# nschloe/flow

Hardware: AMD Instinct MI355X
Metric: ipcs_time_steps_per_sec (higher is better)
Workload: dtype f64

## Files before the change

flow_amd/_hip.py:

```python
import ctypes
import os

import torch

from . import device

_HERE = os.path.dirname(os.path.abspath(__file__))
LIB_PATH = os.path.join(_HERE, 'csrc', 'libflow_hip.so')

REDUCE_WORK = 4096
GMRES_MAX_RESTART = 30
GMRES_PARTIALS = (GMRES_MAX_RESTART + 2) * 1024
GMRES_STATE = 1280
SPMV_ROWS_PER_BLOCK = 256
SPMV_NNZ_PER_BLOCK = 1022
PMG_NNZ_PER_BLOCK = 2044

c_double_p = ctypes.c_void_p
c_int_p = ctypes.c_void_p


class Operator(ctypes.Structure):
    _fields_ = [
        ('kind', ctypes.c_int),
# ... 127 lines not shown
        ('packed16', ctypes.c_void_p),
        ('cbase16', ctypes.c_void_p),
        ('work16_rows', ctypes.c_int),
        ]


class MassStripsS(ctypes.Structure):
    _fields_ = [
        ('nlevels', ctypes.c_int),
        ('rowblocks16', ctypes.c_void_p * 16),
        ('nblocks16', ctypes.c_int * 16),
        ('row_lo_last', ctypes.c_int), ('row_hi_last', ctypes.c_int),
        ]


class MeshS(ctypes.Structure):
    _fields_ = [('nc', ctypes.c_int), ('xy', ctypes.c_void_p),
                ('c0', ctypes.c_int), ('c1', ctypes.c_int)]


class SpaceS(ctypes.Structure):
    _fields_ = [
        ('deg', ctypes.c_int),
        ('n', ctypes.c_int),
        ('nnz', ctypes.c_int),
        ('cell_dofs', ctypes.c_void_p),
        ('cptr', ctypes.c_void_p),
        ('csrc', ctypes.c_void_p),
        ('vptr', ctypes.c_void_p),
        ('vsrc', ctypes.c_void_p),
        ('r0', ctypes.c_int), ('r1', ctypes.c_int),
        ('nnz0', ctypes.c_int), ('nnz1', ctypes.c_int),
        ]


class CoefS(ctypes.Structure):
    _fields_ = [
        ('nl', ctypes.c_int),
        ('cell_stride', ctypes.c_int),
        ('values', ctypes.c_void_p),
        ('G', ctypes.c_void_p),
        ]


FORM_MAX_PROGRAM = 64
FORM_REGISTERS = 8
FORM_MAX_CONSTANTS = 32
FORM_MAX_FIELDS = 6
FORM_MAX_EXPRESSIONS = 4
FORM_MAX_POINTS = 256


class FormS(ctypes.Structure):
    _fields_ = [
        ('nprog', ctypes.c_int),
        ('prog', ctypes.c_int * (4 * FORM_MAX_PROGRAM)),
        ('nconst', ctypes.c_int),
        ('consts', ctypes.c_double * FORM_MAX_CONSTANTS),
        ('nfield', ctypes.c_int),
        ('field', ctypes.c_void_p * FORM_MAX_FIELDS),
        ('field_deg', ctypes.c_int * FORM_MAX_FIELDS),
        ('cell_dofs', ctypes.c_void_p * 2),
        ('nexpr', ctypes.c_int),
        ('expr', ctypes.c_void_p * FORM_MAX_EXPRESSIONS),
        ('expr_nl', ctypes.c_int * FORM_MAX_EXPRESSIONS),
        ('expr_table', ctypes.c_int * FORM_MAX_EXPRESSIONS),
        ('nq', ctypes.c_int),
        ('rule', ctypes.c_void_p),
        ('tables', ctypes.c_void_p),
        ('ntables', ctypes.c_int),
        ('nout', ctypes.c_int),
        ]


class PointGridS(ctypes.Structure):
    _fields_ = [
        ('nx', ctypes.c_int), ('ny', ctypes.c_int),
        ('x0', ctypes.c_double), ('y0', ctypes.c_double),
        ('hx_inv', ctypes.c_double), ('hy_inv', ctypes.c_double),
        ('start', ctypes.c_void_p),
        ('cells', ctypes.c_void_p),
        ]


class NsParams(ctypes.Structure):
    _fields_ = [
        ('dt', ctypes.c_double), ('rho', ctypes.c_double),
        ('mu', ctypes.c_double), ('theta_i', ctypes.c_double),
        ('theta_e', ctypes.c_double),
        ]


ALLREDUCE_FN = ctypes.CFUNCTYPE(ctypes.c_int, ctypes.c_void_p, ctypes.c_int)


class PeerS(ctypes.Structure):
    _fields_ = [
        ('flags', ctypes.c_void_p), ('land', ctypes.c_void_p),
        ('land_cap', ctypes.c_int), ('spin_limit', ctypes.c_int),
        ('nb_flags', ctypes.c_void_p * 2), ('nb_land', ctypes.c_void_p * 2),
        ('seq_host', ctypes.POINTER(ctypes.c_ulonglong * 5)),
        ]


PEER_FLAGS = 16


class CommS(ctypes.Structure):
    _fields_ = [
        ('rank', ctypes.c_int), ('world', ctypes.c_int),
        ('buf', ctypes.c_void_p), ('capacity', ctypes.c_int),
        ('allreduce', ALLREDUCE_FN), ('user', ctypes.c_void_p),
        ('peer', ctypes.POINTER(PeerS)),
        ]


class RcclBinding(ctypes.Structure):
    _fields_ = [('comm', ctypes.c_void_p), ('buf', ctypes.c_void_p),
                ('stream', ctypes.c_void_p)]


class RowsS(ctypes.Structure):
    _fields_ = [
        ('n', ctypes.c_int), ('r0', ctypes.c_int), ('r1', ctypes.c_int),
        ('e0', ctypes.c_int), ('e1', ctypes.c_int), ('nhalo', ctypes.c_int),
        ('send_row', ctypes.c_int * 2), ('send_len', ctypes.c_int * 2),
        ('send_slot', ctypes.c_int * 2),
        ('recv_row', ctypes.c_int * 2), ('recv_len', ctypes.c_int * 2),
        ('recv_slot', ctypes.c_int * 2),
        ]


class MgShardS(ctypes.Structure):
    _fields_ = [
        ('mg', ctypes.POINTER(MgS)),
        ('Ah0', Operator), ('Ps0', Operator), ('Rg', Operator),
        ('Cg', Operator),
        ('up_rowblocks0', ctypes.c_void_p), ('up_nblocks0', ctypes.c_int),
        ('z_lo', ctypes.c_int), ('z_hi', ctypes.c_int),
        ]


class MomentumJvp(ctypes.Structure):
    _fields_ = [
        ('mesh', ctypes.POINTER(MeshS)),
        ('W', ctypes.POINTER(SpaceS)),
        ('bfmask', ctypes.c_void_p),
        ('ui', ctypes.c_void_p),
        ('prm', NsParams),
        ('scratch', ctypes.c_void_p),
        ('nbc', ctypes.c_int),
        ('bc_dofs', ctypes.c_void_p),
        ('bc_mask', ctypes.c_void_p),
        ]


_VP = ctypes.c_void_p
_I = ctypes.c_int
_D = ctypes.c_double
_P = ctypes.POINTER
SYMBOLS = {
    'flow_abi_version': [],
    'flow_launch_count': [_P(ctypes.c_ulonglong)],
    'flow_graph_mode': [_I, ctypes.c_longlong],
    'flow_graph_stats': [_P(ctypes.c_ulonglong)],
    'flow_xcd_tile_host': [_I, _I],
    'flow_spmv_tile_nnz': [_I],
    'flow_operator_apply': [_P(Operator), _VP, _VP, _VP],
    'flow_profile_spmv_begin': [_I, _I],
    'flow_profile_spmv_end': [_P(_D), _P(_I)],
    'flow_profile_event_overhead': [_P(_D), _VP],
    'flow_profile_marker': [_I, _VP],
    'flow_profile_stream_copy': [ctypes.c_size_t, _VP, _VP, _VP],
    'flow_profile_stream_read': [ctypes.c_size_t, _VP, _VP, _VP],
    'flow_operator_diag_inv': [_P(Operator), _VP, _VP, _VP],
    'flow_dot_host': [_I, _VP, _VP, _VP, _P(_D), _VP],
    'flow_norm_host': [_I, _VP, _I, _VP, _P(_D), _VP],
    'flow_axpby': [_I, _D, _VP, _D, _VP, _VP],
    'flow_vmul': [_I, _D, _VP, _VP, _VP, _VP],
    'flow_fill': [_I, _D, _VP, _VP],
    'flow_lincomb': [_I, _I, _P(_D), _P(_VP), _VP, _VP],
    'flow_fingerprint': [_I, _P(_VP), _P(_I), _VP, _VP, _VP],
    'flow_read_doubles': [_VP, _I, _P(_D), _VP],
    'flow_extrapolation_weights': [_I, _P(_D), _D, _I, _I, _P(_D)],
    'flow_scale_rows': [_I, _VP, _VP, _VP, _VP],
    'flow_cg_solve': [_P(Operator), _VP, _P(CoarseS), _P(MgS), _VP, _VP, _D, _D,
                      _I, _I, _I, _VP, ctypes.c_size_t, _P(_I), _P(_D), _VP],
    'flow_cg_solve_guarded': [_P(Operator), _VP, _P(CoarseS), _P(MgS), _VP, _VP,
                              _VP, _D, _D, _I, _I, _I, _VP, ctypes.c_size_t,
                              _P(_I), _P(_D), _P(_I), _VP],
    'flow_mg_apply': [_P(MgS), _I, _VP, _VP, _VP],
    'flow_two_level_apply': [_P(CoarseS), _VP, _VP, _VP, _VP, _VP],
    'flow_bicgstab_solve': [_P(Operator), _VP, _P(IluS), _VP, _VP, _D, _D, _I,
                            _I, _I, _VP, ctypes.c_size_t, _P(_I), _P(_D), _VP],
    'flow_gmres_solve': [_P(Operator), _VP, _P(IluS), _P(PmgS), _VP, _VP, _D,
                         _D, _I, _I, _I, _I, _I, _VP, ctypes.c_size_t, _P(_I),
                         _P(_D), _VP],
    'flow_pmg_pack': [_I, _I, _VP, _VP, _VP, _VP, _VP, _VP, _VP, _VP, _VP],
    'flow_pmg_pack1': [_I, _I, _I, _VP, _VP, _VP, _VP, _VP, _VP, _VP, _VP, _VP,
                       _VP, _VP, _VP, _VP],
    'flow_pmg_cols16': [_I, _VP, _VP, _VP, _VP, _VP, _VP, _VP],
    'flow_pmg_lambda_max': [_P(PmgLevelS), _I, _VP, _VP, _VP, _P(_D), _VP],
    'flow_pmg_apply': [_P(PmgS), _VP, _VP, _VP],
    'flow_tl_apply': [_P(TlS), _VP, _VP, _VP],
    'flow_aggregate_host': [_I, _VP, _VP, _VP, ctypes.c_double, _VP, _VP,
                            _P(ctypes.c_int)],
    'flow_peer_alloc': [ctypes.c_int, _P(ctypes.c_void_p), ctypes.c_char_p],
    'flow_peer_open': [ctypes.c_char_p, _P(ctypes.c_void_p)],
    'flow_peer_close': [_VP],
    'flow_peer_free': [_VP],
    'flow_peer_status': [_P(PeerS), _P(ctypes.c_ulonglong), _VP],
    'flow_mass_pack': [_I, _VP, _VP, _VP, _VP, _VP],
    'flow_mass_pack16': [_I, _I, _VP, _VP, _VP, _VP, _VP, _VP, _VP, _VP, _VP],
    'flow_mass_solve': [_P(MassS), _VP, _VP, _D, _D, _I, _I, _VP,
                        ctypes.c_size_t, _P(_I), _P(_D), _VP],
    'flow_mass_solve_increment': [_P(MassS), _VP, _VP, _VP, _VP, _D, _D, _I, _I, _VP,
                                  ctypes.c_size_t, _P(_I), _P(_D), _VP],
    'flow_gather_rows': [_I, _VP, _I, _VP, _I, _VP, _I, _VP],
    'flow_color_greedy_host': [_I, _VP, _VP, _VP, _P(_I)],
    'flow_color_iterate_host': [_I, _VP, _VP, _VP, _P(_I), _I],
    'flow_ilu0_factor': [_P(IluPlanS), _I, _VP, _VP, _VP, _VP],
    'flow_ilu0_pack': [_P(IluS), _VP, _VP],
    'flow_ilu0_solve': [_P(IluS), _VP, _VP, _VP, _VP],
    'flow_rccl_load': [ctypes.c_char_p],
    'flow_rccl_unique_id': [_VP],
    'flow_rccl_comm_create': [_VP, _I, _I, _P(_VP)],
    'flow_rccl_comm_destroy': [_VP],
    'flow_rccl_allreduce': [_VP, _I],
    'flow_shard_halo': [_P(CommS), _P(RowsS), _I, _VP, _I, _VP],
    'flow_shard_reduce_host': [_P(CommS), _P(RowsS), _I, _VP, _VP, _I, _I, _VP,
                               _P(_D), _VP],
    'flow_shard_cg_solve': [_P(CommS), _P(RowsS), _P(Operator), _VP, _VP, _VP,
                            _D, _D, _I, _I, _I, _VP, ctypes.c_size_t, _P(_I),
                            _P(_D), _P(_I), _VP],
    'flow_shard_mgcg_solve': [_P(CommS), _P(RowsS), _P(Operator), _VP,
                              _P(MgShardS), _VP, _VP, _D, _D, _I, _I, _I, _VP,
                              ctypes.c_size_t, _P(_I), _P(_D), _P(_I), _VP],
    'flow_shard_mass_solve': [_P(CommS), _P(RowsS), _P(MassS), _P(MassStripsS),
                              _VP, _VP, _VP, _VP, _D, _D, _I, _I, _VP,
                              ctypes.c_size_t, _P(_I), _P(_D), _VP],
    'flow_shard_gmres_solve': [_P(CommS), _P(RowsS), _P(Operator), _P(IluS),
                               _P(PmgS), _VP, _VP, _D, _D, _I, _I, _I, _I, _I,
                               _VP, ctypes.c_size_t, _P(_I), _P(_D), _VP],
    'flow_assemble_scalar_matrix': [_I, _P(MeshS), _P(SpaceS), _VP, _VP, _VP],
    'flow_assemble_pressure_rhs': [_P(MeshS), _P(SpaceS), _P(SpaceS), _VP, _VP,
                                   _D, _D, _I, _VP, _VP, _VP],
    'flow_assemble_correction_rhs': [_P(MeshS), _P(SpaceS), _P(SpaceS), _VP,
                                     _VP, _VP, _D, _D, _I, _VP, _VP, _VP],
    'flow_assemble_momentum': [_P(MeshS), _P(SpaceS), _P(SpaceS), _VP, _VP, _VP,
                               _VP, _P(CoefS), _P(CoefS), _P(NsParams), _VP,
                               _VP, _VP, ctypes.c_size_t, _VP],
    'flow_momentum_jvp_apply': [_P(MomentumJvp), _VP, _VP, _VP],
    'flow_assemble_source': [_P(MeshS), _P(SpaceS), _I, _P(CoefS), _VP, _VP,
                             _VP],
    'flow_assemble_magnitude': [_P(MeshS), _P(SpaceS), _I, _VP, _VP, _VP, _VP],
    'flow_assemble_div_adjoint': [_P(MeshS), _P(SpaceS), _P(SpaceS), _VP, _VP,
                                  _VP, _VP],
    'flow_bc_identity_rows': [_P(Operator), _VP, _VP, _I, _VP, _VP],
    'flow_bc_residual': [_I, _VP, _VP, _VP, _VP, _VP],
    'flow_bc_set_values': [_I, _VP, _VP, _VP, _VP],
    'flow_bc_symmetric_matrix': [_I, _VP, _VP, _VP, _VP, _VP, _VP],
    'flow_assemble_heat': [_P(MeshS), _P(SpaceS), _P(SpaceS), _VP, _D, _D, _I,
                           _VP, _VP, _VP, _VP, _VP, _VP],
    'flow_assemble_heat_supg_source': [_P(MeshS), _P(SpaceS), _P(SpaceS), _VP,
                                       _D, _D, _P(CoefS), _VP, _VP, _VP, _VP],
    'flow_form_functional': [_P(MeshS), _P(FormS), _VP, _VP, _P(_D), _VP],
    'flow_form_load_vector': [_P(MeshS), _P(SpaceS), _P(FormS), _VP, _VP, _VP],
    'flow_form_facet_functional': [_P(MeshS), _P(FormS), _I, _VP, _VP, _VP, _VP,
                                   _P(_D), _VP],
    'flow_locate_points': [_P(MeshS), _P(PointGridS), _I, _VP, _VP, _VP, _VP],
    'flow_form_points': [_P(MeshS), _P(FormS), _I, _VP, _VP, _VP, _VP],
    }

_LIB = None


class HipError(RuntimeError):
    pass


class NotConverged(RuntimeError):
    '''Krylov / Newton non-convergence.  A RuntimeError, because callers of the
    reference catch exactly that (tests/test_boussinesq.py:254).'''


ABI_VERSION = 30


def load_library():
    global _LIB
    if _LIB is None:
        if not os.path.isfile(LIB_PATH):
            raise HipError(
                'libflow_hip.so not found at %s -- build it with '
                '`python -c "import __graft_entry__ as g; g.build()"` or '
                '`make -C flow_amd/csrc`' % LIB_PATH
                )
        lib = ctypes.CDLL(LIB_PATH)
        lib.flow_last_error.restype = ctypes.c_char_p
        lib.flow_last_error.argtypes = []
        for name, argtypes in SYMBOLS.items():
            fn = getattr(lib, name)
            fn.restype = ctypes.c_int
            fn.argtypes = argtypes
        got = lib.flow_abi_version()
        if got != ABI_VERSION:
            raise HipError(
                '%s is ABI version %d, these bindings are version %d: '
                'rebuild it (`make -C flow_amd/csrc`)'
                % (LIB_PATH, got, ABI_VERSION))
        _LIB = lib
    return _LIB


def launch_count():
    n = ctypes.c_ulonglong(0)
    check(load_library().flow_launch_count(ctypes.byref(n)))
    return int(n.value)


_GRAPHS = {'mode': None}


def graph_mode(mode, auto_rows=-1, sites=0):
    check(load_library().flow_graph_mode(int(mode) | (int(sites) << 4),
                                         int(auto_rows)))
    _GRAPHS['mode'] = int(mode)


def graphs_possible():
    if _GRAPHS['mode'] is not None:
        return _GRAPHS['mode'] != 0
    return os.environ.get('FLOW_AMD_GRAPHS', '0') not in ('', '0')


def graph_stats():
    v = (ctypes.c_ulonglong * 8)()
    check(load_library().flow_graph_stats(v))
    return {'graphs': int(v[0]), 'captures': int(v[1]), 'replays': int(v[2]),
            'nodes': int(v[3]), 'captures_cg': int(v[4]),
            'captures_gmres': int(v[5]), 'captures_mass': int(v[6])}


def spmv_tile_nnz(kind=0):
    return int(load_library().flow_spmv_tile_nnz(int(kind)))


def lib():
    handle = load_library()
    if not device.on_gpu():
        raise HipError(
            'flow_amd needs an AMD GPU (MI355X): the hot path has no CPU '
            'fallback'
            )
    return handle


def check(rc):
    if rc == 0:
        return
    msg = load_library().flow_last_error().decode('utf-8', 'replace')
    if rc == 1:
        raise NotConverged(msg)
    if rc == 2:
        raise ValueError(msg)
    raise HipError(msg)


def _ptr(t, dtype, numel=None, name='operand'):
    if t is None:
        return None
    if not isinstance(t, torch.Tensor):
        raise TypeError('%s: expected a torch tensor' % name)
    if t.dtype != dtype:
        raise TypeError('%s: dtype %s, expected %s' % (name, t.dtype, dtype))
    if not t.is_cuda:
        raise HipError('%s is not in device memory' % name)
    if not t.is_contiguous():
        raise ValueError('%s is not contiguous' % name)
    if numel is not None and t.numel() < numel:
        raise ValueError(
            '%s has %d elements, needs %d' % (name, t.numel(), numel)
            )
    return ctypes.c_void_p(t.data_ptr())


def f64(t, numel=None, name='fp64 operand'):
    return _ptr(t, torch.float64, numel, name)


def f32(t, numel=None, name='fp32 operand'):
    return _ptr(t, torch.float32, numel, name)


def f16(t, numel=None, name='fp16 operand'):
    return _ptr(t, torch.float16, numel, name)


def i32(t, numel=None, name='int32 operand'):
    return _ptr(t, torch.int32, numel, name)


def u8(t, numel=None, name='uint8 operand'):
    return _ptr(t, torch.uint8, numel, name)

# ... 27 lines not shown
```

flow_amd/csrc/assembly_kernels.hip:

```cpp
#include <cstdlib>

#include "fem_device.h"

namespace flow {

template <int NP>
__global__ __launch_bounds__(kBlock) void gather_kernel(
    int nout, const int* __restrict__ ptr, const int* __restrict__ src,
    const double* __restrict__ scratch, size_t plane_stride, size_t out_stride,
    double* __restrict__ out, const double* __restrict__ stop,
    const unsigned char* __restrict__ idrow = nullptr, size_t id_stride = 0,
    const double* __restrict__ v = nullptr, size_t v_stride = 0) {
  if (stopped(stop)) return;
  for (int k = blockIdx.x * blockDim.x + threadIdx.x; k < nout;
       k += gridDim.x * blockDim.x) {
    const int a = ptr[k];
    const int b = ptr[k + 1];
    double s[NP];
#pragma unroll
    for (int p = 0; p < NP; ++p) s[p] = 0.0;
    for (int t = a; t < b; t += 4) {
      int idx[4];
#pragma unroll
      for (int j = 0; j < 4; ++j) idx[j] = t + j < b ? src[t + j] : -1;
      double w[NP][4];
#pragma unroll
      for (int p = 0; p < NP; ++p)
#pragma unroll
        for (int j = 0; j < 4; ++j)
          w[p][j] = idx[j] >= 0 ? scratch[p * plane_stride + idx[j]] : 0.0;
#pragma unroll
      for (int p = 0; p < NP; ++p)
#pragma unroll
        for (int j = 0; j < 4; ++j) s[p] += w[p][j];
    }
    if (idrow) {
#pragma unroll
      for (int p = 0; p < NP; ++p)
        if (idrow[p * id_stride + k]) s[p] = v[p * v_stride + k];
    }
#pragma unroll
    for (int p = 0; p < NP; ++p) out[static_cast<size_t>(p) * out_stride + k] = s[p];
  }
}

int gather(int nout, int nplanes, const int* ptr, const int* src,
           const double* scratch, size_t plane_stride, double* out,
           hipStream_t st, size_t out_stride, int r0, int r1, const double* stop,
           const unsigned char* idrow, const double* v, size_t v_stride) {
  const size_t os = out_stride ? out_stride : static_cast<size_t>(nout);
  const size_t ids = static_cast<size_t>(nout);
  if (r1 > 0) {
    ptr += r0;
    out += r0;
    if (idrow) idrow += r0;
    if (v) v += r0;
    nout = r1 - r0;
  }
  const dim3 grid(grid_for(nout, kBlock, 1 << 20));
  FLOW_REQUIRE(nplanes == 1 || nplanes == 2, "gather: 1 or 2 planes");
  if (nplanes == 1)
    hipLaunchKernelGGL(gather_kernel<1>, grid, dim3(kBlock), 0, st, nout, ptr,
                       src, scratch, plane_stride, os, out, stop, idrow, ids, v,
                       v_stride);
  else
    hipLaunchKernelGGL(gather_kernel<2>, grid, dim3(kBlock), 0, st, nout, ptr,
                       src, scratch, plane_stride, os, out, stop, idrow, ids, v,
                       v_stride);
  FLOW_CHECK_LAUNCH();
  return FLOW_OK;
}

template <int NL>
__device__ __forceinline__ void load_local(const double* __restrict__ u, int n,
                                           const int* __restrict__ cd, int nc,
                                           int c, int ,
                                           double U[2][NL]) {
#pragma unroll
  for (int i = 0; i < NL; ++i) {
    const int d = cd[i * nc + c];
    U[0][i] = u[d];
    U[1][i] = u[static_cast<size_t>(n) + d];
  }
}

template <int DEG>
__global__ __launch_bounds__(kBlock) void scalar_matrix_kernel(
    int kind, int nc, const double* __restrict__ xy,
    double* __restrict__ scratch) {
  constexpr int NL = Elem<DEG>::NL;
  constexpr int NQ = Elem<2>::NQ;
  const int c = blockIdx.x * blockDim.x + threadIdx.x;
  if (c >= nc) return;
  const Geom g = load_geom(xy, nc, c);
  double Ke[NL][NL];
#pragma unroll
  for (int i = 0; i < NL; ++i)
#pragma unroll
    for (int j = 0; j < NL; ++j) Ke[i][j] = 0.0;
  if (kind == 2) {
#pragma unroll
    for (int i = 0; i < 3; ++i) Ke[i][i] = g.adet / 6.0;
  } else {
#pragma unroll
    for (int q = 0; q < NQ; ++q) {
      const double L[3] = {kQ7L[q][0], kQ7L[q][1], kQ7L[q][2]};
      const double w = 0.5 * kQ7W[q] * g.adet;
      double phi[NL], dphi[NL][3], gphi[NL][2];
      basis<DEG>(L, phi, dphi);
      phys_grad<NL>(g, dphi, gphi);
#pragma unroll
      for (int i = 0; i < NL; ++i)
#pragma unroll
        for (int j = 0; j < NL; ++j)
          Ke[i][j] += (kind == 0)
                          ? w * (gphi[i][0] * gphi[j][0] + gphi[i][1] * gphi[j][1])
                          : w * phi[i] * phi[j];
    }
  }
#pragma unroll
  for (int i = 0; i < NL; ++i)
#pragma unroll
    for (int j = 0; j < NL; ++j)
      scratch[static_cast<size_t>(i * NL + j) * nc + c] = Ke[i][j];
}

template <int DEG>
__global__ __launch_bounds__(kBlock) void pressure_rhs_kernel(
    int nc, int cb, int ce, const double* __restrict__ xy, const int* __restrict__ cdu, int nu,
    const int* __restrict__ cdp, const double* __restrict__ u,
    const double* __restrict__ p0, double alpha_rho_dt, double mu,
    int rotational, double* __restrict__ scratch) {
  constexpr int NL = Elem<DEG>::NL;
  const int c = cb + xcd_tile(blockIdx.x, gridDim.x) * blockDim.x + threadIdx.x;
  if (c >= ce) return;
  const Geom g = load_geom(xy, nc, c);
  double U[2][NL];
  load_local<NL>(u, nu, cdu, nc, c, 2, U);
  double d[3];
  div_at_vertices<DEG>(g, U, d);
  const double area = 0.5 * g.adet;
  const double dsum = d[0] + d[1] + d[2];
  double gp[2] = {0.0, 0.0};
#pragma unroll
  for (int k = 0; k < 3; ++k) {
    double coef = p0[cdp[k * nc + c]];
    if (rotational) coef -= mu * d[k];
    gp[0] += coef * g.gl[k][0];
    gp[1] += coef * g.gl[k][1];
  }
#pragma unroll
  for (int i = 0; i < 3; ++i) {
    const double b = -alpha_rho_dt * (area / 12.0) * (dsum + d[i]) +
                     area * (gp[0] * g.gl[i][0] + gp[1] * g.gl[i][1]);
    scratch[static_cast<size_t>(i) * nc + c] = b;
  }
}

template <int DEG>
__global__ __launch_bounds__(kBlock) void correction_rhs_kernel(
    int nc, int cb, int ce, const double* __restrict__ xy, const int* __restrict__ cdu, int nu,
    const int* __restrict__ cdp, const double* __restrict__ u,
    const double* __restrict__ p1, const double* __restrict__ p0, double dt_rho,
    double mu, int rotational, double* __restrict__ scratch) {
  constexpr int NL = Elem<DEG>::NL;
  constexpr int NQ = Elem<2>::NQ;
  const int c = cb + xcd_tile(blockIdx.x, gridDim.x) * blockDim.x + threadIdx.x;
  if (c >= ce) return;
  const Geom g = load_geom(xy, nc, c);
  double U[2][NL];
  load_local<NL>(u, nu, cdu, nc, c, 2, U);
  double d[3] = {0.0, 0.0, 0.0};
  if (rotational & 1) div_at_vertices<DEG>(g, U, d);
  const double mass = (rotational & 2) ? 0.0 : 1.0;
  double gphi_f[2] = {0.0, 0.0};
#pragma unroll
  for (int k = 0; k < 3; ++k) {
    const int dof = cdp[k * nc + c];
    const double coef = p1[dof] - p0[dof] + mu * d[k];
    gphi_f[0] += coef * g.gl[k][0];
    gphi_f[1] += coef * g.gl[k][1];
  }
  double acc[2][NL];
#pragma unroll
  for (int a = 0; a < 2; ++a)
#pragma unroll
    for (int i = 0; i < NL; ++i) acc[a][i] = 0.0;
#pragma unroll
  for (int q = 0; q < NQ; ++q) {
    const double L[3] = {kQ7L[q][0], kQ7L[q][1], kQ7L[q][2]};
    const double w = 0.5 * kQ7W[q] * g.adet;
    double phi[NL], dphi[NL][3];
    basis<DEG>(L, phi, dphi);
#pragma unroll
    for (int a = 0; a < 2; ++a) {
      double uq = 0.0;
#pragma unroll
      for (int j = 0; j < NL; ++j) uq += U[a][j] * phi[j];
      const double val = w * (mass * uq - dt_rho * gphi_f[a]);
#pragma unroll
      for (int i = 0; i < NL; ++i) acc[a][i] += val * phi[i];
    }
  }
#pragma unroll
  for (int a = 0; a < 2; ++a)
#pragma unroll
    for (int i = 0; i < NL; ++i)
      scratch[static_cast<size_t>(a * NL + i) * nc + c] = acc[a][i];
}

template <int NL>
__device__ __forceinline__ void add_source(const flow_coef& f, int nc, int c,
                                           int dim, double scale,
                                           double acc[][NL]) {
  const size_t nce = f.cell_stride ? static_cast<size_t>(nc) : 1;
  const size_t cc = f.cell_stride ? static_cast<size_t>(c) : 0;
  for (int a = 0; a < dim; ++a) {
    for (int l = 0; l < f.nl; ++l) {
      const double F = scale * f.values[(static_cast<size_t>(a) * f.nl + l) * nce + cc];
#pragma unroll
      for (int i = 0; i < NL; ++i) acc[a][i] += F * f.G[l * NL + i];
    }
  }
}

template <int DEG>
__global__ __launch_bounds__(kBlock) void source_kernel(
    int nc, const double* __restrict__ xy, int dim, flow_coef f,
    double* __restrict__ scratch) {
  constexpr int NL = Elem<DEG>::NL;
  const int c = blockIdx.x * blockDim.x + threadIdx.x;
  if (c >= nc) return;
  const Geom g = load_geom(xy, nc, c);
  double acc[2][NL];
#pragma unroll
  for (int a = 0; a < 2; ++a)
#pragma unroll
    for (int i = 0; i < NL; ++i) acc[a][i] = 0.0;
  add_source<NL>(f, nc, c, dim, g.adet, acc);
  for (int a = 0; a < dim; ++a)
#pragma unroll
    for (int i = 0; i < NL; ++i)
      scratch[static_cast<size_t>(a * NL + i) * nc + c] = acc[a][i];
}

template <int NL>
__device__ __forceinline__ void add_rhs_weak_point(
    double w, double rho, double mu, const double U[2][NL], const double P[3],
    const double L[3], const double phi[NL], const double gphi[NL][2],
    double acc[2][NL]) {
  double uq[2] = {0.0, 0.0};
  double gu[2][2] = {{0.0, 0.0}, {0.0, 0.0}};
#pragma unroll
  for (int j = 0; j < NL; ++j) {
#pragma unroll
    for (int a = 0; a < 2; ++a) {
      uq[a] += U[a][j] * phi[j];
      gu[a][0] += U[a][j] * gphi[j][0];
      gu[a][1] += U[a][j] * gphi[j][1];
    }
  }
  const double pq = P[0] * L[0] + P[1] * L[1] + P[2] * L[2];
  const double conv[2] = {gu[0][0] * uq[0] + gu[0][1] * uq[1],
                          gu[1][0] * uq[0] + gu[1][1] * uq[1]};
#pragma unroll
  for (int i = 0; i < NL; ++i) {
    const double ugp = uq[0] * gphi[i][0] + uq[1] * gphi[i][1];
#pragma unroll
    for (int a = 0; a < 2; ++a) {
      double r = -0.5 * rho * (conv[a] * phi[i] - ugp * uq[a]);
      r -= mu * ((gu[a][0] + gu[0][a]) * gphi[i][0] +
                 (gu[a][1] + gu[1][a]) * gphi[i][1]);
      r += pq * gphi[i][a];
      acc[a][i] += w * r;
    }
  }
}

template <int DEG>
__device__ __forceinline__ void add_rhs_weak_facets(
    int mask, double scale, double mu, const Geom& g,
    const double U[2][Elem<DEG>::NL], const double P[3],
    double acc[2][Elem<DEG>::NL]) {
  constexpr int NL = Elem<DEG>::NL;
  for (int lf = 0; lf < 3; ++lf) {
    if (!((mask >> lf) & 1)) continue;
    const int v0 = facet_v0(lf), v1 = facet_v1(lf);
    const double nL[2] = {-g.gl[lf][0] * g.adet, -g.gl[lf][1] * g.adet};
    for (int gq = 0; gq < 2; ++gq) {
      const double s = gq == 0 ? FLOW_G2A : FLOW_G2B;
      double L[3] = {0.0, 0.0, 0.0};
      L[v0] = 1.0 - s;
      L[v1] = s;
      double phi[NL], dphi[NL][3], gphi[NL][2];
      basis<DEG>(L, phi, dphi);
      phys_grad<NL>(g, dphi, gphi);
      double gu[2][2] = {{0.0, 0.0}, {0.0, 0.0}};
#pragma unroll
      for (int j = 0; j < NL; ++j)
#pragma unroll
        for (int a = 0; a < 2; ++a) {
          gu[a][0] += U[a][j] * gphi[j][0];
          gu[a][1] += U[a][j] * gphi[j][1];
        }
      const double pq = P[0] * L[0] + P[1] * L[1] + P[2] * L[2];
      const double w = 0.5 * scale;
#pragma unroll
      for (int a = 0; a < 2; ++a) {
        const double t = -pq * nL[a] + mu * (gu[0][a] * nL[0] + gu[1][a] * nL[1]);
#pragma unroll
        for (int i = 0; i < NL; ++i) acc[a][i] += w * t * phi[i];
      }
    }
  }
}

template <int DEG>
__global__ __launch_bounds__(kBlock) void momentum_residual_kernel(
    int nc, int cb, int ce, const double* __restrict__ xy, const int* __restrict__ cdu, int nu,
    const int* __restrict__ cdp, const int* __restrict__ bfmask,
    const double* __restrict__ ui, const double* __restrict__ u0,
    const double* __restrict__ p0, flow_coef f0, flow_coef f1,
    flow_ns_params prm, double* __restrict__ scratch) {
  constexpr int NL = Elem<DEG>::NL;
  constexpr int NQ = Elem<DEG>::NQ;
  const int c = cb + xcd_tile(blockIdx.x, gridDim.x) * blockDim.x + threadIdx.x;
  if (c >= ce) return;
  const Geom g = load_geom(xy, nc, c);
  double Ui[2][NL], U0[2][NL], P[3];
  load_local<NL>(ui, nu, cdu, nc, c, 2, Ui);
  load_local<NL>(u0, nu, cdu, nc, c, 2, U0);
#pragma unroll
  for (int k = 0; k < 3; ++k) P[k] = p0[cdp[k * nc + c]];
  const int mask = bfmask[c];
  const double ci = -prm.dt / prm.rho * prm.theta_i;
  const double cexp = -prm.dt / prm.rho * prm.theta_e;
  double acc[2][NL];
#pragma unroll
  for (int a = 0; a < 2; ++a)
#pragma unroll
    for (int i = 0; i < NL; ++i) acc[a][i] = 0.0;

#pragma unroll
  for (int q = 0; q < NQ; ++q) {
    const double L[3] = {qpoint<DEG>(q, 0), qpoint<DEG>(q, 1), qpoint<DEG>(q, 2)};
    const double w = 0.5 * qweight<DEG>(q) * g.adet;
    double phi[NL], dphi[NL][3], gphi[NL][2];
    basis<DEG>(L, phi, dphi);
    phys_grad<NL>(g, dphi, gphi);
#pragma unroll
    for (int a = 0; a < 2; ++a) {
      double du = 0.0;
#pragma unroll
      for (int j = 0; j < NL; ++j) du += (Ui[a][j] - U0[a][j]) * phi[j];
#pragma unroll
      for (int i = 0; i < NL; ++i) acc[a][i] += w * du * phi[i];
    }
    if (ci != 0.0)
      add_rhs_weak_point<NL>(w * ci, prm.rho, prm.mu, Ui, P, L, phi, gphi, acc);
    if (cexp != 0.0)
      add_rhs_weak_point<NL>(w * cexp, prm.rho, prm.mu, U0, P, L, phi, gphi, acc);
  }
  if (mask) {
    if (ci != 0.0) add_rhs_weak_facets<DEG>(mask, ci, prm.mu, g, Ui, P, acc);
    if (cexp != 0.0) add_rhs_weak_facets<DEG>(mask, cexp, prm.mu, g, U0, P, acc);
  }
  if (ci != 0.0) add_source<NL>(f1, nc, c, 2, ci * g.adet, acc);
  if (cexp != 0.0) add_source<NL>(f0, nc, c, 2, cexp * g.adet, acc);
#pragma unroll
  for (int a = 0; a < 2; ++a)
#pragma unroll
    for (int i = 0; i < NL; ++i)
      scratch[static_cast<size_t>(a * NL + i) * nc + c] = acc[a][i];
}

template <int DEG>
__global__ __launch_bounds__(kBlock) void momentum_jvp_kernel(
    int nc, int cb, int ce, const double* __restrict__ xy,
    const int* __restrict__ cdu, int nu, int nv,
    const int* __restrict__ bfmask, const double* __restrict__ ui,
    const double* __restrict__ v, flow_ns_params prm,
    const double* __restrict__ prm_dev,
    double* __restrict__ scratch, const double* __restrict__ stop) {
  constexpr int NL = Elem<DEG>::NL;
  constexpr int NQ = Elem<DEG>::NQ;
  if (stopped(stop)) return;
  const int c = cb + xcd_tile(blockIdx.x, gridDim.x) * blockDim.x + threadIdx.x;
  if (c >= ce) return;
  const Geom g = load_geom(xy, nc, c);
  double U[2][NL], V[2][NL];
  load_local<NL>(ui, nu, cdu, nc, c, 2, U);
  load_local<NL>(v, nv, cdu, nc, c, 2, V);
  const int mask = bfmask[c];
  const double ci = prm_dev ? load_scalar(prm_dev)
                            : -prm.dt / prm.rho * prm.theta_i;
  const double hr = prm_dev ? load_scalar(prm_dev + 1) : 0.5 * prm.rho;
  const double mu = prm_dev ? load_scalar(prm_dev + 2) : prm.mu;
  double acc[2][NL];
#pragma unroll
  for (int a = 0; a < 2; ++a)
#pragma unroll
    for (int i = 0; i < NL; ++i) acc[a][i] = 0.0;

#pragma unroll
  for (int q = 0; q < NQ; ++q) {
    const double L[3] = {qpoint<DEG>(q, 0), qpoint<DEG>(q, 1), qpoint<DEG>(q, 2)};
    const double w = 0.5 * qweight<DEG>(q) * g.adet;
    double uq[2], vq[2], gu[2][2], gv[2][2];
#pragma unroll
    for (int a = 0; a < 2; ++a) {
      uq[a] = eval_at<DEG>(U[a], L);
      vq[a] = eval_at<DEG>(V[a], L);
      double gur[3], gvr[3];
      ref_gradient<DEG>(U[a], L, gur);
      ref_gradient<DEG>(V[a], L, gvr);
#pragma unroll
      for (int d = 0; d < 2; ++d) {
        gu[a][d] = gur[0] * g.gl[0][d] + gur[1] * g.gl[1][d] + gur[2] * g.gl[2][d];
        gv[a][d] = gvr[0] * g.gl[0][d] + gvr[1] * g.gl[1][d] + gvr[2] * g.gl[2][d];
      }
    }
#pragma unroll
    for (int a = 0; a < 2; ++a) {
      const double dconv = gv[a][0] * uq[0] + gv[a][1] * uq[1] +
                           gu[a][0] * vq[0] + gu[a][1] * vq[1];
      const double s0 = w * (vq[a] - ci * hr * dconv);
      double S1[2];
#pragma unroll
      for (int d = 0; d < 2; ++d)
        S1[d] = w * ci * (hr * (vq[d] * uq[a] + uq[d] * vq[a]) -
                          mu * (gv[a][d] + gv[d][a]));
      double T[3];
#pragma unroll
      for (int k = 0; k < 3; ++k) T[k] = g.gl[k][0] * S1[0] + g.gl[k][1] * S1[1];
      test_accumulate<DEG>(L, s0, T, acc[a]);
    }
  }
  if (mask && ci != 0.0) {
    const double P0[3] = {0.0, 0.0, 0.0};
    add_rhs_weak_facets<DEG>(mask, ci, mu, g, V, P0, acc);
  }
#pragma unroll
  for (int a = 0; a < 2; ++a)
#pragma unroll
    for (int i = 0; i < NL; ++i)
      scratch[static_cast<size_t>(a * NL + i) * nc + c] = acc[a][i];
}

template <int DEG>
__global__ __launch_bounds__(kBlock) void momentum_jvp_pair_kernel(
    int nc, int cb, int ce, const double* __restrict__ xy,
    const int* __restrict__ cdu, int nu, int nv,
    const int* __restrict__ bfmask, const double* __restrict__ ui,
    const double* __restrict__ v, flow_ns_params prm,
    const double* __restrict__ prm_dev,
    double* __restrict__ scratch, const double* __restrict__ stop) {
  constexpr int NL = Elem<DEG>::NL;
  constexpr int NQ = Elem<DEG>::NQ;
  if (stopped(stop)) return;
  const int t = xcd_tile(blockIdx.x, gridDim.x) * blockDim.x + threadIdx.x;
  const int c = cb + (t >> 1);
  const int a = t & 1;
  if (c >= ce) return;
  const Geom g = load_geom(xy, nc, c);
  double U[NL], V[NL];
#pragma unroll
  for (int i = 0; i < NL; ++i) {
    const int d = cdu[i * nc + c];
    U[i] = ui[static_cast<size_t>(a) * nu + d];
    V[i] = v[static_cast<size_t>(a) * nv + d];
  }
  const int mask = bfmask[c];
  const double ci = prm_dev ? load_scalar(prm_dev)
                            : -prm.dt / prm.rho * prm.theta_i;
  const double hr = prm_dev ? load_scalar(prm_dev + 1) : 0.5 * prm.rho;
  const double mu = prm_dev ? load_scalar(prm_dev + 2) : prm.mu;
  double acc[NL];
#pragma unroll
  for (int i = 0; i < NL; ++i) acc[i] = 0.0;

#pragma unroll
  for (int q = 0; q < NQ; ++q) {
    const double L[3] = {qpoint<DEG>(q, 0), qpoint<DEG>(q, 1), qpoint<DEG>(q, 2)};
    const double w = 0.5 * qweight<DEG>(q) * g.adet;
    const double uq = eval_at<DEG>(U, L);
    const double vq = eval_at<DEG>(V, L);
    double gur[3], gvr[3], gu[2], gv[2];
    ref_gradient<DEG>(U, L, gur);
    ref_gradient<DEG>(V, L, gvr);
#pragma unroll
    for (int d = 0; d < 2; ++d) {
      gu[d] = gur[0] * g.gl[0][d] + gur[1] * g.gl[1][d] + gur[2] * g.gl[2][d];
      gv[d] = gvr[0] * g.gl[0][d] + gvr[1] * g.gl[1][d] + gvr[2] * g.gl[2][d];
    }
    const double uo = __shfl_xor(uq, 1, 64);
    const double vo = __shfl_xor(vq, 1, 64);
    const double cross = __shfl_xor(a == 0 ? gv[1] : gv[0], 1, 64);
    const double u0 = a == 0 ? uq : uo, u1 = a == 0 ? uo : uq;
    const double v0 = a == 0 ? vq : vo, v1 = a == 0 ? vo : vq;
    const double dconv = gv[0] * u0 + gv[1] * u1 + gu[0] * v0 + gu[1] * v1;
    const double s0 = w * (vq - ci * hr * dconv);
    const double t0 = a == 0 ? gv[0] : cross;
    const double t1 = a == 0 ? cross : gv[1];
    double S1[2];
    S1[0] = w * ci * (hr * (v0 * uq + u0 * vq) - mu * (gv[0] + t0));
    S1[1] = w * ci * (hr * (v1 * uq + u1 * vq) - mu * (gv[1] + t1));
    double T[3];
#pragma unroll
    for (int k = 0; k < 3; ++k) T[k] = g.gl[k][0] * S1[0] + g.gl[k][1] * S1[1];
    test_accumulate<DEG>(L, s0, T, acc);
  }
  if (mask && ci != 0.0) {
    for (int lf = 0; lf < 3; ++lf) {
      if (!((mask >> lf) & 1)) continue;
      const int f0 = facet_v0(lf), f1 = facet_v1(lf);
      const double nL[2] = {-g.gl[lf][0] * g.adet, -g.gl[lf][1] * g.adet};
      for (int gq = 0; gq < 2; ++gq) {
        const double sg = gq == 0 ? FLOW_G2A : FLOW_G2B;
        double L[3] = {0.0, 0.0, 0.0};
        L[f0] = 1.0 - sg;
        L[f1] = sg;
        double gvr[3], gv[2];
        ref_gradient<DEG>(V, L, gvr);
#pragma unroll
        for (int d = 0; d < 2; ++d)
          gv[d] = gvr[0] * g.gl[0][d] + gvr[1] * g.gl[1][d] + gvr[2] * g.gl[2][d];
        const double cross = __shfl_xor(a == 0 ? gv[1] : gv[0], 1, 64);
        const double tn = a == 0 ? gv[0] * nL[0] + cross * nL[1]
                                 : cross * nL[0] + gv[1] * nL[1];
        const double wt = 0.5 * ci * mu * tn;
        double phi[NL], dphi[NL][3];
        basis<DEG>(L, phi, dphi);
#pragma unroll
        for (int i = 0; i < NL; ++i) acc[i] += wt * phi[i];
      }
    }
  }
#pragma unroll
  for (int i = 0; i < NL; ++i)
    scratch[static_cast<size_t>(a * NL + i) * nc + c] = acc[i];
}

__global__ void bc_copy_kernel(int nbc, const int* __restrict__ dofs, int n,
                               int r0, int r1, const double* __restrict__ v,
                               int vs, double* __restrict__ out, int os,
                               const double* __restrict__ stop) {
  if (stopped(stop)) return;
  const int k = blockIdx.x * blockDim.x + threadIdx.x;
  if (k >= nbc) return;
  const int d = dofs[k];
  const int a = d / n;
  const int row = d - a * n;
  if (row >= r0 && row < r1)
    out[static_cast<size_t>(a) * os + row] = v[static_cast<size_t>(a) * vs + row];
}

template <int DEG>
struct BasisTab {
  double phi[Elem<DEG>::NQ][Elem<DEG>::NL];
  double dphi[Elem<DEG>::NQ][Elem<DEG>::NL][3];
};

template <int DEG>
__global__ __launch_bounds__(kBlock) void momentum_jacobian_kernel(
    int nc, int cb, int ce, const double* __restrict__ xy, const int* __restrict__ cdu, int nu,
    const int* __restrict__ bfmask, const double* __restrict__ ui,
    flow_ns_params prm, double* __restrict__ scratch) {
  constexpr int NL = Elem<DEG>::NL;
  constexpr int NQ = Elem<DEG>::NQ;
  constexpr int NP = NL * NL;
  __shared__ double s_uq[NQ][2][64];
  __shared__ double s_gu[NQ][4][64];
  __shared__ BasisTab<DEG> tab;

  const int lane = threadIdx.x & 63;
  const int grp = threadIdx.x >> 6;
  const int c = cb + blockIdx.x * 64 + lane;
  const bool active = c < ce;
  const int cc = active ? c : ce - 1;

  for (int t = threadIdx.x; t < NQ * NL; t += kBlock) {
    const int q = t / NL, i = t % NL;
    const double L[3] = {qpoint<DEG>(q, 0), qpoint<DEG>(q, 1), qpoint<DEG>(q, 2)};
    double phi[NL], dphi[NL][3];
    basis<DEG>(L, phi, dphi);
    tab.phi[q][i] = phi[i];
    tab.dphi[q][i][0] = dphi[i][0];
    tab.dphi[q][i][1] = dphi[i][1];
    tab.dphi[q][i][2] = dphi[i][2];
  }

  const Geom g = load_geom(xy, nc, cc);
  const int mask = bfmask[cc];
  {
    double U[2][NL];
    load_local<NL>(ui, nu, cdu, nc, cc, 2, U);
    for (int q = grp; q < NQ; q += 4) {
      const double L[3] = {qpoint<DEG>(q, 0), qpoint<DEG>(q, 1),
                           qpoint<DEG>(q, 2)};
// ... 503 lines not shown
    const flow_mesh* mesh, const flow_space* W, const flow_space* P,
    const double* u, const double* p1, const double* p0, double dt_rho,
    double mu, int rotational, double* scratch, double* b, void* stream) {
  int rc = check_mesh_space(mesh, W);
  if (rc) return rc;
  if ((rc = check_mesh_space(mesh, P))) return rc;
  FLOW_REQUIRE(P->deg == 1 && W->vptr && W->vsrc, "spaces");
  FLOW_REQUIRE(u && p1 && p0 && scratch && b, "pointers");
  hipStream_t st = as_stream(stream);
  const CellRange cr(mesh);
  FLOW_DISPATCH_DEG(W->deg, correction_rhs_kernel, cell_grid(cr.count()), st,
                    mesh->nc, cr.cb, cr.ce, mesh->xy, W->cell_dofs, W->n,
                    P->cell_dofs, u, p1, p0, dt_rho, mu, rotational, scratch);
  const int nl = W->deg == 1 ? 3 : 6;
  return gather(W->n, 2, W->vptr, W->vsrc, scratch,
                static_cast<size_t>(nl) * mesh->nc, b, st, 0, W->r0, W->r1);
}

static int check_coef(const flow_coef* f) {
  FLOW_REQUIRE(f && f->nl >= 1 && f->nl <= 21 && f->values && f->G, "coefficient");
  FLOW_REQUIRE(f->cell_stride == 0 || f->cell_stride == 1, "coefficient stride");
  return FLOW_OK;
}

extern "C" int flow_assemble_source(const flow_mesh* mesh, const flow_space* V,
                                    int dim, const flow_coef* f, double* scratch,
                                    double* b, void* stream) {
  int rc = check_mesh_space(mesh, V);
  if (rc) return rc;
  if ((rc = check_coef(f))) return rc;
  FLOW_REQUIRE(dim == 1 || dim == 2, "dim");
  FLOW_REQUIRE(scratch && b && V->vptr && V->vsrc, "pointers");
  hipStream_t st = as_stream(stream);
  FLOW_DISPATCH_DEG(V->deg, source_kernel, cell_grid(mesh->nc), st, mesh->nc,
                    mesh->xy, dim, *f, scratch);
  const int nl = V->deg == 1 ? 3 : 6;
  return gather(V->n, dim, V->vptr, V->vsrc, scratch,
                static_cast<size_t>(nl) * mesh->nc, b, st);
}

extern "C" int flow_assemble_momentum(
    const flow_mesh* mesh, const flow_space* W, const flow_space* P,
    const int* bfmask, const double* ui, const double* u0, const double* p0,
    const flow_coef* f0, const flow_coef* f1, const flow_ns_params* prm,
    double* scratch, double* F, double* Jvals, size_t j_plane_stride,
    void* stream) {
  int rc = check_mesh_space(mesh, W);
  if (rc) return rc;
  if ((rc = check_mesh_space(mesh, P))) return rc;
  if ((rc = check_coef(f0))) return rc;
  if ((rc = check_coef(f1))) return rc;
  FLOW_REQUIRE(P->deg == 1, "pressure space must be P1");
  FLOW_REQUIRE(bfmask && ui && u0 && p0 && prm && scratch, "pointers");
  FLOW_REQUIRE(prm->dt > 0.0 && prm->rho > 0.0 && prm->mu > 0.0, "parameters");
  hipStream_t st = as_stream(stream);
  const int nl = W->deg == 1 ? 3 : 6;
  const CellRange cr(mesh);
  if (F) {
    FLOW_REQUIRE(W->vptr && W->vsrc, "vector map");
    FLOW_DISPATCH_DEG(W->deg, momentum_residual_kernel, cell_grid(cr.count()),
                      st, mesh->nc, cr.cb, cr.ce, mesh->xy, W->cell_dofs, W->n,
                      P->cell_dofs, bfmask, ui, u0, p0, *f0, *f1, *prm, scratch);
    if ((rc = gather(W->n, 2, W->vptr, W->vsrc, scratch,
                     static_cast<size_t>(nl) * mesh->nc, F, st, 0, W->r0,
                     W->r1)))
      return rc;
  }
  if (Jvals) {
    FLOW_REQUIRE(W->cptr && W->csrc && W->nnz > 0, "matrix map");
    FLOW_REQUIRE(j_plane_stride >= (size_t)W->nnz, "Jacobian plane stride");
    FLOW_DISPATCH_DEG(W->deg, momentum_jacobian_kernel,
                      dim3((cr.count() + 63) / 64), st, mesh->nc, cr.cb, cr.ce,
                      mesh->xy, W->cell_dofs, W->n, bfmask, ui, *prm, scratch);
    int k0 = 0, k1 = W->nnz;
    if (W->r1 > 0) {
      FLOW_REQUIRE(W->nnz0 >= 0 && W->nnz0 < W->nnz1 && W->nnz1 <= W->nnz,
                   "space nonzero range");
      k0 = W->nnz0;
      k1 = W->nnz1;
    }
    hipLaunchKernelGGL(gather_blocks_kernel,
                       dim3(grid_for(k1 - k0, kBlock, 1 << 20)), dim3(kBlock), 0,
                       st, k0, k1, mesh->nc, nl * nl, W->cptr, W->csrc, scratch,
                       j_plane_stride, Jvals);
    FLOW_CHECK_LAUNCH();
  }
  return FLOW_OK;
}

int flow::momentum_jvp_check(const flow_momentum_jvp* J) {
  FLOW_REQUIRE(J != nullptr, "matrix-free Jacobian is NULL");
  int rc = check_mesh_space(J->mesh, J->W);
  if (rc) return rc;
  FLOW_REQUIRE(J->W->vptr && J->W->vsrc, "vector map");
  FLOW_REQUIRE(J->bfmask && J->ui && J->scratch, "matrix-free Jacobian pointers");
  FLOW_REQUIRE(J->prm.dt > 0.0 && J->prm.rho > 0.0 && J->prm.mu > 0.0,
               "parameters");
  FLOW_REQUIRE(J->nbc >= 0 && (J->nbc == 0 || J->bc_dofs), "Dirichlet dofs");
  return FLOW_OK;
}

__global__ void jvp_params_kernel(flow_ns_params prm, double* __restrict__ dst) {
  if (threadIdx.x == 0) {
    store_scalar(dst, -prm.dt / prm.rho * prm.theta_i);
    store_scalar(dst + 1, 0.5 * prm.rho);
    store_scalar(dst + 2, prm.mu);
  }
}

int flow::momentum_jvp_params(const flow_momentum_jvp* J, double* dst,
                              hipStream_t st) {
  hipLaunchKernelGGL(jvp_params_kernel, dim3(1), dim3(64), 0, st, J->prm, dst);
  FLOW_CHECK_LAUNCH();
  return FLOW_OK;
}

int flow::momentum_jvp_apply(const flow_momentum_jvp* J, const double* v,
                             double* out, hipStream_t st, int v_stride,
                             int out_stride, const double* stop,
                             const double* prm_dev) {
  const flow_mesh* mesh = J->mesh;
  const flow_space* W = J->W;
  const int nl = W->deg == 1 ? 3 : 6;
  const int vs = v_stride ? v_stride : W->n;
  const int os = out_stride ? out_stride : W->n;
  const CellRange cr(mesh);
  int rc;
  static const bool pair = [] {
    const char* e = getenv("FLOW_AMD_JVP_PAIR");
    return e && e[0] == '1';
  }();
  if (W->deg == 2 && pair) {
    hipLaunchKernelGGL(momentum_jvp_pair_kernel<2>, cell_grid(2 * cr.count()),
                       dim3(kBlock), 0, st, mesh->nc, cr.cb, cr.ce, mesh->xy,
                       W->cell_dofs, W->n, vs, J->bfmask, J->ui, v, J->prm,
                       prm_dev, J->scratch, stop);
    FLOW_CHECK_LAUNCH();
  } else {
    FLOW_DISPATCH_DEG(W->deg, momentum_jvp_kernel, cell_grid(cr.count()), st,
                      mesh->nc, cr.cb, cr.ce, mesh->xy, W->cell_dofs, W->n, vs,
                      J->bfmask, J->ui, v, J->prm, prm_dev, J->scratch, stop);
  }
  if ((rc = gather(W->n, 2, W->vptr, W->vsrc, J->scratch,
                   static_cast<size_t>(nl) * mesh->nc, out, st, os, W->r0,
                   W->r1, stop, J->nbc > 0 ? J->bc_mask : nullptr, v, vs)))
    return rc;
  if (J->nbc > 0 && !J->bc_mask) {
    const int r0 = W->r1 > 0 ? W->r0 : 0, r1 = W->r1 > 0 ? W->r1 : W->n;
    hipLaunchKernelGGL(bc_copy_kernel, dim3(grid_for(J->nbc)), dim3(kBlock), 0,
                       st, J->nbc, J->bc_dofs, W->n, r0, r1, v, vs, out, os, stop);
    FLOW_CHECK_LAUNCH();
  }
  return FLOW_OK;
}

extern "C" int flow_momentum_jvp_apply(const flow_momentum_jvp* J,
                                       const double* v, double* out,
                                       void* stream) {
  int rc = momentum_jvp_check(J);
  if (rc) return rc;
  FLOW_REQUIRE(v && out && v != out, "jvp vectors");
  return momentum_jvp_apply(J, v, out, as_stream(stream), 0, 0, nullptr);
}

extern "C" int flow_assemble_magnitude(const flow_mesh* mesh, const flow_space* W,
                                       int mode, const double* u,
                                       double* scratch, double* b,
                                       void* stream) {
  int rc = check_mesh_space(mesh, W);
  if (rc) return rc;
  FLOW_REQUIRE(mode == 0 || mode == 1, "mode");
  FLOW_REQUIRE(u && scratch && b && W->vptr && W->vsrc, "pointers");
  hipStream_t st = as_stream(stream);
  const CellRange cr(mesh);
  FLOW_DISPATCH_DEG(W->deg, magnitude_kernel, cell_grid(cr.count()), st, mesh->nc,
                    cr.cb, cr.ce, mesh->xy, W->cell_dofs, W->n, u, mode, scratch);
  return gather(W->n, 1, W->vptr, W->vsrc, scratch, 0, b, st, 0, W->r0, W->r1);
}

extern "C" int flow_assemble_div_adjoint(const flow_mesh* mesh,
                                         const flow_space* W, const flow_space* P,
                                         const double* p, double* scratch,
                                         double* out, void* stream) {
  int rc = check_mesh_space(mesh, W);
  if (rc) return rc;
  if ((rc = check_mesh_space(mesh, P))) return rc;
  FLOW_REQUIRE(P->deg == 1, "pressure space must be P1");
  FLOW_REQUIRE(p && scratch && out && W->vptr && W->vsrc, "pointers");
  hipStream_t st = as_stream(stream);
  FLOW_DISPATCH_DEG(W->deg, div_adjoint_kernel, cell_grid(mesh->nc), st, mesh->nc,
                    mesh->xy, P->cell_dofs, p, scratch);
  const int nl = W->deg == 1 ? 3 : 6;
  return gather(W->n, 2, W->vptr, W->vsrc, scratch,
                static_cast<size_t>(nl) * mesh->nc, out, st);
}

extern "C" int flow_bc_identity_rows(const flow_operator* A, double* vals_planes,
                                     const int* diag_idx, int nbc,
                                     const int* dofs, void* stream) {
  FLOW_REQUIRE(A && A->n > 0 && A->nnz > 0 && A->rowptr, "operator");
  FLOW_REQUIRE(A->kind >= 0 && A->kind <= 2, "operator kind");
  FLOW_REQUIRE(vals_planes && diag_idx && nbc >= 0, "pointers");
  if (nbc == 0) return FLOW_OK;
  FLOW_REQUIRE(dofs != nullptr, "dofs");
  FLOW_REQUIRE(vals_planes == A->vals[0], "vals_planes must be A->vals[0]");
  const long long stride =
      A->kind == 0 ? A->nnz : static_cast<long long>(A->vals[1] - A->vals[0]);
  FLOW_REQUIRE(stride >= A->nnz, "plane stride");
  if (A->kind == 2)
    FLOW_REQUIRE(A->vals[2] - A->vals[0] == 2 * stride &&
                     A->vals[3] - A->vals[0] == 3 * stride,
                 "equally spaced planes");
  hipLaunchKernelGGL(bc_identity_rows_kernel, dim3(grid_for(nbc)), dim3(kBlock),
                     0, as_stream(stream), A->kind, A->n,
                     static_cast<size_t>(stride), A->rowptr, diag_idx, nbc, dofs,
                     vals_planes);
  FLOW_CHECK_LAUNCH();
  return FLOW_OK;
}

extern "C" int flow_bc_residual(int nbc, const int* dofs, const double* g,
                                const double* u, double* F, void* stream) {
  FLOW_REQUIRE(nbc >= 0, "nbc");
  if (nbc == 0) return FLOW_OK;
  FLOW_REQUIRE(dofs && g && u && F, "pointers");
  hipLaunchKernelGGL(bc_residual_kernel, dim3(grid_for(nbc)), dim3(kBlock), 0,
                     as_stream(stream), nbc, dofs, g, u, F);
  FLOW_CHECK_LAUNCH();
  return FLOW_OK;
}

extern "C" int flow_bc_set_values(int nbc, const int* dofs, const double* g,
                                  double* x, void* stream) {
  FLOW_REQUIRE(nbc >= 0, "nbc");
  if (nbc == 0) return FLOW_OK;
  FLOW_REQUIRE(dofs && g && x, "pointers");
  hipLaunchKernelGGL(bc_residual_kernel, dim3(grid_for(nbc)), dim3(kBlock), 0,
                     as_stream(stream), nbc, dofs, g,
                     static_cast<const double*>(nullptr), x);
  FLOW_CHECK_LAUNCH();
  return FLOW_OK;
}

extern "C" int flow_bc_symmetric_matrix(int n, const int* rowptr,
                                        const int* cols, const double* vals_in,
                                        const unsigned char* isbc,
                                        double* vals_out, void* stream) {
  FLOW_REQUIRE(n > 0 && rowptr && cols && vals_in && isbc && vals_out, "pointers");
  hipLaunchKernelGGL(bc_symmetric_kernel, dim3(grid_for(n)), dim3(kBlock), 0,
                     as_stream(stream), n, rowptr, cols, vals_in, isbc, vals_out);
  FLOW_CHECK_LAUNCH();
  return FLOW_OK;
}

extern "C" int flow_assemble_heat(const flow_mesh* mesh, const flow_space* Q,
                                  const flow_space* W, const double* conv,
                                  double kappa, double rho_cp, int supg,
                                  double* scratch, double* Avals,
                                  double* Msupg_vals, double* tau_out,
                                  int* status_dev, void* stream) {
  int rc = check_mesh_space(mesh, Q);
  if (rc) return rc;
  if ((rc = check_mesh_space(mesh, W))) return rc;
  FLOW_REQUIRE(conv && scratch && Avals && status_dev, "pointers");
  FLOW_REQUIRE(Q->cptr && Q->csrc && Q->nnz > 0, "matrix map");
  FLOW_REQUIRE(!supg || Msupg_vals, "Msupg_vals required with supg");
  FLOW_REQUIRE(kappa > 0.0 && rho_cp > 0.0, "coefficients");
  hipStream_t st = as_stream(stream);
  const CellRange cr(mesh);
  const dim3 grid = cell_grid(cr.count());
#define FLOW_HEAT(DQ, DW)                                                      \
  do {                                                                         \
    if (supg)                                                                  \
      hipLaunchKernelGGL((heat_kernel<DQ, DW, true>), grid, dim3(kBlock), 0, st, \
                         mesh->nc, cr.cb, cr.ce, mesh->xy, W->cell_dofs, W->n, \
                         conv, kappa, rho_cp, scratch, tau_out, status_dev);   \
    else                                                                       \
      hipLaunchKernelGGL((heat_kernel<DQ, DW, false>), grid, dim3(kBlock), 0,  \
                         st, mesh->nc, cr.cb, cr.ce, mesh->xy, W->cell_dofs,   \
                         W->n, conv, kappa, rho_cp, scratch, tau_out,          \
                         status_dev);                                          \
  } while (0)
  if (Q->deg == 1 && W->deg == 1) FLOW_HEAT(1, 1);
  else if (Q->deg == 1 && W->deg == 2) FLOW_HEAT(1, 2);
  else if (Q->deg == 2 && W->deg == 1) FLOW_HEAT(2, 1);
  else FLOW_HEAT(2, 2);
#undef FLOW_HEAT
  FLOW_CHECK_LAUNCH();
  const int nl = Q->deg == 1 ? 3 : 6;
  const size_t plane = static_cast<size_t>(nl) * nl * mesh->nc;
  int k0 = 0, k1 = 0;
  if (Q->r1 > 0) {
    FLOW_REQUIRE(Q->nnz0 >= 0 && Q->nnz0 < Q->nnz1 && Q->nnz1 <= Q->nnz,
                 "space nonzero range");
    k0 = Q->nnz0;
    k1 = Q->nnz1;
  }
  if ((rc = gather(Q->nnz, 1, Q->cptr, Q->csrc, scratch, 0, Avals, st, 0, k0, k1)))
    return rc;
  if (supg)
    return gather(Q->nnz, 1, Q->cptr, Q->csrc, scratch + plane, 0, Msupg_vals, st,
                  0, k0, k1);
  return FLOW_OK;
}

extern "C" int flow_assemble_heat_supg_source(
// ... 30 lines not shown
```

flow_amd/csrc/common.h:

```cpp
#pragma once
#include <hip/hip_runtime.h>

#include <algorithm>
#include <cstdarg>
#include <cstdio>
#include <functional>
#include <vector>

#include "../../include/flow_hip.h"

namespace flow {
extern unsigned long long g_launches;
}
#undef hipLaunchKernelGGL
#define hipLaunchKernelGGL(kernelName, numBlocks, numThreads, memPerBlock,        \
                           streamId, ...)                                       \
  do {                                                                          \
    ++flow::g_launches;                                                         \
    (kernelName)<<<(numBlocks), (numThreads), (memPerBlock), (streamId)>>>(     \
        __VA_ARGS__);                                                           \
  } while (0)

namespace flow {

void set_error(const char* fmt, ...);

inline hipStream_t as_stream(void* s) { return static_cast<hipStream_t>(s); }

int ilu_apply(const flow_ilu* ilu, const double* in, double* out, double* work,
              hipStream_t st, const double* stop = nullptr);
int ilu_check(const flow_ilu* ilu, int op_size);

int pmg_apply(const flow_pmg* M, const double* r, double* z, hipStream_t st,
              const double* stop = nullptr);
int pmg_check(const flow_pmg* M, int op_size);
int tl_apply(const flow_tl* T, const double* r, double* z, hipStream_t st,
             const double* stop = nullptr);
int tl_check(const flow_tl* T, int op_size);
int operator_apply(const flow_operator* A, const double* x, double* y,
                   hipStream_t st, const double* stop = nullptr);
int operator_size(const flow_operator* A);
int sum_partials_host(double* work, int nparts, double* host, hipStream_t st);
int check_operator(const flow_operator* A);
int fill(int n, double value, double* y, hipStream_t st);
struct NoEarly {
  __device__ __forceinline__ void operator()(int, bool) const {}
};

enum Slot {
  kGamma = 0, kAlpha, kBeta, kRes2, kB2, kRho, kOmega, kRhoNew, kTmp,
  kBreak, kTarget2, kDone, kConvIt, kIter, kNumSlots = 16
};
int read_state(const double* S, double* host, hipStream_t st);
int check_comm(const flow_comm* c, long long need);
int check_rows(const flow_rows* R);
int exchange(const flow_comm* c, int count);
int exchange_halo(const flow_comm* C, const flow_rows* R, int ncomp, int sum_count,
                  int hoff, hipStream_t st);

int gather(int nout, int nplanes, const int* ptr, const int* src,
           const double* scratch, size_t plane_stride, double* out,
           hipStream_t st, size_t out_stride = 0, int r0 = 0, int r1 = 0,
           const double* stop = nullptr, const unsigned char* idrow = nullptr,
           const double* v = nullptr, size_t v_stride = 0);
int momentum_jvp_check(const flow_momentum_jvp* J);
int momentum_jvp_apply(const flow_momentum_jvp* J, const double* v, double* out,
                       hipStream_t st, int v_stride = 0, int out_stride = 0,
                       const double* stop = nullptr,
                       const double* prm_dev = nullptr);
int momentum_jvp_params(const flow_momentum_jvp* J, double* dst, hipStream_t st);

constexpr long long kReplayAutoRows = 1500000;
struct KeyHash {
  unsigned long long h = 1469598103934665603ull;
  void bytes(const void* p, size_t n) {
    const unsigned char* c = static_cast<const unsigned char*>(p);
    for (size_t i = 0; i < n; ++i) h = (h ^ c[i]) * 1099511628211ull;
  }
  template <class T> KeyHash& pod(const T& v) {
    bytes(&v, sizeof(T));
    return *this;
  }
  template <class T> KeyHash& obj(const T* p) {
    const unsigned char tag = p ? 1 : 0;
    bytes(&tag, 1);
    if (p) bytes(p, sizeof(T));
    return *this;
  }
};
enum ReplaySite { kReplayCg = 1, kReplayGmres = 2, kReplayMass = 4 };
bool replay_wanted(long long rows, int site);
int replay_prepare(unsigned long long key, int site, hipStream_t st,
                   const std::function<int()>& body, hipGraphExec_t* exec,
                   int* nodes);
int replay_launch(hipGraphExec_t exec, int nodes, hipStream_t st);
void key_operator(KeyHash& k, const flow_operator* A, bool skip_prm = false);

#define FLOW_CHECK_HIP(expr)                                                 \
  do {                                                                       \
    hipError_t err_ = (expr);                                                \
    if (err_ != hipSuccess) {                                                \
      flow::set_error("%s failed: %s (%s:%d)", #expr, hipGetErrorString(err_), \
                      __FILE__, __LINE__);                                   \
      return FLOW_HIP_ERROR;                                                 \
    }                                                                        \
  } while (0)

#define FLOW_REQUIRE(cond, msg)                                  \
  do {                                                           \
    if (!(cond)) {                                               \
      flow::set_error("invalid argument: %s (%s)", msg, #cond);  \
      return FLOW_INVALID;                                       \
    }                                                            \
  } while (0)

#define FLOW_CHECK_LAUNCH() FLOW_CHECK_HIP(hipGetLastError())

constexpr int kBlock = 256;
constexpr int kRedBlocks = 1024;
constexpr int kMaxGrid = 2048;

inline int grid_for(long long n, int per_block = kBlock, int cap = kMaxGrid) {
  long long g = (n + per_block - 1) / per_block;
  if (g < 1) g = 1;
  if (g > cap) g = cap;
  return static_cast<int>(g);
}

__device__ __forceinline__ double load_scalar(const double* p) {
  return __hip_atomic_load(const_cast<double*>(p), __ATOMIC_RELAXED,
                           __HIP_MEMORY_SCOPE_SYSTEM);
}
__device__ __forceinline__ void store_scalar(double* p, double v) {
  __hip_atomic_store(p, v, __ATOMIC_RELAXED, __HIP_MEMORY_SCOPE_SYSTEM);
}

__device__ __forceinline__ bool stopped(const double* stop) {
  return stop != nullptr && load_scalar(stop) != 0.0;
}

constexpr int kXcdRun = 64;
__host__ __device__ __forceinline__ int xcd_tile(int b, int nwg) {
  constexpr int kGroup = 8 * kXcdRun;
  const int full = (nwg / kGroup) * kGroup;
  if (b < full) {
    const int g = b / kGroup, i = b - g * kGroup;
    return g * kGroup + (i & 7) * kXcdRun + (i >> 3);
  }
  const int nt = nwg - full, i = b - full;
  const int q = nt >> 3, r = nt & 7, xcd = i & 7;
  return full + (xcd < r ? xcd * (q + 1) : r * (q + 1) + (xcd - r) * q) +
         (i >> 3);
}

__device__ inline double block_sum(double v) {
  __shared__ double wave_part[4];
#pragma unroll
  for (int off = 32; off > 0; off >>= 1) v += __shfl_down(v, off, 64);
  const int lane = threadIdx.x & 63;
  const int wave = threadIdx.x >> 6;
  __syncthreads();
  if (lane == 0) wave_part[wave] = v;
  __syncthreads();
  if (threadIdx.x == 0) v = wave_part[0] + wave_part[1] + wave_part[2] + wave_part[3];
  return v;
}

__device__ inline double block_sum_once(double v) {
  __shared__ double wave_part_once[4];
#pragma unroll
  for (int off = 32; off > 0; off >>= 1) v += __shfl_down(v, off, 64);
  if ((threadIdx.x & 63) == 0) wave_part_once[threadIdx.x >> 6] = v;
  __syncthreads();
  if (threadIdx.x == 0)
    v = wave_part_once[0] + wave_part_once[1] + wave_part_once[2] +
        wave_part_once[3];
  return v;
}

__device__ inline double block_max(double v) {
  __shared__ double wave_part_m[4];
#pragma unroll
  for (int off = 32; off > 0; off >>= 1) v = fmax(v, __shfl_down(v, off, 64));
  const int lane = threadIdx.x & 63;
  const int wave = threadIdx.x >> 6;
  __syncthreads();
  if (lane == 0) wave_part_m[wave] = v;
  __syncthreads();
  if (threadIdx.x == 0)
    v = fmax(fmax(wave_part_m[0], wave_part_m[1]), fmax(wave_part_m[2], wave_part_m[3]));
  return v;
}

}
```

flow_amd/csrc/la_kernels.hip:

```cpp
#include <cstring>

#include "common.h"
#include "csr_stream.h"

namespace flow {

thread_local char g_error[512] = "";

void set_error(const char* fmt, ...) {
  va_list ap;
  va_start(ap, fmt);
  vsnprintf(g_error, sizeof(g_error), fmt, ap);
  va_end(ap);
}

static_assert(3 * kRedBlocks + kNumSlots <= FLOW_REDUCE_WORK, "work size");


template <bool DOT>
__global__ __launch_bounds__(kBlock) void spmv_stream_kernel(
    int n, const int* __restrict__ rowptr, const int* __restrict__ cols,
    const double* __restrict__ vals0, const double* __restrict__ vals1,
    const int* __restrict__ rowblocks, const double* __restrict__ x,
    double* __restrict__ y, double* __restrict__ dpart,
// ... 44 lines not shown
        g = ci * yi;
        rr = yi * yi;
      }
    } else {
      y[r] = ci - s;
    }
  }
  if (DOTS) {
    g = block_sum(g);
    rr = block_sum(rr);
    if (threadIdx.x == 0) {
      gpart[blockIdx.x] = g;
      rpart[blockIdx.x] = rr;
    }
  }
}

template <bool DOTS>
__global__ __launch_bounds__(kBlock) void mg_up2_kernel(
    const int* __restrict__ rowblocks, const int* __restrict__ p_rowptr,
    const int* __restrict__ p_cols, const double* __restrict__ p_vals,
    const int* __restrict__ a_rowptr, const int* __restrict__ a_cols,
    const double* __restrict__ a_vals, const double* __restrict__ xc,
    const double* __restrict__ c, const double* __restrict__ dinv, double omega,
    double* __restrict__ y, double* __restrict__ gpart,
    double* __restrict__ rpart, const double* __restrict__ stop,
    int own_lo = 0, int own_hi = 0x7fffffff) {
  __shared__ double prod_p[kTile];
  __shared__ double prod_a[kTile];
  if (stopped(stop)) return;
  const int tile = xcd_tile(blockIdx.x, gridDim.x);
  const int r0 = rowblocks[tile];
  const int r1 = rowblocks[tile + 1];
  const int r = r0 + threadIdx.x;
  double ci = 0.0, di = 0.0;
  if (r < r1) {
    ci = c[r];
    di = dinv[r];
  }
  const double sp = stream_rows_sum(r0, r1, p_rowptr, p_cols, p_vals, xc, prod_p);
  const double sa = stream_rows_sum(r0, r1, a_rowptr, a_cols, a_vals, c, prod_a);
  double g = 0.0, rr = 0.0;
  if (r < r1) {
    const double yi = sp + omega * di * (2.0 * ci - sa);
    y[r] = yi;
    if (DOTS && r >= own_lo && r < own_hi) {
      g = ci * yi;
      rr = yi * yi;
    }
  }
  if (DOTS) {
    g = block_sum(g);
    rr = block_sum(rr);
    if (threadIdx.x == 0) {
      gpart[blockIdx.x] = g;
      rpart[blockIdx.x] = rr;
    }
  }
}

template <bool DOT>
__global__ __launch_bounds__(kBlock) void spmv_stream_block2_kernel(
    int n, const int* __restrict__ rowptr, const int* __restrict__ cols,
    const double* __restrict__ vxx, const double* __restrict__ vxy,
    const double* __restrict__ vyx, const double* __restrict__ vyy,
    const int* __restrict__ rowblocks, const double* __restrict__ x,
    double* __restrict__ y, double* __restrict__ dpart,
    const double* __restrict__ stop) {
  __shared__ double prod0[kTile2];
  __shared__ double prod1[kTile2];
  if (stopped(stop)) return;
  const int tile = xcd_tile(blockIdx.x, gridDim.x);
  const int r0 = rowblocks[tile];
  const int r1 = rowblocks[tile + 1];
  const int k0 = rowptr[r0];
  const int k1 = rowptr[r1];
  const int ka = k0 & ~1;
  const int r = r0 + threadIdx.x;
  int a = 0, b = 0;
  if (r < r1) {
    a = rowptr[r] - ka;
    b = rowptr[r + 1] - ka;
  }
  const int npair = (k1 - ka + 1) >> 1;
  const int2* __restrict__ c2p = reinterpret_cast<const int2*>(cols + ka);
  const double2* __restrict__ pxx = reinterpret_cast<const double2*>(vxx + ka);
  const double2* __restrict__ pxy = reinterpret_cast<const double2*>(vxy + ka);
  const double2* __restrict__ pyx = reinterpret_cast<const double2*>(vyx + ka);
  const double2* __restrict__ pyy = reinterpret_cast<const double2*>(vyy + ka);
#pragma unroll
  for (int j = 0; j < kPairs2; ++j) {
    const int p = threadIdx.x + j * kBlock;
    if (p < npair) {
      const int2 c = c2p[p];
      const double2 axx = pxx[p], axy = pxy[p], ayx = pyx[p], ayy = pyy[p];
      const int cx = 2 * p >= k0 - ka ? c.x : cols[k0];
      const int cy = 2 * p + 1 < k1 - ka ? c.y : cols[k0];
      const double u0 = x[cx], u1 = x[n + cx];
      const double w0 = x[cy], w1 = x[n + cy];
      prod0[2 * p] = axx.x * u0 + axy.x * u1;
      prod1[2 * p] = ayx.x * u0 + ayy.x * u1;
      prod0[2 * p + 1] = axx.y * w0 + axy.y * w1;
      prod1[2 * p + 1] = ayx.y * w0 + ayy.y * w1;
    }
  }
  __syncthreads();
  double t = 0.0;
  if (r < r1) {
    double s0 = 0.0, s1 = 0.0;
    for (int k = a; k < b; ++k) {
      s0 += prod0[k];
      s1 += prod1[k];
    }
    y[r] = s0;
    y[n + r] = s1;
    if (DOT) t = s0 * x[r] + s1 * x[n + r];
  }
  if (DOT) {
    t = block_sum_once(t);
    if (threadIdx.x == 0) dpart[blockIdx.x] = t;
  }
}

template <bool DOT>
__global__ __launch_bounds__(kBlock) void spmv_stream_pair_kernel(
    int n, const int* __restrict__ rowptr, const int* __restrict__ cols,
    const double* __restrict__ vals, const int* __restrict__ rowblocks,
    const unsigned char* __restrict__ mask, const double* __restrict__ x,
    double* __restrict__ y, int xs, double* __restrict__ dpart,
    const double* __restrict__ stop) {
  __shared__ double2 prod[kTile2];
  if (stopped(stop)) return;
  int r, r1;
  const double2 s =
      stream_tile_pair_row_sum(rowptr, cols, vals, rowblocks, x, xs, prod, r, r1);
  double s0 = s.x, s1 = s.y;
  double t = 0.0;
  if (r < r1) {
    const double x0 = x[r], x1 = x[xs + r];
    if (!mask[r]) s0 = x0;
    if (!mask[n + r]) s1 = x1;
    y[r] = s0;
    y[xs + r] = s1;
    if (DOT) t = s0 * x0 + s1 * x1;
  }
  if (DOT) {
    t = block_sum_once(t);
    if (threadIdx.x == 0) dpart[blockIdx.x] = t;
  }
}

int check_operator(const flow_operator* A) {
  FLOW_REQUIRE(A != nullptr, "operator is NULL");
  FLOW_REQUIRE(A->kind >= 0 && A->kind <= 4, "operator kind");
  if (A->kind == 3) {
    const flow_momentum_jvp* J =
        static_cast<const flow_momentum_jvp*>(A->matfree);
    int rc = momentum_jvp_check(J);
    if (rc) return rc;
    FLOW_REQUIRE(A->n == J->W->n, "matrix-free operator size");
    return FLOW_OK;
  }
  FLOW_REQUIRE(A->n > 0 && A->nnz > 0 && A->nblocks > 0, "operator sizes");
  FLOW_REQUIRE(A->rowptr && A->cols && A->rowblocks, "operator pattern");
  const int planes = (A->kind == 0 || A->kind == 4) ? 1 : (A->kind == 1 ? 2 : 4);
  FLOW_REQUIRE(A->kind != 4 || A->rowmask != nullptr, "operator row mask");
  for (int p = 0; p < planes; ++p) {
    FLOW_REQUIRE(A->vals[p] != nullptr, "operator value plane");
    FLOW_REQUIRE((reinterpret_cast<size_t>(A->vals[p]) & 15) == 0,
                 "value planes must be 16-byte aligned");
  }
  FLOW_REQUIRE((reinterpret_cast<size_t>(A->cols) & 7) == 0,
               "cols must be 8-byte aligned");
  return FLOW_OK;
}

static inline int op_size(const flow_operator* A) {
  return A->kind == 0 ? A->n : 2 * A->n;
}

static inline int dot_parts(const flow_operator* A) {
  return A->kind == 1 ? 2 * A->nblocks : A->nblocks;
}

struct SpmvProfile {
  int rows = 0, cap = 0, used = 0;
  hipEvent_t* ev = nullptr;
};
static SpmvProfile g_spmv_profile;

void key_operator(KeyHash& k, const flow_operator* A, bool skip_prm) {
  k.obj(A);
  if (A && A->kind == 3 && A->matfree) {
    flow_momentum_jvp J = *static_cast<const flow_momentum_jvp*>(A->matfree);
    if (skip_prm) J.prm = flow_ns_params{0.0, 0.0, 0.0, 0.0, 0.0};
    k.obj(&J).obj(J.mesh).obj(J.W);
  }
}

static int apply(const flow_operator* A, const double* x, double* y,
                 hipStream_t st, double* dpart = nullptr,
                 const double* stop = nullptr, int vec_stride = 0,
                 int out_stride = 0, const double* jvp_prm = nullptr) {
  if (A->kind == 3) {
    FLOW_REQUIRE(dpart == nullptr, "matrix-free operators carry no fused dot");
    return momentum_jvp_apply(static_cast<const flow_momentum_jvp*>(A->matfree),
                              x, y, st, vec_stride, out_stride, stop, jvp_prm);
  }
  const int xs = vec_stride ? vec_stride : A->n;
  const dim3 grid(A->nblocks, A->kind == 1 ? 2 : 1);
  const double* v1 = A->kind == 1 ? A->vals[1] : A->vals[0];
  if (A->kind == 4) {
    if (dpart)
      hipLaunchKernelGGL(spmv_stream_pair_kernel<true>, grid, dim3(kBlock), 0, st,
                         A->n, A->rowptr, A->cols, A->vals[0], A->rowblocks,
                         A->rowmask, x, y, xs, dpart, stop);
    else
      hipLaunchKernelGGL(spmv_stream_pair_kernel<false>, grid, dim3(kBlock), 0,
                         st, A->n, A->rowptr, A->cols, A->vals[0], A->rowblocks,
                         A->rowmask, x, y, xs, dpart, stop);
  } else if (A->kind == 2) {
    if (dpart)
      hipLaunchKernelGGL(spmv_stream_block2_kernel<true>, grid, dim3(kBlock), 0,
                         st, A->n, A->rowptr, A->cols, A->vals[0], A->vals[1],
                         A->vals[2], A->vals[3], A->rowblocks, x, y, dpart,
                         stop);
    else
      hipLaunchKernelGGL(spmv_stream_block2_kernel<false>, grid, dim3(kBlock), 0,
                         st, A->n, A->rowptr, A->cols, A->vals[0], A->vals[1],
                         A->vals[2], A->vals[3], A->rowblocks, x, y, dpart,
                         stop);
  } else if (dpart) {
    SpmvProfile& pf = g_spmv_profile;
    const bool timed = pf.used < pf.cap && A->kind == 0 && A->n == pf.rows;
    if (timed) FLOW_CHECK_HIP(hipEventRecord(pf.ev[2 * pf.used], st));
    hipLaunchKernelGGL(spmv_stream_kernel<true>, grid, dim3(kBlock), 0, st, A->n,
                       A->rowptr, A->cols, A->vals[0], v1, A->rowblocks, x, y,
                       dpart, stop);
    if (timed) FLOW_CHECK_HIP(hipEventRecord(pf.ev[2 * pf.used++ + 1], st));
  } else {
    hipLaunchKernelGGL(spmv_stream_kernel<false>, grid, dim3(kBlock), 0, st,
                       A->n, A->rowptr, A->cols, A->vals[0], v1, A->rowblocks, x,
                       y, dpart, stop);
  }
  FLOW_CHECK_LAUNCH();
  return FLOW_OK;
}

int operator_apply(const flow_operator* A, const double* x, double* y,
                   hipStream_t st, const double* stop) {
  return apply(A, x, y, st, nullptr, stop);
}
int operator_size(const flow_operator* A) { return op_size(A); }

__global__ void diag_inv_kernel(int n, int planes_kind,
                                const int* __restrict__ diag_idx,
                                const double* __restrict__ v0,
                                const double* __restrict__ v1,
                                const unsigned char* __restrict__ mask,
                                double* __restrict__ dinv) {
  for (int i = blockIdx.x * blockDim.x + threadIdx.x; i < n;
       i += gridDim.x * blockDim.x) {
    const int k = diag_idx[i];
    dinv[i] = (mask && !mask[i]) ? 1.0 : 1.0 / v0[k];
    if (planes_kind > 0)
      dinv[n + i] = (mask && !mask[n + i]) ? 1.0 : 1.0 / v1[k];
  }
}

__global__ __launch_bounds__(kBlock) void dot3_kernel(
    int n, int nd, const double* __restrict__ a0, const double* __restrict__ b0,
    const double* __restrict__ a1, const double* __restrict__ b1,
    const double* __restrict__ a2, const double* __restrict__ b2,
    double* __restrict__ partial) {
  double s0 = 0.0, s1 = 0.0, s2 = 0.0;
  for (int i = blockIdx.x * blockDim.x + threadIdx.x; i < n;
       i += gridDim.x * blockDim.x) {
    s0 += a0[i] * b0[i];
    if (nd > 1) s1 += a1[i] * b1[i];
    if (nd > 2) s2 += a2[i] * b2[i];
  }
  s0 = block_sum(s0);
  if (nd > 1) s1 = block_sum(s1);
  if (nd > 2) s2 = block_sum(s2);
  if (threadIdx.x == 0) {
    partial[blockIdx.x] = s0;
    if (nd > 1) partial[kRedBlocks + blockIdx.x] = s1;
    if (nd > 2) partial[2 * kRedBlocks + blockIdx.x] = s2;
  }
}

__global__ __launch_bounds__(kBlock) void absmax_kernel(
    int n, const double* __restrict__ x, double* __restrict__ partial) {
  double m = 0.0;
  for (int i = blockIdx.x * blockDim.x + threadIdx.x; i < n;
       i += gridDim.x * blockDim.x)
    m = fmax(m, fabs(x[i]));
  m = block_max(m);
  if (threadIdx.x == 0) partial[blockIdx.x] = m;
}

__global__ __launch_bounds__(kBlock) void finish_kernel(
    int nparts, int nd, int is_max, const double* __restrict__ partial,
    double* __restrict__ out) {
  for (int j = 0; j < nd; ++j) {
    double v = 0.0;
    for (int i = threadIdx.x; i < nparts; i += kBlock) {
      const double p = load_scalar(partial + j * kRedBlocks + i);
      v = is_max ? fmax(v, p) : v + p;
    }
    v = is_max ? block_max(v) : block_sum(v);
    if (threadIdx.x == 0) store_scalar(out + j, v);
  }
}

__global__ void axpby_kernel(int n, double a, const double* __restrict__ x,
                             double b, double* __restrict__ y) {
  for (int i = blockIdx.x * blockDim.x + threadIdx.x; i < n;
       i += gridDim.x * blockDim.x)
    y[i] = (b == 0.0) ? a * x[i] : a * x[i] + b * y[i];
}

__global__ void fill_kernel(int n, double value, double* __restrict__ y) {
  for (int i = blockIdx.x * blockDim.x + threadIdx.x; i < n;
       i += gridDim.x * blockDim.x)
    y[i] = value;
}

int fill(int n, double value, double* y, hipStream_t st) {
  hipLaunchKernelGGL(fill_kernel, dim3(grid_for(n)), dim3(kBlock), 0, st, n,
                     value, y);
  FLOW_CHECK_LAUNCH();
  return FLOW_OK;
}

__global__ void vmul_kernel(int n, double a, const double* x, const double* y,
                            double* out, const double* stop = nullptr) {
  if (stopped(stop)) return;
  for (int i = blockIdx.x * blockDim.x + threadIdx.x; i < n;
       i += gridDim.x * blockDim.x)
    out[i] = a * x[i] * y[i];
}

__global__ void residual_kernel(int n, const double* __restrict__ b,
                                const double* __restrict__ q,
                                const double* __restrict__ dinv,
                                double* __restrict__ r, double* __restrict__ z) {
  for (int i = blockIdx.x * blockDim.x + threadIdx.x; i < n;
       i += gridDim.x * blockDim.x) {
    const double ri = b[i] - q[i];
    r[i] = ri;
    if (z) z[i] = dinv ? dinv[i] * ri : ri;
  }
}

constexpr int kScalarBlock = 1024;
__global__ __launch_bounds__(kScalarBlock) void cg_scalar_kernel(
    int nparts, int ndelta, int first, const double* __restrict__ gpart,
    const double* __restrict__ rpart, const double* __restrict__ dpart,
    double rtol2, double atol2, double* __restrict__ S) {
// ... 746 lines not shown

extern "C" int flow_xcd_tile_host(int block, int nblocks) {
  return xcd_tile(block, nblocks);
}

extern "C" int flow_profile_spmv_begin(int rows, int max_launches) {
  SpmvProfile& pf = g_spmv_profile;
  FLOW_REQUIRE(rows > 0 && max_launches > 0 && max_launches <= 100000,
               "profile arguments");
  FLOW_REQUIRE(pf.ev == nullptr, "a profile is already running");
  pf.ev = new hipEvent_t[2 * static_cast<size_t>(max_launches)];
  for (int i = 0; i < 2 * max_launches; ++i)
    FLOW_CHECK_HIP(hipEventCreate(&pf.ev[i]));
  pf.rows = rows;
  pf.used = 0;
  pf.cap = max_launches;
  return FLOW_OK;
}

__global__ void profile_null_kernel() {}

__global__ void profile_busy_kernel() {
  const unsigned long long t0 = wall_clock64();
  for (int i = 0; i < 100000; ++i) {
    if (wall_clock64() - t0 > 2000ull) break;
    __builtin_amdgcn_s_sleep(8);
  }
}

extern "C" int flow_profile_event_overhead(double* overhead_us, void* stream) {
  FLOW_REQUIRE(overhead_us != nullptr, "overhead result");
  hipStream_t st = as_stream(stream);
  constexpr int kN = 33;
  hipEvent_t ev[2 * kN];
  for (int i = 0; i < 2 * kN; ++i) FLOW_CHECK_HIP(hipEventCreate(&ev[i]));
  for (int i = 0; i < kN; ++i) {
    hipLaunchKernelGGL(profile_busy_kernel, dim3(256), dim3(64), 0, st);
    FLOW_CHECK_HIP(hipEventRecord(ev[2 * i], st));
    hipLaunchKernelGGL(profile_null_kernel, dim3(1), dim3(64), 0, st);
    FLOW_CHECK_HIP(hipEventRecord(ev[2 * i + 1], st));
  }
  FLOW_CHECK_HIP(hipStreamSynchronize(st));
  double t[kN];
  for (int i = 0; i < kN; ++i) {
    float ms = 0.0f;
    FLOW_CHECK_HIP(hipEventElapsedTime(&ms, ev[2 * i], ev[2 * i + 1]));
    t[i] = 1.0e3 * ms;
  }
  for (int i = 0; i < 2 * kN; ++i) (void)hipEventDestroy(ev[i]);
  for (int i = 1; i < kN; ++i)
    for (int j = i; j > 0 && t[j] < t[j - 1]; --j) {
      const double tmp = t[j];
      t[j] = t[j - 1];
      t[j - 1] = tmp;
    }
  *overhead_us = t[kN / 2];
  return FLOW_OK;
}

extern "C" int flow_profile_spmv_end(double* total_us, int* launches) {
  SpmvProfile& pf = g_spmv_profile;
  FLOW_REQUIRE(total_us && launches, "profile results");
  FLOW_REQUIRE(pf.ev != nullptr, "no profile is running");
  double total = 0.0;
  int rc = FLOW_OK;
  for (int i = 0; i < pf.used && rc == FLOW_OK; ++i) {
    float ms = 0.0f;
    if (hipEventSynchronize(pf.ev[2 * i + 1]) != hipSuccess ||
        hipEventElapsedTime(&ms, pf.ev[2 * i], pf.ev[2 * i + 1]) != hipSuccess) {
      set_error("reading the SpMV profile events failed");
      rc = FLOW_HIP_ERROR;
    }
    total += 1.0e3 * ms;
  }
  for (int i = 0; i < 2 * pf.cap; ++i) (void)hipEventDestroy(pf.ev[i]);
  delete[] pf.ev;
  *total_us = total;
  *launches = pf.used;
  pf = SpmvProfile();
  return rc;
}

extern "C" int flow_peer_alloc(int land_cap, void** base_out, char* handle_out) {
  FLOW_REQUIRE(land_cap > 0 && base_out && handle_out, "flow_peer_alloc arguments");
  static_assert(sizeof(hipIpcMemHandle_t) == 64, "IPC handle size");
  const size_t bytes = sizeof(unsigned long long) * FLOW_PEER_FLAGS +
                       2 * sizeof(double) * static_cast<size_t>(land_cap);
  void* base = nullptr;
  if (hipExtMallocWithFlags(&base, bytes, hipDeviceMallocFinegrained) != hipSuccess) {
    (void)hipGetLastError();
    FLOW_CHECK_HIP(hipMalloc(&base, bytes));
  }
  FLOW_CHECK_HIP(hipMemset(base, 0, bytes));
  FLOW_CHECK_HIP(hipDeviceSynchronize());
  hipIpcMemHandle_t h;
  hipError_t err = hipIpcGetMemHandle(&h, base);
  if (err != hipSuccess) {
    (void)hipGetLastError();
    (void)hipFree(base);
    FLOW_CHECK_HIP(hipMalloc(&base, bytes));
    FLOW_CHECK_HIP(hipMemset(base, 0, bytes));
    FLOW_CHECK_HIP(hipDeviceSynchronize());
    FLOW_CHECK_HIP(hipIpcGetMemHandle(&h, base));
  }
  memcpy(handle_out, &h, sizeof(h));
  *base_out = base;
  return FLOW_OK;
}

extern "C" int flow_peer_open(const char* handle, void** base_out) {
  FLOW_REQUIRE(handle && base_out, "flow_peer_open arguments");
  hipIpcMemHandle_t h;
  memcpy(&h, handle, sizeof(h));
  FLOW_CHECK_HIP(hipIpcOpenMemHandle(base_out, h, hipIpcMemLazyEnablePeerAccess));
  return FLOW_OK;
}

extern "C" int flow_peer_close(void* mapped_base) {
  FLOW_REQUIRE(mapped_base != nullptr, "flow_peer_close argument");
  FLOW_CHECK_HIP(hipIpcCloseMemHandle(mapped_base));
  return FLOW_OK;
}

extern "C" int flow_peer_free(void* base) {
  FLOW_REQUIRE(base != nullptr, "flow_peer_free argument");
  FLOW_CHECK_HIP(hipFree(base));
  return FLOW_OK;
}

extern "C" int flow_peer_status(const flow_peer* peer,
                                unsigned long long* error_host, void* stream) {
  FLOW_REQUIRE(peer && peer->flags && error_host, "flow_peer_status arguments");
  hipStream_t st = as_stream(stream);
  FLOW_CHECK_HIP(hipMemcpyAsync(error_host, peer->flags + 4, sizeof(*error_host),
                                hipMemcpyDeviceToHost, st));
  FLOW_CHECK_HIP(hipStreamSynchronize(st));
  return FLOW_OK;
}

extern "C" int flow_operator_apply(const flow_operator* A, const double* x,
                                   double* y, void* stream) {
  int rc = check_operator(A);
  if (rc) return rc;
  FLOW_REQUIRE(x && y && x != y, "x, y");
  return apply(A, x, y, as_stream(stream));
}

extern "C" int flow_operator_diag_inv(const flow_operator* A,
                                      const int* diag_idx, double* dinv,
                                      void* stream) {
  int rc = check_operator(A);
  if (rc) return rc;
  FLOW_REQUIRE(diag_idx && dinv, "diag_idx, dinv");
  FLOW_REQUIRE(A->kind != 3, "a matrix-free operator has no stored diagonal");
  const double* v1 = (A->kind == 0 || A->kind == 4)
                         ? A->vals[0]
                         : (A->kind == 1 ? A->vals[1] : A->vals[3]);
  hipLaunchKernelGGL(diag_inv_kernel, dim3(grid_for(A->n)), dim3(kBlock), 0,
                     as_stream(stream), A->n, A->kind, diag_idx, A->vals[0], v1,
                     A->kind == 4 ? A->rowmask
                                  : static_cast<const unsigned char*>(nullptr),
                     dinv);
  FLOW_CHECK_LAUNCH();
  return FLOW_OK;
}

__global__ void scale_rows_kernel(int n, const int* __restrict__ rowptr,
                                  const double* __restrict__ d,
                                  double* __restrict__ vals) {
  for (int r = blockIdx.x * blockDim.x + threadIdx.x; r < n;
       r += gridDim.x * blockDim.x) {
    const double di = d[r];
    for (int k = rowptr[r]; k < rowptr[r + 1]; ++k) vals[k] *= di;
  }
}

extern "C" int flow_scale_rows(int n, const int* rowptr, const double* d,
                               double* vals, void* stream) {
  FLOW_REQUIRE(n > 0 && rowptr && d && vals, "scale rows arguments");
  hipLaunchKernelGGL(scale_rows_kernel, dim3(grid_for(n)), dim3(kBlock), 0,
                     as_stream(stream), n, rowptr, d, vals);
  FLOW_CHECK_LAUNCH();
  return FLOW_OK;
}

extern "C" int flow_dot_host(int n, const double* x, const double* y,
                             double* work, double* result_host, void* stream) {
  FLOW_REQUIRE(n > 0 && x && y && work && result_host, "dot arguments");
  hipStream_t st = as_stream(stream);
  int np = 0;
  int rc = dots(n, 1, x, y, x, y, x, y, work, &np, st);
  if (rc) return rc;
  double* S = work + 3 * kRedBlocks;
  hipLaunchKernelGGL(finish_kernel, dim3(1), dim3(kBlock), 0, st, np, 1, 0, work,
                     S);
  FLOW_CHECK_LAUNCH();
  return read_slot(S, 0, result_host, st);
}

extern "C" int flow_norm_host(int n, const double* x, int kind, double* work,
                              double* result_host, void* stream) {
  FLOW_REQUIRE(n > 0 && x && work && result_host, "norm arguments");
  FLOW_REQUIRE(kind == 0 || kind == 1, "norm kind");
  hipStream_t st = as_stream(stream);
  double* S = work + 3 * kRedBlocks;
  if (kind == 0) {
    int rc = flow_dot_host(n, x, x, work, result_host, stream);
    if (rc) return rc;
    *result_host = sqrt(*result_host);
    return FLOW_OK;
  }
  const int g = grid_for(n, kBlock * 4, kRedBlocks);
  hipLaunchKernelGGL(absmax_kernel, dim3(g), dim3(kBlock), 0, st, n, x, work);
  hipLaunchKernelGGL(finish_kernel, dim3(1), dim3(kBlock), 0, st, g, 1, 1, work,
                     S);
  FLOW_CHECK_LAUNCH();
  return read_slot(S, 0, result_host, st);
}

extern "C" int flow_axpby(int n, double a, const double* x, double b, double* y,
                          void* stream) {
  FLOW_REQUIRE(n > 0 && x && y, "axpby arguments");
  hipLaunchKernelGGL(axpby_kernel, dim3(grid_for(n)), dim3(kBlock), 0,
                     as_stream(stream), n, a, x, b, y);
  FLOW_CHECK_LAUNCH();
  return FLOW_OK;
}

__global__ void gather_rows_kernel(int ncomp, int m, const int* __restrict__ idx,
                                   const double* __restrict__ src, int src_stride,
                                   double* __restrict__ dst, int dst_stride) {
  for (int t = blockIdx.x * blockDim.x + threadIdx.x; t < ncomp * m;
       t += gridDim.x * blockDim.x) {
    const int a = t / m, k = t - a * m;
    dst[static_cast<size_t>(a) * dst_stride + k] =
        src[static_cast<size_t>(a) * src_stride + idx[k]];
  }
}

extern "C" int flow_gather_rows(int ncomp, const int* idx, int m,
                                const double* src, int src_stride, double* dst,
                                int dst_stride, void* stream) {
  FLOW_REQUIRE(ncomp >= 1 && m > 0 && idx && src && dst && src_stride > 0 &&
                   dst_stride >= m,
               "gather_rows arguments");
  hipLaunchKernelGGL(gather_rows_kernel, dim3(grid_for(static_cast<long long>(ncomp) * m)),
                     dim3(kBlock), 0, as_stream(stream), ncomp, m, idx, src,
                     src_stride, dst, dst_stride);
  FLOW_CHECK_LAUNCH();
  return FLOW_OK;
}

__global__ __launch_bounds__(kBlock) void stream_copy_kernel(
    size_t n2, const double2* __restrict__ src, double2* __restrict__ dst) {
  constexpr int U = 4;
  const size_t stride = static_cast<size_t>(gridDim.x) * blockDim.x;
  size_t i = static_cast<size_t>(blockIdx.x) * blockDim.x + threadIdx.x;
  for (; i + (U - 1) * stride < n2; i += U * stride) {
    double2 v[U];
#pragma unroll
    for (int u = 0; u < U; ++u) {
      v[u].x = __builtin_nontemporal_load(&src[i + u * stride].x);
      v[u].y = __builtin_nontemporal_load(&src[i + u * stride].y);
    }
#pragma unroll
    for (int u = 0; u < U; ++u) {
      __builtin_nontemporal_store(v[u].x, &dst[i + u * stride].x);
      __builtin_nontemporal_store(v[u].y, &dst[i + u * stride].y);
    }
  }
  for (; i < n2; i += stride) dst[i] = src[i];
}

__global__ __launch_bounds__(kBlock) void stream_read_kernel(
    size_t n2, const double2* __restrict__ src, double* __restrict__ sink) {
  constexpr int U = 8;
  const size_t stride = static_cast<size_t>(gridDim.x) * blockDim.x;
  size_t i = static_cast<size_t>(blockIdx.x) * blockDim.x + threadIdx.x;
  double acc = 0.0;
  for (; i + (U - 1) * stride < n2; i += U * stride) {
    double2 v[U];
#pragma unroll
    for (int u = 0; u < U; ++u) v[u] = src[i + u * stride];
#pragma unroll
    for (int u = 0; u < U; ++u) acc += v[u].x + v[u].y;
  }
  for (; i < n2; i += stride) acc += src[i].x + src[i].y;
  if (acc == 12345.678) sink[0] = acc;
}

extern "C" int flow_profile_stream_copy(size_t n, const double* src, double* dst,
                                        void* stream) {
  FLOW_REQUIRE(n >= 2 && n % 2 == 0 && src != nullptr, "stream copy arguments");
  FLOW_REQUIRE(reinterpret_cast<uintptr_t>(src) % 16 == 0 &&
                   reinterpret_cast<uintptr_t>(dst) % 16 == 0 && dst != nullptr,
               "stream copy: 16-byte aligned buffers");
  hipLaunchKernelGGL(stream_copy_kernel, dim3(8192), dim3(kBlock), 0,
                     as_stream(stream), n / 2,
                     reinterpret_cast<const double2*>(src),
                     reinterpret_cast<double2*>(dst));
  FLOW_CHECK_LAUNCH();
  return FLOW_OK;
}

extern "C" int flow_profile_stream_read(size_t n, const double* src, double* sink,
                                        void* stream) {
  FLOW_REQUIRE(n >= 2 && n % 2 == 0 && src != nullptr && sink != nullptr,
// ... 503 lines not shown
    case 1: CALL(1); break;      \
    case 2: CALL(2); break;      \
    case 3: CALL(3); break;      \
    case 4: CALL(4); break;      \
    case 5: CALL(5); break;      \
    case 6: CALL(6); break;      \
    case 7: CALL(7); break;      \
    default: CALL(8); break;     \
  }

static int gmres_combine(int N, int nv, const double* c, double cw,
                         const double* w, const double* V, double* out,
                         double* nn_partial, bool accumulate, hipStream_t st) {
  const int g = grid_for(N, kBlock, kRedBlocks);
  if (nv == 0) {
    FLOW_REQUIRE(w != nullptr, "gmres combine");
    Coef8 none = {};
    hipLaunchKernelGGL(gmres_combine_kernel<1>, dim3(g), dim3(kBlock), 0, st, N,
                       none, cw, 1, w, V, static_cast<size_t>(N), out,
                       nn_partial);
  }
  for (int k0 = 0; k0 < nv; k0 += 8) {
    const int chunk = nv - k0 < 8 ? nv - k0 : 8;
    Coef8 coef = {};
    for (int k = 0; k < chunk; ++k) coef.c[k] = c[k0 + k];
    double* nnp = (k0 + 8 >= nv) ? nn_partial : nullptr;
#define FLOW_CALL(NV)                                                          \
  hipLaunchKernelGGL(gmres_combine_kernel<NV>, dim3(g), dim3(kBlock), 0, st, N, \
                     coef, cw, (k0 == 0 && !accumulate) ? 1 : 0, w,            \
                     V + static_cast<size_t>(k0) * N, static_cast<size_t>(N),  \
                     out, nnp)
    FLOW_NV_SWITCH(chunk, FLOW_CALL)
#undef FLOW_CALL
  }
  FLOW_CHECK_LAUNCH();
  return FLOW_OK;
}

static int gmres_combine_dev(int N, int nv, const double* coef, const double* cw,
                             const double* w, const double* V, double* out,
                             double* nn_partial, bool accumulate,
                             const double* stop, hipStream_t st) {
  const int g = grid_for(N, kBlock, kRedBlocks);
  for (int k0 = 0; k0 < nv; k0 += 8) {
    const int chunk = nv - k0 < 8 ? nv - k0 : 8;
    double* nnp = (k0 + 8 >= nv) ? nn_partial : nullptr;
#define FLOW_CALL(NV)                                                           \
  hipLaunchKernelGGL(gmres_combine_dev_kernel<NV>, dim3(g), dim3(kBlock), 0, st, \
                     N, coef + k0, cw, (k0 == 0 && !accumulate) ? 1 : 0, w,     \
                     V + static_cast<size_t>(k0) * N, static_cast<size_t>(N),   \
                     out, nnp, stop)
    FLOW_NV_SWITCH(chunk, FLOW_CALL)
#undef FLOW_CALL
  }
  FLOW_CHECK_LAUNCH();
  return FLOW_OK;
}

static double gmres_least_squares(const double (*H)[kGmresMax + 1], int j,
                                  double beta, double* y) {
  double R[kGmresMax][kGmresMax + 1];
  double g[kGmresMax + 1];
  double cs[kGmresMax], sn[kGmresMax];
  g[0] = beta;
  for (int c = 0; c < j; ++c) {
    for (int r = 0; r <= c + 1; ++r) R[c][r] = H[c][r];
    for (int i = 0; i < c; ++i) {
      const double t = cs[i] * R[c][i] + sn[i] * R[c][i + 1];
      R[c][i + 1] = -sn[i] * R[c][i] + cs[i] * R[c][i + 1];
      R[c][i] = t;
    }
    const double d = hypot(R[c][c], R[c][c + 1]);
    cs[c] = d > 0.0 ? R[c][c] / d : 1.0;
    sn[c] = d > 0.0 ? R[c][c + 1] / d : 0.0;
    R[c][c] = d;
    g[c + 1] = -sn[c] * g[c];
    g[c] = cs[c] * g[c];
  }
  for (int i = j - 1; i >= 0; --i) {
    double t = g[i];
    for (int c = i + 1; c < j; ++c) t -= R[c][i] * y[c];
    y[i] = R[i][i] != 0.0 ? t / R[i][i] : 0.0;
  }
  return fabs(g[j]);
}

static int gmres(const flow_operator* A, const double* dinv, const flow_ilu* ilu,
                 const flow_pmg* pmg, const double* b, double* x, double rtol,
                 double atol, int maxit, int m, int x_is_zero, int expected,
                 int verify, double* work, int* iters_host, double* resid_host,
                 hipStream_t st) {
  const int N = op_size(A);
  double* partial = work;
  double* S = work + 3 * kRedBlocks;
  double* V = work + FLOW_REDUCE_WORK;
  double* Z = V + static_cast<size_t>(m + 1) * N;
  double* iwork = Z + static_cast<size_t>(m) * N;
  double* P = iwork + N;
  double* Pww = P + kGmresMax * kRedBlocks;
  double* Pnn = Pww + kRedBlocks;
  double* G = P + FLOW_GMRES_PARTIALS;
  const double* stop = S + kDone;
  const int gv = grid_for(N);
  const int gd = grid_for(N, kBlock, kRedBlocks);
  int np = 0, rc;

  const double* jprm = nullptr;
  const bool precond = pmg || ilu || dinv;
  const double* Zbase = precond ? Z : V;
  auto precondition = [&](int j) -> int {
    const double* in = V + static_cast<size_t>(j) * N;
    double* out = Z + static_cast<size_t>(j) * N;
    if (pmg) return pmg_apply(pmg, in, out, st, stop);
    if (ilu) return ilu_apply(ilu, in, out, iwork, st, stop);
    if (dinv)
      hipLaunchKernelGGL(vmul_kernel, dim3(gv), dim3(kBlock), 0, st, N, 1.0, dinv,
                         in, out, stop);
    return FLOW_OK;
  };
  auto arnoldi = [&](int j, double beta, double target, bool last) -> int {
    int r;
    double* w = V + static_cast<size_t>(j + 1) * N;
    if ((r = precondition(j))) return r;
    if ((r = apply(A, Zbase + static_cast<size_t>(j) * N, w, st, nullptr, stop, 0,
                   0, jprm)))
      return r;
    for (int k0 = 0; k0 <= j; k0 += 8) {
      const int chunk = j + 1 - k0 < 8 ? j + 1 - k0 : 8;
#define FLOW_CALL(NV)                                                         \
  hipLaunchKernelGGL(gmres_dots_kernel<NV>, dim3(gd), dim3(kBlock), 0, st, N,  \
                     w, V + static_cast<size_t>(k0) * N,                      \
                     static_cast<size_t>(N), k0 == 0 ? 1 : 0,                 \
                     P + k0 * kRedBlocks, Pww, stop)
      FLOW_NV_SWITCH(chunk, FLOW_CALL)
#undef FLOW_CALL
    }
    hipLaunchKernelGGL(gmres_step_kernel, dim3(1), dim3(kBlock), 0, st, gd, j,
                       last ? 1 : 0, beta, target, P, G, S);
    FLOW_CHECK_LAUNCH();
    if (!last &&
        (r = gmres_combine_dev(N, j + 1, G + kGCoef, G + kGCw, w, V, w, Pnn, false,
                               stop, st)))
      return r;
    return FLOW_OK;
  };

  const bool replay = replay_wanted(N, kReplayGmres);
  KeyHash base;
  if (replay) {
    base.pod(0x676dull);
    key_operator(base, A, true);
    base.pod(dinv).obj(ilu).obj(ilu ? ilu->plan : nullptr).obj(pmg);
    base.pod(work).pod(N).pod(m);
    if (A->kind == 3) {
      jprm = G + kGJvp;
      if ((rc = momentum_jvp_params(
               static_cast<const flow_momentum_jvp*>(A->matfree), G + kGJvp, st)))
        return rc;
    }
  }
  auto arnoldi_replayed = [&](int j, bool last) -> int {
    if (!replay) return arnoldi(j, -1.0, 0.0, last);
    KeyHash key = base;
    key.pod(j).pod(last);
    hipGraphExec_t graph = nullptr;
    int nodes = 0, r;
    if ((r = replay_prepare(key.h, kReplayGmres, st,
                            [&]() { return arnoldi(j, -1.0, 0.0, last); }, &graph,
                            &nodes)))
      return r;
    return graph ? replay_launch(graph, nodes, st) : arnoldi(j, -1.0, 0.0, last);
  };

  if ((rc = fill(kNumSlots, 0.0, S, st))) return rc;
  double resid = 0.0;
  int it = 0;
  bool first = true;
  bool claimed = false;
  double state[kNumSlots];
  while (true) {
    const bool b_is_r0 = x_is_zero && it == 0;
    if (b_is_r0) {
      hipLaunchKernelGGL(axpby_kernel, dim3(gv), dim3(kBlock), 0, st, N, 1.0, b,
                         0.0, V);
    } else {
      if ((rc = apply(A, x, iwork, st))) return rc;
      hipLaunchKernelGGL(residual_kernel, dim3(gv), dim3(kBlock), 0, st, N, b,
                         iwork,
                         static_cast<const double*>(nullptr), V,
                         static_cast<double*>(nullptr));
    }
    const int have_b2 = first && !b_is_r0;
    if ((rc = dots(N, have_b2 ? 2 : 1, V, V, b, b, V, V, partial, &np, st)))
      return rc;
    hipLaunchKernelGGL(gmres_begin_kernel, dim3(1), dim3(kBlock), 0, st, np,
                       have_b2, first ? 1 : 0, claimed ? 1 : 0, rtol, atol,
                       partial, S);
    if (have_b2)
      hipLaunchKernelGGL(gmres_drop_start_kernel, dim3(gv), dim3(kBlock), 0, st,
                         N, S, b, V, x);
    FLOW_CHECK_LAUNCH();
    first = false;
    claimed = false;
    if (it >= maxit) {
      if ((rc = read_state(S, state, st))) return rc;
      resid = state[kBeta];
      if (state[kDone] == 4.0) break;
      *iters_host = it;
      *resid_host = resid;
      if (state[kDone] == 2.0) {
        set_error("GMRES broke down (NaN residual) at iteration %d", it);
      } else {
        set_error("GMRES did not converge in %d iterations: |r| = %.3e > %.3e",
                  it, resid, state[kTarget2]);
      }
      return FLOW_NOT_CONVERGED;
    }

    const int it0 = it;
    int enq = 0, cols = 0;
    bool converged = false, start_passes = false;
    while (true) {
      const int room = (m < maxit - it0 ? m : maxit - it0) - enq;
      if (room <= 0) break;
      int plan = expected - (it0 + enq);
      if (plan < 1) plan = 1;
      if (plan > room) plan = room;
      for (int k = 0; k < plan; ++k, ++enq) {
        const bool last = enq + 1 >= m || it0 + enq + 1 >= maxit;
        if ((rc = arnoldi_replayed(enq, last))) return rc;
      }
      if ((rc = read_state(S, state, st))) return rc;
      cols = static_cast<int>(state[kConvIt]);
      if (state[kDone] == 2.0) {
        *iters_host = it0 + cols;
        *resid_host = state[kRes2];
        set_error("GMRES broke down (NaN) at iteration %d", it0 + cols);
        return FLOW_NOT_CONVERGED;
      }
      resid = state[kRes2];
      if (state[kDone] == 4.0) {
        start_passes = true;
        break;
      }
      if (state[kDone] != 0.0) {
        converged = state[kDone] == 1.0;
        break;
      }
    }
    if (start_passes) break;
    it = it0 + (cols > 0 ? cols : 1);
    if ((rc = fill(1, 0.0, S + kDone, st))) return rc;
    if (cols > 0 &&
        (rc = gmres_combine_dev(N, cols, G + kGYc, nullptr, nullptr, Zbase, x,
                                nullptr, true, nullptr, st)))
      return rc;
    x_is_zero = 0;
    if (converged && !verify) break;
    claimed = converged;
  }
  *iters_host = it;
  *resid_host = resid;
  return FLOW_OK;
}

static int check_solver_args(const flow_operator* A, const double* b,
                             const double* x, double rtol, double atol,
                             int maxit, int check_every, int first_check,
                             const double* work, size_t work_len, size_t nvec,
                             const int* iters_host, const double* resid_host) {
  int rc = check_operator(A);
  if (rc) return rc;
  FLOW_REQUIRE(b && x && work && iters_host && resid_host, "solver pointers");
  FLOW_REQUIRE(rtol >= 0.0 && atol >= 0.0 && maxit >= 0 && check_every > 0 &&
                   first_check >= 0,
               "solver tolerances");
  FLOW_REQUIRE(work_len >= FLOW_REDUCE_WORK + nvec * (size_t)op_size(A),
               "solver workspace too small");
  return FLOW_OK;
}

extern "C" int flow_cg_solve(const flow_operator* A, const double* dinv,
                             const flow_coarse* coarse, const flow_mg* mg,
                             const double* b,
                             double* x, double rtol, double atol, int maxit,
                             int check_every, int first_check, double* work,
                             size_t work_len, int* iters_host,
                             double* resid_host, void* stream) {
  int rc = check_solver_args(A, b, x, rtol, atol, maxit, check_every,
                             first_check, work, work_len, 5, iters_host,
                             resid_host);
  if (rc) return rc;
  FLOW_REQUIRE(A->kind != 3, "CG: assembled (symmetric) operators only");
  if (coarse) {
    FLOW_REQUIRE(dinv != nullptr, "two-level preconditioner needs dinv");
    FLOW_REQUIRE(A->kind == 0, "two-level preconditioner: scalar operators");
    if ((rc = check_coarse(coarse, A->n))) return rc;
  }
  if (mg) {
    FLOW_REQUIRE(coarse == nullptr, "multigrid and two-level are exclusive");
    FLOW_REQUIRE(dinv != nullptr && A->kind == 0,
                 "multigrid preconditioner: scalar operators with dinv");
    if ((rc = check_mg(mg, A->n))) return rc;
    FLOW_REQUIRE(mg->nlevels >= 2, "multigrid: at least two levels");
  }
  FLOW_REQUIRE(work_len >= cg_work_len(A, coarse, mg),
               "solver workspace too small (FLOW_REDUCE_WORK + 5 N + SpMV "
               "workgroups + 2 [+ 2 lda] [+ 2 mg->Ps[0].nblocks])");
  FLOW_REQUIRE(reinterpret_cast<uintptr_t>(work) % 16 == 0,
               "solver workspace must be 16-byte aligned");
  return cg(A, dinv, coarse, mg, b, x, rtol, atol, maxit, check_every,
            first_check, work, iters_host, resid_host, as_stream(stream));
}

extern "C" int flow_cg_solve_guarded(
    const flow_operator* A, const double* dinv, const flow_coarse* coarse,
    const flow_mg* mg, const double* b, double* x, const double* x_fallback,
    double rtol, double atol, int maxit, int check_every, int first_check,
    double* work, size_t work_len, int* iters_host, double* resid_host,
    int* starts_dropped_host, void* stream) {
  FLOW_REQUIRE(starts_dropped_host != nullptr, "starts_dropped_host is NULL");
  *starts_dropped_host = 0;
  int rc = check_solver_args(A, b, x, rtol, atol, maxit, check_every,
                             first_check, work, work_len, 5, iters_host,
                             resid_host);
  if (rc) return rc;
  FLOW_REQUIRE(A->kind != 3, "CG: assembled (symmetric) operators only");
  if (coarse) {
    FLOW_REQUIRE(dinv != nullptr, "two-level preconditioner needs dinv");
    FLOW_REQUIRE(A->kind == 0, "two-level preconditioner: scalar operators");
    if ((rc = check_coarse(coarse, A->n))) return rc;
  }
  if (mg) {
    FLOW_REQUIRE(coarse == nullptr, "multigrid and two-level are exclusive");
    FLOW_REQUIRE(dinv != nullptr && A->kind == 0,
                 "multigrid preconditioner: scalar operators with dinv");
    if ((rc = check_mg(mg, A->n))) return rc;
    FLOW_REQUIRE(mg->nlevels >= 2, "multigrid: at least two levels");
  }
  FLOW_REQUIRE(work_len >= cg_work_len(A, coarse, mg),
               "solver workspace too small");
  FLOW_REQUIRE(reinterpret_cast<uintptr_t>(work) % 16 == 0,
               "solver workspace must be 16-byte aligned");
  FLOW_REQUIRE(x_fallback != x, "the fallback start must not alias x");
  hipStream_t st = as_stream(stream);
  const int N = op_size(A);
  bool rejected = false;
  rc = cg(A, dinv, coarse, mg, b, x, rtol, atol, maxit, check_every,
          first_check, work, iters_host, resid_host, st, &rejected);
  if (rc || !rejected) return rc;
  *starts_dropped_host = 1;
  if (x_fallback) {
    hipLaunchKernelGGL(axpby_kernel, dim3(grid_for(N)), dim3(kBlock), 0, st, N,
                       1.0, x_fallback, 0.0, x);
    FLOW_CHECK_LAUNCH();
    rc = cg(A, dinv, coarse, mg, b, x, rtol, atol, maxit, check_every, 0, work,
            iters_host, resid_host, st, &rejected);
    if (rc || !rejected) return rc;
    *starts_dropped_host = 2;
  }
  if ((rc = fill(N, 0.0, x, st))) return rc;
  return cg(A, dinv, coarse, mg, b, x, rtol, atol, maxit, check_every, 0, work,
            iters_host, resid_host, st);
}

extern "C" int flow_mg_apply(const flow_mg* mg, int n, const double* r,
                             double* z, void* stream) {
  FLOW_REQUIRE(mg && r && z && r != z && n > 0, "mg apply");
  int rc = check_mg(mg, n);
  if (rc) return rc;
  return vcycle(mg, r, z, as_stream(stream));
}

extern "C" int flow_two_level_apply(const flow_coarse* coarse,
                                    const double* dinv, const double* r,
                                    double* z, double* work, void* stream) {
  FLOW_REQUIRE(coarse && dinv && r && z && work && r != z, "two-level apply");
  int rc = check_coarse(coarse, coarse->n);
  if (rc) return rc;
  FLOW_REQUIRE(reinterpret_cast<uintptr_t>(work) % 16 == 0,
               "two-level workspace must be 16-byte aligned");
  return two_level(coarse, dinv, r, z, work, work + coarse->lda,
                   as_stream(stream));
}

extern "C" int flow_bicgstab_solve(const flow_operator* A, const double* dinv,
                                   const flow_ilu* ilu, const double* b,
                                   double* x, double rtol, double atol,
                                   int maxit, int check_every,
                                   int first_check, double* work,
                                   size_t work_len, int* iters_host,
                                   double* resid_host, void* stream) {
  int rc = check_solver_args(A, b, x, rtol, atol, maxit, check_every,
                             first_check, work, work_len, 7, iters_host,
                             resid_host);
  if (rc) return rc;
  if (ilu) {
    if ((rc = ilu_check(ilu, op_size(A)))) return rc;
    FLOW_REQUIRE(work_len >= FLOW_REDUCE_WORK + 8 * (size_t)op_size(A),
                 "solver workspace too small for the ILU sweep buffer");
  }
  return bicgstab(A, dinv, ilu, b, x, rtol, atol, maxit, check_every,
                  first_check, work, iters_host, resid_host, as_stream(stream));
}

extern "C" int flow_gmres_solve(const flow_operator* A, const double* dinv,
                                const flow_ilu* ilu, const flow_pmg* pmg,
                                const double* b, double* x,
                                double rtol, double atol, int maxit, int restart,
                                int x_is_zero, int expected_its, int verify,
                                double* work, size_t work_len, int* iters_host,
                                double* resid_host, void* stream) {
  int rc = check_solver_args(A, b, x, rtol, atol, maxit, 1, 0, work, work_len, 0,
                             iters_host, resid_host);
  if (rc) return rc;
  FLOW_REQUIRE(restart >= 1 && restart <= FLOW_GMRES_MAX_RESTART,
               "GMRES restart length");
  FLOW_REQUIRE(expected_its >= 0, "expected iterations");
  FLOW_REQUIRE(work_len >= FLOW_REDUCE_WORK +
                               (2 * static_cast<size_t>(restart) + 2) *
                                   op_size(A) +
                               FLOW_GMRES_PARTIALS + FLOW_GMRES_STATE,
               "solver workspace too small (FLOW_REDUCE_WORK + (2 restart + 2) N "
               "+ FLOW_GMRES_PARTIALS + FLOW_GMRES_STATE)");
  FLOW_REQUIRE(!(ilu && pmg), "one preconditioner: ilu or pmg");
  if (ilu && (rc = ilu_check(ilu, op_size(A)))) return rc;
  if (pmg && (rc = pmg_check(pmg, op_size(A)))) return rc;
  return gmres(A, dinv, ilu, pmg, b, x, rtol, atol, maxit, restart, x_is_zero,
               expected_its, verify, work, iters_host, resid_host,
               as_stream(stream));
}


namespace flow {

int check_comm(const flow_comm* c, long long need) {
  FLOW_REQUIRE(c != nullptr && c->allreduce != nullptr && c->buf != nullptr,
               "communicator");
  FLOW_REQUIRE(c->world >= 1 && c->world <= kNumSlots && c->rank >= 0 &&
                   c->rank < c->world,
               "communicator rank / world (at most 16 ranks)");
  FLOW_REQUIRE(c->capacity >= need, "exchange buffer too small");
  FLOW_REQUIRE(reinterpret_cast<uintptr_t>(c->buf) % 16 == 0,
               "exchange buffer must be 16-byte aligned");
  return FLOW_OK;
}

int check_rows(const flow_rows* R) {
  FLOW_REQUIRE(R != nullptr, "row ranges are NULL");
  FLOW_REQUIRE(0 <= R->e0 && R->e0 <= R->r0 && R->r0 < R->r1 && R->r1 <= R->e1 &&
                   R->e1 <= R->n,
               "row ranges");
  FLOW_REQUIRE(R->nhalo >= 0, "halo size");
  for (int i = 0; i < 2; ++i) {
    FLOW_REQUIRE(R->send_len[i] >= 0 && R->recv_len[i] >= 0, "halo lengths");
    FLOW_REQUIRE(R->send_len[i] == 0 ||
                     (R->send_row[i] >= R->r0 &&
                      R->send_row[i] + R->send_len[i] <= R->r1 &&
                      R->send_slot[i] >= 0 &&
                      R->send_slot[i] + R->send_len[i] <= R->nhalo),
                 "halo send range");
    FLOW_REQUIRE(R->recv_len[i] == 0 ||
                     (R->recv_row[i] >= R->e0 &&
                      R->recv_row[i] + R->recv_len[i] <= R->e1 &&
                      (R->recv_row[i] + R->recv_len[i] <= R->r0 ||
                       R->recv_row[i] >= R->r1) &&
                      R->recv_slot[i] >= 0 &&
                      R->recv_slot[i] + R->recv_len[i] <= R->nhalo),
                 "halo receive range");
  }
  return FLOW_OK;
}

int exchange(const flow_comm* c, int count) {
  const int rc = c->allreduce(c->user, count);
  if (rc != 0) {
    set_error("the all-reduce callback failed (code %d, %d doubles)", rc, count);
    return FLOW_HIP_ERROR;
  }
  return FLOW_OK;
// ... 1090 lines not shown
```

flow_amd/fem/ops.py:

```python
import ctypes

import numpy
import torch

from . import reference
from .function import (
    Function, Expression, Constant, as_cell_coefficient, cell_lattice_points,
    )
from .space import mesh_geometry_dev
from .. import _hip
from .. import device


def mesh_struct(mesh):
    if 'mesh_struct' not in mesh._cache:
        xy = mesh_geometry_dev(mesh)
        s = _hip.MeshS(mesh.num_cells(), _hip.f64(xy, 6 * mesh.num_cells(), 'xy'))
        mesh._cache['mesh_struct'] = (s, xy)
    return mesh._cache['mesh_struct'][0]


def space_struct(layout):
    if 'struct' not in layout._dev:
        nc = layout.mesh.num_cells()
        cd = layout.dev('cell_dofs')
        s = _hip.SpaceS(
            layout.degree, layout.N, layout.nnz,
            _hip.i32(cd, layout.nloc * nc, 'cell_dofs'),
            _hip.i32(layout.dev('cptr'), layout.nnz + 1, 'cptr'),
            _hip.i32(layout.dev('csrc'), layout.nloc**2 * nc, 'csrc'),
            _hip.i32(layout.dev('vptr'), layout.N + 1, 'vptr'),
            _hip.i32(layout.dev('vsrc'), layout.nloc * nc, 'vsrc'),
            )
        layout._dev['struct'] = s
    return layout._dev['struct']


_G_CACHE = {}


def coef_struct(coef, mesh, test_degree):
    key = (coef.k, test_degree, str(device.get()))
    if key not in _G_CACHE:
        _G_CACHE[key] = device.to_device(
            reference.source_matrix(coef.k, test_degree)
            )
    G = _G_CACHE[key]
    nce = mesh.num_cells() if coef.cell_stride else 1
    s = _hip.CoefS(
        coef.nl, coef.cell_stride,
        _hip.f64(coef.values, coef.dim * coef.nl * nce, 'coefficient values'),
        _hip.f64(G, coef.nl * reference.nloc(test_degree), 'G'),
        )
    return s, (coef.values, G)


def scratch(mesh, ndoubles):
    buf = mesh._cache.get('scratch')
    if buf is None or buf.numel() < ndoubles:
        mesh._cache['scratch'] = None
        buf = device.empty(ndoubles)
        mesh._cache['scratch'] = buf
    if device._POISON:
        _hip.fill(buf, float('nan'))
    return buf


_WORK = {}


def work(ndoubles):
    key = str(device.get())
    buf = _WORK.get(key)
    if buf is None or buf.numel() < ndoubles:
        _WORK[key] = None
        buf = device.empty(ndoubles)
        _WORK[key] = buf
    return buf


def plane_stride(layout):
    return layout.nnz + (layout.nnz & 1)


def value_plane(layout):
    return device.zeros(plane_stride(layout))


class Matrix(object):
    NPLANES = {0: 1, 1: 2, 2: 4, 4: 1}

    def __init__(self, layout, kind, vals=None, rowmask=None):
        self.layout = layout
        self.kind = kind
        assert (rowmask is not None) == (kind == 4)
        if rowmask is not None:
            assert rowmask.dtype == torch.uint8 and \
                rowmask.numel() == 2 * layout.N
        self.rowmask = rowmask
        self.nplanes = self.NPLANES[kind]
        nnz = layout.nnz
        self.stride = plane_stride(layout)
        if vals is None:
            vals = device.zeros(self.nplanes * self.stride)
        elif vals.numel() == self.nplanes * nnz and self.stride != nnz:
            packed = device.zeros(self.nplanes * self.stride)
            for p in range(self.nplanes):
                packed[p * self.stride:p * self.stride + nnz] = \
                    vals[p * nnz:(p + 1) * nnz]
            vals = packed
        assert vals.numel() == self.nplanes * self.stride
        assert vals.data_ptr() % 16 == 0
        self.vals = vals
        self._op = None
        return

    @property
    def size(self):
        return self.layout.N * (1 if self.kind == 0 else 2)

    def plane(self, p):
        return self.vals[p * self.stride:p * self.stride + self.layout.nnz]

    def operator(self):
        if self._op is None:
            lay = self.layout
            op = _hip.Operator()
            op.kind = self.kind
            op.n = lay.N
            op.nnz = lay.nnz
            rb = lay.dev('rowblocks2' if self.kind in (2, 4) else 'rowblocks')
            op.nblocks = rb.numel() - 1
            op.rowptr = _hip.i32(lay.dev('rowptr'), lay.N + 1, 'rowptr')
            op.cols = _hip.i32(lay.dev('cols'), lay.nnz, 'cols')
            op.rowblocks = _hip.i32(rb, None, 'rowblocks')
            base = _hip.f64(self.vals, self.nplanes * self.stride, 'vals').value
            for p in range(self.nplanes):
                op.vals[p] = base + 8 * p * self.stride
            if self.rowmask is not None:
                op.rowmask = _hip.u8(self.rowmask, 2 * lay.N, 'rowmask').value
            self._op = op
        return self._op

    def apply(self, x, y):
        lib = _hip.lib()
        assert x.data_ptr() != y.data_ptr()
        _hip.check(lib.flow_operator_apply(
            ctypes.byref(self.operator()), _hip.f64(x, self.size, 'x'),
            _hip.f64(y, self.size, 'y'), _hip.stream()
            ))
        return y

    def diag_inv(self):
        lib = _hip.lib()
        out = device.empty(self.size)
        _hip.check(lib.flow_operator_diag_inv(
            ctypes.byref(self.operator()),
            _hip.i32(self.layout.dev('diag_idx'), self.layout.N, 'diag_idx'),
            _hip.f64(out), _hip.stream()
            ))
        return out

    def to_scipy(self):
        import scipy.sparse as sp
        lay = self.layout
        rp = lay.pattern('rowptr')
        cols = lay.pattern('cols')
        v = device.to_host(self.vals).numpy()
        nnz = lay.nnz
        st = self.stride
        P = [sp.csr_matrix((v[p * st:p * st + nnz], cols, rp),
                           shape=(lay.N, lay.N)) for p in range(self.nplanes)]
        if self.kind == 0:
            return P[0]
        if self.kind == 4:
            m = device.to_host(self.rowmask).numpy().astype(float)
            blocks = [
                sp.diags(m[c * lay.N:(c + 1) * lay.N]).dot(P[0])
                + sp.diags(1.0 - m[c * lay.N:(c + 1) * lay.N])
                for c in range(2)
                ]
            return sp.block_diag(blocks, format='csr')
        if self.kind == 1:
            return sp.block_diag(P, format='csr')
        return sp.bmat([[P[0], P[1]], [P[2], P[3]]], format='csr')


class MomentumJacobian(object):
    kind = 3

    def __init__(self, W, bfmask, ui, prm, bc_dofs, mesh_s=None, space_s=None):
        mesh = W.mesh()
        self.layout = W.layout
        self.size = W.size()
        n2 = self.size
        nc = mesh.num_cells()
        if mesh_s is None:
            mesh_s = mesh_struct(mesh)
        if space_s is None:
            space_s = space_struct(W.layout)
        self._keep = (bfmask, ui, bc_dofs,
                      device.empty(2 * W.layout.nloc * nc), mesh_s, space_s)
        self.struct = _hip.MomentumJvp(
            ctypes.pointer(mesh_s),
            ctypes.pointer(space_s),
            _hip.i32(bfmask, nc, 'bfmask'), _hip.f64(ui, n2, 'ui'), prm,
            _hip.f64(self._keep[3]), int(bc_dofs.numel()),
            _hip.i32(bc_dofs) if bc_dofs.numel() else None,
            self._bc_mask(bc_dofs),
            )
        op = _hip.Operator()
        op.kind = 3
        op.n = W.layout.N
        op.matfree = ctypes.cast(ctypes.pointer(self.struct), ctypes.c_void_p)
        self._op = op

    def operator(self):
        return self._op

    def _bc_mask(self, bc_dofs):
        if not bc_dofs.numel():
            return None
        held = getattr(self, '_mask', None)
        stamp = (bc_dofs.data_ptr(), bc_dofs.numel(), bc_dofs._version)
        if held is None or held[0] is not bc_dofs or held[2] != stamp:
            mask = torch.zeros(self.size, dtype=torch.uint8,
                               device=bc_dofs.device)
            mask[bc_dofs.long()] = 1
            device.synchronize()
            self._mask = held = (bc_dofs, mask, stamp)
        return _hip.u8(held[1], self.size, 'bc_mask')

    def rebind(self, bfmask, ui, prm, bc_dofs):
        nc = self.layout.mesh.num_cells()
        self._keep = (bfmask, ui, bc_dofs) + self._keep[3:]
        s = self.struct
        s.bfmask = _hip.i32(bfmask, nc, 'bfmask')
        s.ui = _hip.f64(ui, self.size, 'ui')
        s.prm = prm
        s.nbc = int(bc_dofs.numel())
        s.bc_dofs = _hip.i32(bc_dofs) if bc_dofs.numel() else None
        s.bc_mask = self._bc_mask(bc_dofs)
        return self

    @classmethod
    def cached(cls, W, bfmask, ui, prm, bc_dofs, mesh_s=None, space_s=None):
        key = ('jvp_operator', id(mesh_s), id(space_s))
        held = W.layout._dev.get(key)
        if held is None:
            held = cls(W, bfmask, ui, prm, bc_dofs, mesh_s, space_s)
            W.layout._dev[key] = held
            return held
        return held.rebind(bfmask, ui, prm, bc_dofs)

    def apply(self, x, y):
        lib = _hip.lib()
        assert x.data_ptr() != y.data_ptr()
        _hip.check(lib.flow_momentum_jvp_apply(
            ctypes.byref(self.struct), _hip.f64(x, self.size, 'x'),
            _hip.f64(y, self.size, 'y'), _hip.stream()
            ))
        return y


STIFFNESS, MASS, LUMPED_MASS = 0, 1, 2


def assemble_scalar_matrix(layout, kind):
    key = ('matrix', kind)
    if key not in layout._dev:
        lib = _hip.lib()
        mesh = layout.mesh
        A = Matrix(layout, 0)
        buf = scratch(mesh, layout.nloc**2 * mesh.num_cells())
        _hip.check(lib.flow_assemble_scalar_matrix(
            kind, ctypes.byref(mesh_struct(mesh)),
            ctypes.byref(space_struct(layout)), _hip.f64(buf),
            _hip.f64(A.vals), _hip.stream()
            ))
        layout._dev[key] = A
    return layout._dev[key]


def assemble_mass(V):
    return assemble_scalar_matrix(V.layout, MASS)


def assemble_stiffness(V):
    return assemble_scalar_matrix(V.layout, STIFFNESS)


def symmetric_bc_matrix(A, isbc):
    lib = _hip.lib()
    lay = A.layout
    out = Matrix(lay, 0)
    _hip.check(lib.flow_bc_symmetric_matrix(
        lay.N, _hip.i32(lay.dev('rowptr')), _hip.i32(lay.dev('cols')),
        _hip.f64(A.vals, lay.nnz), _hip.u8(isbc, lay.N, 'isbc'),
        _hip.f64(out.vals, lay.nnz), _hip.stream()
        ))
    return out


class CoarseSpace(object):

    def __init__(self, A, isbc=None, singular=False, target_nc=4096):
        import scipy.sparse as sp
        lay = A.layout
        n = lay.N
        assert A.kind == 0
        isbc = numpy.zeros(n, dtype=bool) if isbc is None else \
            numpy.asarray(isbc, dtype=bool)
        x = lay.dof_coords
        h = numpy.sqrt(2.0 * lay.mesh.cell_areas().mean())
        nfree = int(n - isbc.sum())
        s = max(2.0, numpy.sqrt(max(nfree, 1) / float(target_nc)))
        while True:
            ix = numpy.floor((x[:, 0] - x[:, 0].min()) / (s * h) + 1e-9)
            iy = numpy.floor((x[:, 1] - x[:, 1].min()) / (s * h) + 1e-9)
            key = (ix * 2000003 + iy).astype(numpy.int64)
            key[isbc] = -1
            ukey, agg = numpy.unique(key, return_inverse=True)
            if len(ukey) and ukey[0] == -1:
                agg = agg - 1
                nc = len(ukey) - 1
            else:
                nc = len(ukey)
            if nc <= 1.25 * target_nc or s > 1.0e6:
                break
            s *= 1.1
        assert nc >= 1
        self.s = s
        self.nc = nc
        self.n = n
        free = numpy.nonzero(agg >= 0)[0]
        Pm = sp.csr_matrix(
            (numpy.ones(len(free)), (free, agg[free])), shape=(n, nc)
            )
        Ah = A.to_scipy()
        Ac = (Pm.T.dot(Ah).dot(Pm)).toarray()
        if singular:
            e = numpy.ones(nc)
            beta = numpy.trace(Ac) / nc
            Ainv = numpy.linalg.inv(Ac + beta * numpy.outer(e, e) / nc) \
                - numpy.outer(e, e) / (beta * nc)
        else:
            Ainv = numpy.linalg.inv(Ac)
        Ainv = 0.5 * (Ainv + Ainv.T)
        order = numpy.argsort(agg[free], kind='stable')
        agg_dofs = free[order].astype(numpy.int32)
        agg_ptr = numpy.zeros(nc + 1, dtype=numpy.int64)
        numpy.cumsum(numpy.bincount(agg[free], minlength=nc), out=agg_ptr[1:])
        self.agg_of_host = agg.astype(numpy.int32)
        lda = (nc + 3) // 4 * 4
        A32 = numpy.zeros((nc, lda), dtype=numpy.float32)
        A32[:, :nc] = Ainv
        self._keep = (
            device.to_device(agg_ptr.astype(numpy.int32)),
            device.to_device(agg_dofs),
            device.to_device(self.agg_of_host),
            device.to_device(A32),
            )
        k = self._keep
        self.struct = _hip.CoarseS(
            n, nc, _hip.i32(k[0], nc + 1), _hip.i32(k[1], len(agg_dofs)),
            _hip.i32(k[2], n), lda, _hip.f32(k[3], nc * lda)
            )


def vector_norm(x, kind='l2'):
    lib = _hip.lib()
    code = {'l2': 0, 'linf': 1}[kind]
    res = ctypes.c_double(0.0)
    _hip.check(lib.flow_norm_host(
        x.numel(), _hip.f64(x), code, _hip.f64(work(_hip.REDUCE_WORK)),
        ctypes.byref(res), _hip.stream()
        ))
    return res.value


def dot(x, y):
    lib = _hip.lib()
    assert x.numel() == y.numel()
    res = ctypes.c_double(0.0)
    _hip.check(lib.flow_dot_host(
        x.numel(), _hip.f64(x), _hip.f64(y), _hip.f64(work(_hip.REDUCE_WORK)),
        ctypes.byref(res), _hip.stream()
        ))
    return res.value


def axpby(a, x, b, y):
    lib = _hip.lib()
    assert x.numel() == y.numel()
    _hip.check(lib.flow_axpby(
        x.numel(), float(a), _hip.f64(x), float(b), _hip.f64(y), _hip.stream()
        ))
    return y


copy = _hip.copy
fill = _hip.fill


def vmul(x, y, out=None, a=1.0):
    lib = _hip.lib()
    assert x.numel() == y.numel()
    if out is None:
        out = device.empty(x.numel())
    _hip.check(lib.flow_vmul(
# ... 457 lines not shown
```

flow_amd/fem/space.py:

```python
import numpy

from . import reference

SPMV_ROWS_PER_BLOCK = 256
SPMV_NNZ_PER_BLOCK = 1022


class ScalarLayout(object):

    def __init__(self, mesh, degree):
        assert degree in (1, 2)
        self.mesh = mesh
        self.degree = degree
        self.nloc = reference.nloc(degree)
        nv = mesh.num_vertices()
        if degree == 1:
            self.N = nv
            self.cell_dofs = mesh.cell_vertices.copy()
            self.vertex_dofs = numpy.arange(nv, dtype=numpy.int32)
            self.edge_dofs = None
            self.dof_coords = mesh.points.copy()
        else:
            edges = mesh.edges.astype(numpy.int64)
            ne = len(edges)
            vkey = numpy.arange(nv, dtype=numpy.int64) * (nv + 1)
            ekey = edges[:, 0] * (nv + 1) + 1 + edges[:, 1]
            order = numpy.argsort(numpy.concatenate([vkey, ekey]))
            rank = numpy.empty(nv + ne, dtype=numpy.int32)
            rank[order] = numpy.arange(nv + ne, dtype=numpy.int32)
            self.N = nv + ne
            self.vertex_dofs = rank[:nv]
            self.edge_dofs = rank[nv:]
            self.cell_dofs = numpy.concatenate([
                self.vertex_dofs[mesh.cell_vertices],
                self.edge_dofs[mesh.cell_edges],
                ], axis=1).astype(numpy.int32)
            coords = numpy.empty((self.N, 2))
            coords[self.vertex_dofs] = mesh.points
            coords[self.edge_dofs] = 0.5 * (
                mesh.points[edges[:, 0]] + mesh.points[edges[:, 1]]
                )
            self.dof_coords = coords
        self.cell_dofs = numpy.ascontiguousarray(self.cell_dofs)
        self._pattern = None
        self._vmap = None
        self._dev = {}
        return

    def _build_pattern(self):
        nloc = self.nloc
        nc = len(self.cell_dofs)
        cd = self.cell_dofs.astype(numpy.int64)
        key = (cd[:, :, None] * self.N + cd[:, None, :]).ravel()
        order = numpy.argsort(key, kind='stable')
        skey = key[order]
        del key
        new = numpy.empty(len(skey), dtype=bool)
        new[0] = True
        numpy.not_equal(skey[1:], skey[:-1], out=new[1:])
        first = numpy.nonzero(new)[0]
        ukey = skey[first]
        del skey, new
        rows = ukey // self.N
        cols = (ukey % self.N).astype(numpy.int32)
        nnz = len(ukey)
        rowptr = numpy.zeros(self.N + 1, dtype=numpy.int64)
        numpy.cumsum(numpy.bincount(rows, minlength=self.N), out=rowptr[1:])
        cptr = numpy.concatenate([first, [len(order)]]).astype(numpy.int32)
        csrc = ((order % (nloc * nloc)) * nc + order // (nloc * nloc)).astype(
            numpy.int32
            )
        assert nloc * nloc * nc < 2**31
        is_diag = cols == rows
        diag_idx = numpy.nonzero(is_diag)[0].astype(numpy.int32)
        assert len(diag_idx) == self.N
        self._pattern = {
            'rowptr': rowptr.astype(numpy.int32),
            'cols': cols,
            'nnz': nnz,
            'cptr': cptr,
            'csrc': csrc,
            'diag_idx': diag_idx,
            'rowblocks': csr_stream_rowblocks(rowptr),
            'rowblocks2': csr_stream_rowblocks(
                rowptr, nnz_per_block=SPMV_NNZ_PER_BLOCK),
            }
        return

    def pattern(self, name):
        if self._pattern is None:
            self._build_pattern()
        return self._pattern[name]

    @property
    def nnz(self):
        return self.pattern('nnz')

    def _build_vmap(self):
        nc = len(self.cell_dofs)
        flat = self.cell_dofs.ravel()
        order = numpy.argsort(flat, kind='stable')
        vptr = numpy.zeros(self.N + 1, dtype=numpy.int64)
        numpy.cumsum(numpy.bincount(flat, minlength=self.N), out=vptr[1:])
        vsrc = ((order % self.nloc) * nc + order // self.nloc).astype(
            numpy.int32
            )
        self._vmap = {'vptr': vptr.astype(numpy.int32), 'vsrc': vsrc}
        return

    def vmap(self, name):
        if self._vmap is None:
            self._build_vmap()
        return self._vmap[name]

    def dev(self, name):
        from .. import device
        if name not in self._dev:
            if name == 'cell_dofs':
                arr = numpy.ascontiguousarray(self.cell_dofs.T)
            elif name in ('vptr', 'vsrc'):
                arr = self.vmap(name)
            else:
                arr = self.pattern(name)
            if name == 'cols':
                arr = numpy.concatenate([arr, numpy.zeros(4, dtype=arr.dtype)])
            self._dev[name] = device.to_device(arr)
        return self._dev[name]


def csr_stream_rowblocks(rowptr, rows_per_block=SPMV_ROWS_PER_BLOCK,
                         nnz_per_block=None):
    if nnz_per_block is None:
        from .. import _hip
        try:
            nnz_per_block = _hip.spmv_tile_nnz(0)
        except (OSError, _hip.HipError):
            nnz_per_block = _hip.SPMV_NNZ_PER_BLOCK
    rowptrs = rowptr if isinstance(rowptr, (list, tuple)) else [rowptr]
    rowptrs = [numpy.asarray(rp, dtype=numpy.int64) for rp in rowptrs]
    n = len(rowptrs[0]) - 1
    for rp in rowptrs:
        assert len(rp) == n + 1
        if n > 0:
            assert (rp[1:] - rp[:-1]).max() <= nnz_per_block, \
                'row longer than the CSR-stream LDS tile'
    blocks = [0]
    r = 0
    while r < n:
        r_next = min(r + rows_per_block, n)
        for rp in rowptrs:
            r_nnz = int(numpy.searchsorted(
                rp, rp[r] + nnz_per_block, side='right')) - 1
            r_next = min(r_next, r_nnz)
        assert r_next > r
        blocks.append(r_next)
        r = r_next
    return numpy.array(blocks, dtype=numpy.int32)


def mesh_geometry_dev(mesh):
    from .. import device
    if 'geom_dev' not in mesh._cache:
        p = mesh.points[mesh.cell_vertices]
        xy = numpy.ascontiguousarray(p.transpose(2, 1, 0))
        mesh._cache['geom_dev'] = device.to_device(xy)
    return mesh._cache['geom_dev']


def scalar_layout(mesh, degree):
    key = ('layout', degree)
    if key not in mesh._cache:
        mesh._cache[key] = ScalarLayout(mesh, degree)
    return mesh._cache[key]


class FunctionSpace(object):

    def __new__(cls, mesh, family='CG', *args, **kwargs):
        if isinstance(family, MixedElement):
            return MixedFunctionSpace(mesh, family)
        return super(FunctionSpace, cls).__new__(cls)

    def __init__(self, mesh, family='CG', degree=1, dim=1, _component=None,
                 _parent=None):
        if isinstance(family, FiniteElement):
            degree = family.degree()
            dim = family.dim
            family = family.family
        assert family in ('CG', 'Lagrange', 'P'), family
        assert dim in (1, 2)
        self._mesh = mesh
        self.degree = degree
        self.dim = dim
        self.layout = scalar_layout(mesh, degree)
        self.component = _component
        self.parent = _parent
        return

    def mesh(self):
        return self._mesh

    @property
    def N(self):
        return self.layout.N

    def size(self):
        return self.dim * self.layout.N

    def dim_(self):
        return self.size()

    def num_sub_spaces(self):
        return self.dim if self.dim > 1 else 0

    def sub(self, i):
        assert self.dim == 2 and i in (0, 1)
        return FunctionSpace(
            self._mesh, 'CG', self.degree, dim=1, _component=i, _parent=self
            )

    def collapse(self):
        return FunctionSpace(self._mesh, 'CG', self.degree, dim=1)

    def ufl_element(self):
        return FiniteElement('Lagrange', 'triangle', self.degree, self.dim)

    def tabulate_dof_coordinates(self):
        c = self.layout.dof_coords
        return numpy.concatenate([c] * self.dim) if self.dim > 1 else c

    def same_as(self, other):
        return (
            self._mesh is other._mesh and self.degree == other.degree
            and self.dim == other.dim
            )


class FiniteElement(object):
    def __init__(self, family, cell, degree, dim=1):
        self.family = family
        self.cell = cell
        self._degree = degree
        self.dim = dim

    def degree(self):
        return self._degree

    def __mul__(self, other):
        return MixedElement([self, other])


class MixedElement(object):
    def __init__(self, elements):
        self.elements = list(elements)


class MixedFunctionSpace(object):

    def __init__(self, mesh, element):
        self._mesh = mesh
        self.spaces = [FunctionSpace(mesh, e) for e in element.elements]

    def mesh(self):
        return self._mesh

    def sub(self, i):
        return self.spaces[i]

    def num_sub_spaces(self):
        return len(self.spaces)


def VectorElement(family, cell, degree):
    return FiniteElement(family, cell, degree, dim=2)


def VectorFunctionSpace(mesh, family, degree):
    return FunctionSpace(mesh, family, degree, dim=2)
```

flow_amd/navier_stokes/pressure_correction.py:

```python
from __future__ import print_function

import ctypes
import time

import numpy

from ..fem import ops
from ..fem.bcs import collect
from ..fem.function import Function, as_cell_coefficient, scalar_value
from ..message import Message, info
from .. import _hip
from .. import device
from .. import parallel
from . import start_vectors
from .start_vectors import (
    extrapolation_weights, forget_history,
    extrapolated_increment as _extrapolated_increment,
    remember_increment as _remember_increment,
    newton_key as _newton_key,
    )
from .newton_preconditioner import (
    age as _age, contraction as _contraction, choose_cycle as _choose_cycle,
    contraction_on_strips as _contraction_on_strips,
    coarse_jacobian as _coarse_jacobian, mass_share as _mass_share,
# ... 87 lines not shown
                                                         'chebyshev')
                == 'chebyshev'))


def _history(lay):
    hist = lay._dev.get('step_history')
    if hist is None or not _uses_history() or not hist.get('continuing'):
        return None
    return hist

last_step_info = {}

_THETA = {
    'forward euler': (0.0, 1.0),
    'backward euler': (1.0, 0.0),
    'crank-nicolson': (0.5, 0.5),
    }


def _persistent(lay, name, n):
    key = ('persistent', name)
    buf = lay._dev.get(key)
    if buf is None or buf.numel() != n:
        buf = lay._dev[key] = device.empty(n)
    return buf


def _zeros(n):
    return _hip.fill(device.empty(n), 0.0)


def _bc_arrays(bcs, size):
    dofs, vals = collect(bcs, size)
    hit = _BC_UPLOADS.get(id(vals))
    if hit is not None and hit[0] is vals and hit[1] is dofs:
        return hit[2]
    out = (
        dofs, device.to_device(dofs.astype(numpy.int32)),
        device.to_device(vals.astype(numpy.float64)),
        )
    if len(_BC_UPLOADS) >= 16:
        _BC_UPLOADS.clear()
    _BC_UPLOADS[id(vals)] = (vals, dofs, out)
    return out


_BC_UPLOADS = {}


def _mesh_s(mesh):
    return parallel.mesh_view(mesh) if parallel.active() \
        else ops.mesh_struct(mesh)


def _space_s(layout):
    return parallel.view(layout).space if parallel.active() \
        else ops.space_struct(layout)


def _bc_mask(dofs, n, comp=None):
    mask = numpy.zeros(n, dtype=numpy.uint8)
    if comp is None:
        mask[dofs] = 1
    else:
        sel = dofs[(dofs >= comp * n) & (dofs < (comp + 1) * n)] - comp * n
        mask[sel] = 1
    return mask


def _as_ilu(kind, pre):
    if kind == 'ilu0':
        return pre
    if kind == 'tlilu':
        return pre.front if getattr(pre, 'use_cycle', True) else pre.fine
    return None


class _Bare(object):

    def __init__(self, factors):
        self.factors = factors

    def apply(self, r, z):
        return self.factors.solve(r, z)


def _remainder_tolerance(lay, npar, lin_atol, nrm, tol):
    frac = npar.get('linear_remainder_fraction', 0.0)
    quad_c = lay._dev.get('newton_quad_C')
    if not frac or quad_c is None or not numpy.isfinite(quad_c):
        return lin_atol
    predicted = quad_c * nrm * nrm
    return max(lin_atol, min(frac * predicted,
                             npar.get('linear_atol_cap', 1.0e-4) * tol))


def _compute_tentative_velocity(
        u, p0, f, u_bcs, time_step_method, rho, mu, dt, v=None,
        tol=1.0e-10
        ):
    lib = _hip.lib()
    assert time_step_method in _THETA, time_step_method
    theta_i, theta_e = _THETA[time_step_method]
    alpha = 1.0
    if parallel.active():
        return _tentative_velocity_on_strips(
            u, p0, f, u_bcs, theta_i, theta_e, rho, mu, dt, tol), alpha
    W = u[0].function_space()
    P = p0.function_space()
    mesh = W.mesh()
    lay = W.layout
    nc = mesh.num_cells()
    n2 = W.size()

    ui = Function(W, ops.copy(
        _persistent(lay, 'newton_iterate', n2) if _hip.graphs_possible()
        else device.empty(n2), u[0].data))
    hist = _history(lay)
    candidates = ['u0']
    if hist is not None and 'ui' in hist and \
            solver_parameters['newton'].get('initial_guess') == 'best':
        settled = 'ui_prev' in hist and 0.7 <= dt / hist['dt'] <= 1.5
        if hist.get('countdown', 0) > 0 and (
                hist['winner'] != 'ux' or settled):
            hist['countdown'] -= 1
            candidates = [hist['winner']]
        else:
            candidates = ['u0', 'ui']
            if settled:
                candidates.append('ux')

    f0 = as_cell_coefficient(f[0], mesh, 2)
    f1 = as_cell_coefficient(f[1], mesh, 2)
    f0s, keep0 = ops.coef_struct(f0, mesh, lay.degree)
    f1s, keep1 = ops.coef_struct(f1, mesh, lay.degree)
    prm = _hip.NsParams(dt, rho, mu, theta_i, theta_e)
    bc_dofs_host, bc_dofs, bc_vals = _bc_arrays(u_bcs, n2)
    nbc = bc_dofs.numel()
    bfmask = mesh._cache.get('bfmask_dev')
    if bfmask is None:
        bfmask = device.to_device(mesh.cell_bfacet_mask())
        mesh._cache['bfmask_dev'] = bfmask

    J = lay._dev.get('jacobian')
    if J is None:
        J = ops.Matrix(lay, 2)
        lay._dev['jacobian'] = J
    F = device.empty(n2)
    dx = device.empty(n2)
    buf = ops.scratch(mesh, max(2 * lay.nloc, 4 * lay.nloc**2) * nc)
    ms = ops.mesh_struct(mesh)
    ws = ops.space_struct(lay)
    ps = ops.space_struct(P.layout)
    st = _hip.stream()
    npar = solver_parameters['newton']

    def assemble(want_f, want_j):
        _hip.check(lib.flow_assemble_momentum(
            ctypes.byref(ms), ctypes.byref(ws), ctypes.byref(ps),
            _hip.i32(bfmask, nc, 'bfmask'), _hip.f64(ui.data, n2),
            _hip.f64(u[0].data, n2), _hip.f64(p0.data, P.size()),
            ctypes.byref(f0s), ctypes.byref(f1s), ctypes.byref(prm),
            _hip.f64(buf), _hip.f64(F, n2) if want_f else None,
            _hip.f64(J.vals, 4 * J.stride) if want_j else None, J.stride, st
            ))

    def residual():
        assemble(True, False)
        _hip.check(lib.flow_bc_residual(
            nbc, _hip.i32(bc_dofs), _hip.f64(bc_vals), _hip.f64(ui.data),
            _hip.f64(F), st
            ))
        return ops.vector_norm(F)

    def load_candidate(name):
        ops.copy(ui.data, u[0].data if name == 'u0' else hist['ui'])
        if name == 'ux':
            r = dt / hist['dt']
            ops.axpby(r, hist['ui'], 1.0, ui.data)
            ops.axpby(-r, hist['ui_prev'], 1.0, ui.data)

    first_nrm = None
    if candidates != ['u0']:
        best = None
        for name in candidates:
            load_candidate(name)
            nrm_c = residual()
            score = 3.0 * nrm_c if name == 'ux' else nrm_c
            if best is None or score < best[3]:
                best = (name, nrm_c, _hip.clone(F) if len(candidates) > 1
                        else None, score)
        if len(candidates) > 1:
            hist['winner'] = best[0]
            hist['countdown'] = npar['guess_retry']
            if best[0] != candidates[-1]:
                load_candidate(best[0])
                ops.copy(F, best[2])
        first_nrm = best[1]
        last_step_info['initial_guess'] = best[0]

    history = []
    linear_its = []
    applications = []
    linear_residuals = []
    last_linear_residual = 0.0
    it = 0
    Jop = None
    finish = None
    by_total = npar.get('linear_history', 'increments') == 'total' and \
        npar.get('linear_solver', 'gmres') == 'gmres'
    total_pred = found = None
    loose_step = False
    while True:
        if first_nrm is not None:
            nrm, first_nrm = first_nrm, None
        else:
            nrm = residual()
        if nrm < tol and finish is not None and \
                npar.get('finish_loose_solves', True):
            info('Newton iteration %d passes against the prediction: its '
                 'linear solve is continued to the tight tolerance' % it)
            nrm, last_linear_residual = finish()
            linear_residuals[-1] = last_linear_residual
            last_step_info['newton_finished_loose_solves'] = \
                last_step_info.get('newton_finished_loose_solves', 0) + 1
        finish = None
        if history and history[-1] > 0.0:
            quad = numpy.sqrt(max(nrm**2 - last_linear_residual**2, 0.0))
            lay._dev['newton_quad_C'] = quad / history[-1]**2
        history.append(nrm)
        info('Newton iteration %d: r (abs) = %.3e (tol = %.3e)' % (it, nrm, tol))
        if nrm < tol:
            break
        if it >= npar['maximum_iterations'] or not numpy.isfinite(nrm):
            raise RuntimeError(
                'Newton solver did not converge after %d iterations '
                '(residual history %r)' % (it, history)
                )
        def assemble_jacobian():
            assemble(False, True)
            _hip.check(lib.flow_bc_identity_rows(
                ctypes.byref(J.operator()), _hip.f64(J.vals),
                _hip.i32(lay.dev('diag_idx')), nbc, _hip.i32(bc_dofs), st
                ))

        ops.fill(dx, 0.0)
        dx_is_zero = True
        hkey = _newton_key(it)
        extrapolate = npar.get('linear_start') == 'extrapolated'
        if extrapolate and by_total and it == 0:
            dx_is_zero = not _extrapolated_increment(
                lay, dt, dx, int(npar.get('linear_start_points', 5)),
                key='newton_total', degree=npar.get('linear_start_degree'))
            if not dx_is_zero:
                total_pred = ops.copy(_persistent(lay, 'newton_total_pred', n2),
                                      dx)
        elif extrapolate and by_total and loose_step and total_pred is not None:
            ops.copy(dx, total_pred)
            ops.axpby(-1.0, found, 1.0, dx)
            dx_is_zero = False
        elif hkey is not None and extrapolate:
            dx_is_zero = not _extrapolated_increment(
                lay, dt, dx, int(npar.get('linear_start_points', 5)),
                key=hkey, degree=npar.get('linear_start_degree'))
        pre = None
        kind = npar.get('preconditioner', 'jacobi')
        use_gmres = npar.get('linear_solver', 'gmres') == 'gmres'
        key = (rho, mu, theta_i, nbc, hash(bc_dofs_host.tobytes()))
        if kind == 'pmg':
            rej = lay._dev.get('pmg_rejected')
            if lay.degree != 2 or not use_gmres:
                kind = 'ilu0'
            elif rej is not None and rej[0] == key and dt > 0.5 * rej[1]:
                kind = npar.get('fallback', 'ilu0')
        if kind == 'tlilu' and (lay.degree != 2 or not use_gmres):
            kind = 'ilu0'
        with_ilu = kind in ('ilu0', 'pmg', 'tlilu')
        matfree = with_ilu and npar.get('matrix_free', True)
        if not matfree:
            assemble_jacobian()
        if matfree and Jop is None:
            Jop = ops.MomentumJacobian.cached(W, bfmask, ui.data, prm, bc_dofs)
        operator = Jop if matfree else J
        refactored = False

        def build(kind):
            from ..fem import ilu
            slot = {'ilu0': 'jacobian_ilu', 'pmg': 'jacobian_pmg',
                    'tlilu': 'jacobian_tl'}[kind]
            pre = lay._dev.get(slot)
            if not (pre is None or pre.key != key or pre.stale or (
                    it == 0 and not (1.0 / npar['ilu_lag'] <= dt / pre.dt
                                     <= npar['ilu_lag']))):
                return kind, pre, False
            if matfree:
                assemble_jacobian()
            lay._dev['newton_rebuilds'] = lay._dev.get('newton_rebuilds', 0) + 1
            last_step_info['newton_preconditioner_rebuilds'] = \
                lay._dev['newton_rebuilds']
            if kind == 'pmg':
                if pre is None:
                    from ..fem.pmg import Pmg
                    pre = Pmg(W, **npar.get('pmg', {}))
                    lay._dev[slot] = pre
                J1 = _coarse_jacobian(
                    pre, W, P, ui, p0, f0, f1, prm, bfmask, bc_dofs_host)
                pre.refactor(J, J1, mass_share=_mass_share(pre, J1)
                             if pre.coarse_auto else None)
                last_step_info['pmg_coarse_steps'] = pre.struct.coarse_steps
                pre.dt, pre.key, pre.stale = dt, key, False
                pre.contraction = _contraction(pre, operator, lay, bc_dofs_host)
                last_step_info['pmg_contraction'] = pre.contraction
                if not pre.contraction < npar.get('pmg_accept', 0.8):
                    lay._dev['pmg_rejected'] = (key, dt)
                    pre.stale = True
                    fallback = npar.get('fallback', 'ilu0')
                    info('p-multigrid rejected (contraction %.2f): %s'
                         % (pre.contraction, fallback))
# ... 764 lines not shown
```

include/flow_hip.h:

```cpp
#ifndef FLOW_HIP_H
#define FLOW_HIP_H

#include <stddef.h>

#ifdef __cplusplus
extern "C" {
#endif

#define FLOW_OK 0
#define FLOW_NOT_CONVERGED 1
#define FLOW_INVALID 2
#define FLOW_HIP_ERROR 3

#define FLOW_SPMV_ROWS_PER_BLOCK 256
#define FLOW_SPMV_NNZ_PER_BLOCK 1022
int flow_spmv_tile_nnz(int kind);

const char* flow_last_error(void);
int flow_abi_version(void);
int flow_launch_count(unsigned long long* count_host);
int flow_graph_mode(int mode, long long auto_rows);
int flow_graph_stats(unsigned long long* stats_host);
int flow_xcd_tile_host(int block, int nblocks);

// ... 270 lines not shown
  void* user;
  const flow_peer* peer;
} flow_comm;
int flow_peer_alloc(int land_cap, void** base_out, char* handle_out);
int flow_peer_open(const char* handle, void** base_out);
int flow_peer_close(void* mapped_base);
int flow_peer_free(void* base);
int flow_peer_status(const flow_peer* peer, unsigned long long* error_host,
                     void* stream);

#define FLOW_RCCL_ID_BYTES 128
typedef struct {
  void* comm;
  double* buf;
  void* stream;
} flow_rccl_binding;
int flow_rccl_load(const char* librccl_path);
int flow_rccl_unique_id(char* id_host);
int flow_rccl_comm_create(const char* id_host, int rank, int world,
                          void** comm_out);
int flow_rccl_comm_destroy(void* comm);
int flow_rccl_allreduce(void* user, int count);

typedef struct {
  int n;
  int r0, r1;
  int e0, e1;
  int nhalo;
  int send_row[2], send_len[2], send_slot[2];
  int recv_row[2], recv_len[2], recv_slot[2];
} flow_rows;

int flow_shard_halo(const flow_comm* comm, const flow_rows* rows, int ncomp,
                    double* x, int stride, void* stream);
int flow_shard_reduce_host(const flow_comm* comm, const flow_rows* rows,
                           int ncomp, const double* x, const double* y,
                           int stride, int kind, double* work,
                           double* result_host, void* stream);

int flow_shard_cg_solve(const flow_comm* comm, const flow_rows* rows,
                        const flow_operator* A, const double* dinv,
                        const double* b, double* x, double rtol, double atol,
                        int maxit, int check_every, int first_check,
                        double* work, size_t work_len, int* iters_host,
                        double* resid_host, int* start_rejected_host,
                        void* stream);

typedef struct {
  const flow_mg* mg;
  flow_operator Ah0, Ps0, Rg;
  flow_operator Cg;
  const int* up_rowblocks0;
  int up_nblocks0;
  int z_lo, z_hi;
} flow_mg_shard;
int flow_shard_mgcg_solve(const flow_comm* comm, const flow_rows* rows,
                          const flow_operator* A, const double* dinv,
                          const flow_mg_shard* mgs, const double* b, double* x,
                          double rtol, double atol, int maxit, int check_every,
                          int first_check, double* work, size_t work_len,
                          int* iters_host, double* resid_host,
                          int* start_rejected_host, void* stream);

typedef struct {
  int nlevels;
  const int* rowblocks16[16];
  int nblocks16[16];
  int row_lo_last, row_hi_last;
} flow_mass_strips;
int flow_shard_mass_solve(const flow_comm* comm, const flow_rows* rows,
                          const flow_mass* M, const flow_mass_strips* levels,
                          const double* b, const double* xbase,
                          const double* delta0, double* x, double rtol,
                          double atol, int maxit, int first_check, double* work,
                          size_t work_len, int* iters_host, double* resid_host,
                          void* stream);

int flow_shard_gmres_solve(const flow_comm* comm, const flow_rows* rows,
                           const flow_operator* A, const flow_ilu* ilu,
                           const flow_pmg* pmg, const double* b, double* x,
                           double rtol, double atol,
                           int maxit, int restart, int x_is_zero,
                           int expected_its, int verify, double* work,
                           size_t work_len, int* iters_host, double* resid_host,
                           void* stream);

typedef struct {
  int nc;
  const double* xy;
  int c0, c1;
} flow_mesh;

typedef struct {
  int deg;
  int n;
  int nnz;
  const int* cell_dofs;
  const int* cptr;
  const int* csrc;
  const int* vptr;
  const int* vsrc;
  int r0, r1;
  int nnz0, nnz1;
} flow_space;

typedef struct {
  int nl;
  int cell_stride;
  const double* values;
  const double* G;
} flow_coef;

int flow_assemble_scalar_matrix(int kind, const flow_mesh* mesh,
                                const flow_space* V, double* scratch,
                                double* vals, void* stream);

int flow_assemble_pressure_rhs(const flow_mesh* mesh, const flow_space* W,
                               const flow_space* P, const double* u,
                               const double* p0, double alpha_rho_dt, double mu,
                               int rotational, double* scratch, double* b,
                               void* stream);

int flow_assemble_correction_rhs(const flow_mesh* mesh, const flow_space* W,
                                 const flow_space* P, const double* u,
                                 const double* p1, const double* p0,
                                 double dt_rho, double mu, int rotational,
                                 double* scratch, double* b, void* stream);

typedef struct {
  double dt, rho, mu, theta_i, theta_e;
} flow_ns_params;
int flow_assemble_momentum(const flow_mesh* mesh, const flow_space* W,
                           const flow_space* P, const int* bfmask,
                           const double* ui, const double* u0,
                           const double* p0, const flow_coef* f0,
                           const flow_coef* f1, const flow_ns_params* prm,
                           double* scratch, double* F, double* Jvals,
                           size_t j_plane_stride, void* stream);

typedef struct {
  const flow_mesh* mesh;
  const flow_space* W;
  const int* bfmask;
  const double* ui;
  flow_ns_params prm;
  double* scratch;
  int nbc;
  const int* bc_dofs;
  const unsigned char* bc_mask;
} flow_momentum_jvp;
int flow_momentum_jvp_apply(const flow_momentum_jvp* J, const double* v,
                            double* out, void* stream);

int flow_assemble_source(const flow_mesh* mesh, const flow_space* V, int dim,
                         const flow_coef* f, double* scratch, double* b,
                         void* stream);

int flow_assemble_div_adjoint(const flow_mesh* mesh, const flow_space* W,
                              const flow_space* P, const double* p,
                              double* scratch, double* out, void* stream);

int flow_assemble_magnitude(const flow_mesh* mesh, const flow_space* W, int mode,
                            const double* u, double* scratch, double* b,
                            void* stream);

#define FLOW_FORM_MAX_PROGRAM 64
#define FLOW_FORM_REGISTERS 8
#define FLOW_FORM_MAX_CONSTANTS 32
#define FLOW_FORM_MAX_FIELDS 6
#define FLOW_FORM_MAX_EXPRESSIONS 4
#define FLOW_FORM_MAX_POINTS 256
#define FLOW_FORM_OP_CONST 0
#define FLOW_FORM_OP_COORD 1
#define FLOW_FORM_OP_FIELD 2
#define FLOW_FORM_OP_EXPR 3
#define FLOW_FORM_OP_MOV 4
#define FLOW_FORM_OP_ADD 5
#define FLOW_FORM_OP_SUB 6
#define FLOW_FORM_OP_MUL 7
#define FLOW_FORM_OP_DIV 8
#define FLOW_FORM_OP_POW 9
#define FLOW_FORM_OP_NEG 10
#define FLOW_FORM_OP_ABS 11
#define FLOW_FORM_OP_SQRT 12
#define FLOW_FORM_OP_EXP 13
#define FLOW_FORM_OP_LN 14
#define FLOW_FORM_OP_SIN 15
#define FLOW_FORM_OP_COS 16
#define FLOW_FORM_OP_OUT 17
#define FLOW_FORM_OP_NORMAL 18
typedef struct {
  int nprog;
  int prog[4 * FLOW_FORM_MAX_PROGRAM];
  int nconst;
  double consts[FLOW_FORM_MAX_CONSTANTS];
  int nfield;
  const double* field[FLOW_FORM_MAX_FIELDS];
  int field_deg[FLOW_FORM_MAX_FIELDS];
  const int* cell_dofs[2];
  int nexpr;
  const double* expr[FLOW_FORM_MAX_EXPRESSIONS];
  int expr_nl[FLOW_FORM_MAX_EXPRESSIONS];
  int expr_table[FLOW_FORM_MAX_EXPRESSIONS];
  int nq;
  const double* rule;
  const double* tables;
  int ntables;
  int nout;
} flow_form;

int flow_form_functional(const flow_mesh* mesh, const flow_form* form,
                         double* scratch, double* work, double* result_host,
                         void* stream);

int flow_form_facet_functional(const flow_mesh* mesh, const flow_form* form,
                               int nfacets, const int* facet_cell,
                               const int* facet_local, double* scratch,
                               double* work, double* result_host, void* stream);

int flow_form_load_vector(const flow_mesh* mesh, const flow_space* V,
                          const flow_form* form, double* scratch, double* b,
                          void* stream);

typedef struct {
  int nx, ny;
  double x0, y0;
  double hx_inv, hy_inv;
  const int* start;
  const int* cells;
} flow_point_grid;

int flow_locate_points(const flow_mesh* mesh, const flow_point_grid* grid, int n,
                       const double* xy, int* cell, double* bary, void* stream);

int flow_form_points(const flow_mesh* mesh, const flow_form* form, int n,
                     const int* cell, const double* bary, double* out,
                     void* stream);

int flow_bc_identity_rows(const flow_operator* A, double* vals_planes,
                          const int* diag_idx, int nbc, const int* dofs,
                          void* stream);
int flow_bc_residual(int nbc, const int* dofs, const double* g, const double* u,
                     double* F, void* stream);
int flow_bc_set_values(int nbc, const int* dofs, const double* g, double* x,
                       void* stream);
int flow_bc_symmetric_matrix(int n, const int* rowptr, const int* cols,
                             const double* vals_in, const unsigned char* isbc,
                             double* vals_out, void* stream);

int flow_assemble_heat(const flow_mesh* mesh, const flow_space* Q,
                       const flow_space* W, const double* conv, double kappa,
                       double rho_cp, int supg, double* scratch, double* Avals,
                       double* Msupg_vals, double* tau_out, int* status_dev,
                       void* stream);

int flow_assemble_heat_supg_source(const flow_mesh* mesh, const flow_space* Q,
                                   const flow_space* W, const double* conv,
                                   double kappa, double rho_cp,
                                   const flow_coef* source, double* scratch,
                                   double* b, int* status_dev, void* stream);

#ifdef __cplusplus
}
#endif
#endif
```

Measured before the change: 127.2.

## Tile momentum residual and JVP by spatial cell boxes with LDS scatter-gather

Cells are grouped into spatial tiles of at most 512 cells, built on the host from centroid boxes. Each block computes per-cell momentum residual or Jacobian-vector contributions into shared memory and directly sums the rows owned entirely by that tile. Only boundary-row contributions go to a compact global scratch buffer for a separate row gather. This aims to cut global scratch write/read traffic and the full-size gather pass, at the cost of host preprocessing, extra index arrays, and a large LDS footprint per block that may limit occupancy.

```diff
diff --git a/flow_amd/_hip.py b/flow_amd/_hip.py
--- a/flow_amd/_hip.py
+++ b/flow_amd/_hip.py
@@ -303,6 +303,36 @@
         ('nbc', ctypes.c_int),
         ('bc_dofs', ctypes.c_void_p),
         ('bc_mask', ctypes.c_void_p),
+        ]
+
+
+TILE_CELLS = 512
+
+
+class CellTiles(ctypes.Structure):
+    _fields_ = [
+        ('ntiles', ctypes.c_int),
+        ('nc', ctypes.c_int),
+        ('n', ctypes.c_int),
+        ('nbnd', ctypes.c_int),
+        ('nbrows', ctypes.c_int),
+        ('cell_ptr', ctypes.c_void_p),
+        ('cells', ctypes.c_void_p),
+        ('cell_bnd', ctypes.c_void_p),
+        ('row_ptr', ctypes.c_void_p),
+        ('rows', ctypes.c_void_p),
+        ('ent_ptr', ctypes.c_void_p),
+        ('slots', ctypes.c_void_p),
+        ('brows', ctypes.c_void_p),
+        ('bptr', ctypes.c_void_p),
+        ('bsrc', ctypes.c_void_p),
+        ]
+
+
+class MomentumJvpTiled(ctypes.Structure):
+    _fields_ = [
+        ('J', ctypes.POINTER(MomentumJvp)),
+        ('tiles', ctypes.POINTER(CellTiles)),
         ]
 
 
@@ -402,6 +432,10 @@
                                _VP, _P(CoefS), _P(CoefS), _P(NsParams), _VP,
                                _VP, _VP, ctypes.c_size_t, _VP],
     'flow_momentum_jvp_apply': [_P(MomentumJvp), _VP, _VP, _VP],
+    'flow_momentum_jvp_tiled_apply': [_P(MomentumJvpTiled), _VP, _VP, _VP],
+    'flow_assemble_momentum_residual_tiled': [
+        _P(MeshS), _P(SpaceS), _P(SpaceS), _P(CellTiles), _VP, _VP, _VP, _VP,
+        _P(CoefS), _P(CoefS), _P(NsParams), _VP, _VP, _VP],
     'flow_assemble_source': [_P(MeshS), _P(SpaceS), _I, _P(CoefS), _VP, _VP,
                              _VP],
     'flow_assemble_magnitude': [_P(MeshS), _P(SpaceS), _I, _VP, _VP, _VP, _VP],
diff --git a/flow_amd/csrc/assembly_kernels.hip b/flow_amd/csrc/assembly_kernels.hip
--- a/flow_amd/csrc/assembly_kernels.hip
+++ b/flow_amd/csrc/assembly_kernels.hip
@@ -3,6 +3,29 @@
 #include "fem_device.h"
 
 namespace flow {
+
+template <int NP>
+__device__ __forceinline__ void fold_list(int a, int b, const int* __restrict__ src,
+                                          const double* __restrict__ scratch,
+                                          size_t plane_stride, double s[NP]) {
+#pragma unroll
+  for (int p = 0; p < NP; ++p) s[p] = 0.0;
+  for (int t = a; t < b; t += 4) {
+    int idx[4];
+#pragma unroll
+    for (int j = 0; j < 4; ++j) idx[j] = t + j < b ? src[t + j] : -1;
+    double w[NP][4];
+#pragma unroll
+    for (int p = 0; p < NP; ++p)
+#pragma unroll
+      for (int j = 0; j < 4; ++j)
+        w[p][j] = idx[j] >= 0 ? scratch[p * plane_stride + idx[j]] : 0.0;
+#pragma unroll
+    for (int p = 0; p < NP; ++p)
+#pragma unroll
+      for (int j = 0; j < 4; ++j) s[p] += w[p][j];
+  }
+}
 
 template <int NP>
 __global__ __launch_bounds__(kBlock) void gather_kernel(
@@ -14,26 +37,8 @@
   if (stopped(stop)) return;
   for (int k = blockIdx.x * blockDim.x + threadIdx.x; k < nout;
        k += gridDim.x * blockDim.x) {
-    const int a = ptr[k];
-    const int b = ptr[k + 1];
     double s[NP];
-#pragma unroll
-    for (int p = 0; p < NP; ++p) s[p] = 0.0;
-    for (int t = a; t < b; t += 4) {
-      int idx[4];
-#pragma unroll
-      for (int j = 0; j < 4; ++j) idx[j] = t + j < b ? src[t + j] : -1;
-      double w[NP][4];
-#pragma unroll
-      for (int p = 0; p < NP; ++p)
-#pragma unroll
-        for (int j = 0; j < 4; ++j)
-          w[p][j] = idx[j] >= 0 ? scratch[p * plane_stride + idx[j]] : 0.0;
-#pragma unroll
-      for (int p = 0; p < NP; ++p)
-#pragma unroll
-        for (int j = 0; j < 4; ++j) s[p] += w[p][j];
-    }
+    fold_list<NP>(ptr[k], ptr[k + 1], src, scratch, plane_stride, s);
     if (idrow) {
 #pragma unroll
       for (int p = 0; p < NP; ++p)
@@ -41,6 +46,29 @@
     }
 #pragma unroll
     for (int p = 0; p < NP; ++p) out[static_cast<size_t>(p) * out_stride + k] = s[p];
+  }
+}
+
+template <int NP>
+__global__ __launch_bounds__(kBlock) void gather_rows_kernel(
+    int nrows, const int* __restrict__ rows, const int* __restrict__ ptr,
+    const int* __restrict__ src, const double* __restrict__ scratch,
+    size_t plane_stride, size_t out_stride, double* __restrict__ out,
+    const double* __restrict__ stop, const unsigned char* __restrict__ idrow,
+    size_t id_stride, const double* __restrict__ v, size_t v_stride) {
+  if (stopped(stop)) return;
+  for (int k = blockIdx.x * blockDim.x + threadIdx.x; k < nrows;
+       k += gridDim.x * blockDim.x) {
+    const int row = rows[k];
+    double s[NP];
+    fold_list<NP>(ptr[k], ptr[k + 1], src, scratch, plane_stride, s);
+    if (idrow) {
+#pragma unroll
+      for (int p = 0; p < NP; ++p)
+        if (idrow[p * id_stride + row]) s[p] = v[p * v_stride + row];
+    }
+#pragma unroll
+    for (int p = 0; p < NP; ++p) out[static_cast<size_t>(p) * out_stride + row] = s[p];
   }
 }
 
@@ -316,6 +344,57 @@
 }
 
 template <int DEG>
+__device__ __forceinline__ void residual_cell(
+    int nc, const double* __restrict__ xy, const int* __restrict__ cdu, int nu,
+    const int* __restrict__ cdp, const int* __restrict__ bfmask,
+    const double* __restrict__ ui, const double* __restrict__ u0,
+    const double* __restrict__ p0, const flow_coef& f0, const flow_coef& f1,
+    const flow_ns_params& prm, int c, double acc[2][Elem<DEG>::NL]) {
+  constexpr int NL = Elem<DEG>::NL;
+  constexpr int NQ = Elem<DEG>::NQ;
+  const Geom g = load_geom(xy, nc, c);
+  double Ui[2][NL], U0[2][NL], P[3];
+  load_local<NL>(ui, nu, cdu, nc, c, 2, Ui);
+  load_local<NL>(u0, nu, cdu, nc, c, 2, U0);
+#pragma unroll
+  for (int k = 0; k < 3; ++k) P[k] = p0[cdp[k * nc + c]];
+  const int mask = bfmask[c];
+  const double ci = -prm.dt / prm.rho * prm.theta_i;
+  const double cexp = -prm.dt / prm.rho * prm.theta_e;
+#pragma unroll
+  for (int a = 0; a < 2; ++a)
+#pragma unroll
+    for (int i = 0; i < NL; ++i) acc[a][i] = 0.0;
+
+#pragma unroll
+  for (int q = 0; q < NQ; ++q) {
+    const double L[3] = {qpoint<DEG>(q, 0), qpoint<DEG>(q, 1), qpoint<DEG>(q, 2)};
+    const double w = 0.5 * qweight<DEG>(q) * g.adet;
+    double phi[NL], dphi[NL][3], gphi[NL][2];
+    basis<DEG>(L, phi, dphi);
+    phys_grad<NL>(g, dphi, gphi);
+#pragma unroll
+    for (int a = 0; a < 2; ++a) {
+      double du = 0.0;
+#pragma unroll
+      for (int j = 0; j < NL; ++j) du += (Ui[a][j] - U0[a][j]) * phi[j];
+#pragma unroll
+      for (int i = 0; i < NL; ++i) acc[a][i] += w * du * phi[i];
+    }
+    if (ci != 0.0)
+      add_rhs_weak_point<NL>(w * ci, prm.rho, prm.mu, Ui, P, L, phi, gphi, acc);
+    if (cexp != 0.0)
+      add_rhs_weak_point<NL>(w * cexp, prm.rho, prm.mu, U0, P, L, phi, gphi, acc);
+  }
+  if (mask) {
+    if (ci != 0.0) add_rhs_weak_facets<DEG>(mask, ci, prm.mu, g, Ui, P, acc);
+    if (cexp != 0.0) add_rhs_weak_facets<DEG>(mask, cexp, prm.mu, g, U0, P, acc);
+  }
+  if (ci != 0.0) add_source<NL>(f1, nc, c, 2, ci * g.adet, acc);
+  if (cexp != 0.0) add_source<NL>(f0, nc, c, 2, cexp * g.adet, acc);
+}
+
+template <int DEG>
 __global__ __launch_bounds__(kBlock) void momentum_residual_kernel(
     int nc, int cb, int ce, const double* __restrict__ xy, const int* __restrict__ cdu, int nu,
     const int* __restrict__ cdp, const int* __restrict__ bfmask,
@@ -323,19 +402,52 @@
     const double* __restrict__ p0, flow_coef f0, flow_coef f1,
     flow_ns_params prm, double* __restrict__ scratch) {
   constexpr int NL = Elem<DEG>::NL;
-  constexpr int NQ = Elem<DEG>::NQ;
   const int c = cb + xcd_tile(blockIdx.x, gridDim.x) * blockDim.x + threadIdx.x;
   if (c >= ce) return;
+  double acc[2][NL];
+  residual_cell<DEG>(nc, xy, cdu, nu, cdp, bfmask, ui, u0, p0, f0, f1, prm, c,
+                     acc);
+#pragma unroll
+  for (int a = 0; a < 2; ++a)
+#pragma unroll
+    for (int i = 0; i < NL; ++i)
+      scratch[static_cast<size_t>(a * NL + i) * nc + c] = acc[a][i];
+}
+
+template <int DEG>
+struct ResidualCell {
+  int nc;
+  const double* xy;
+  const int* cdu;
+  int nu;
+  const int* cdp;
+  const int* bfmask;
+  const double *ui, *u0, *p0;
+  flow_coef f0, f1;
+  flow_ns_params prm;
+  __device__ __forceinline__ void operator()(int c, double acc[2][Elem<DEG>::NL]) const {
+    residual_cell<DEG>(nc, xy, cdu, nu, cdp, bfmask, ui, u0, p0, f0, f1, prm, c,
+                       acc);
+  }
+};
+
+template <int DEG>
+__device__ __forceinline__ void jvp_cell(
+    int nc, const double* __restrict__ xy, const int* __restrict__ cdu, int nu,
+    int nv, const int* __restrict__ bfmask, const double* __restrict__ ui,
+    const double* __restrict__ v, const flow_ns_params& prm,
+    const double* __restrict__ prm_dev, int c, double acc[2][Elem<DEG>::NL]) {
+  constexpr int NL = Elem<DEG>::NL;
+  constexpr int NQ = Elem<DEG>::NQ;
   const Geom g = load_geom(xy, nc, c);
-  double Ui[2][NL], U0[2][NL], P[3];
-  load_local<NL>(ui, nu, cdu, nc, c, 2, Ui);
-  load_local<NL>(u0, nu, cdu, nc, c, 2, U0);
-#pragma unroll
-  for (int k = 0; k < 3; ++k) P[k] = p0[cdp[k * nc + c]];
+  double U[2][NL], V[2][NL];
+  load_local<NL>(ui, nu, cdu, nc, c, 2, U);
+  load_local<NL>(v, nv, cdu, nc, c, 2, V);
   const int mask = bfmask[c];
-  const double ci = -prm.dt / prm.rho * prm.theta_i;
-  const double cexp = -prm.dt / prm.rho * prm.theta_e;
-  double acc[2][NL];
+  const double ci = prm_dev ? load_scalar(prm_dev)
+                            : -prm.dt / prm.rho * prm.theta_i;
+  const double hr = prm_dev ? load_scalar(prm_dev + 1) : 0.5 * prm.rho;
+  const double mu = prm_dev ? load_scalar(prm_dev + 2) : prm.mu;
 #pragma unroll
   for (int a = 0; a < 2; ++a)
 #pragma unroll
@@ -345,33 +457,40 @@
   for (int q = 0; q < NQ; ++q) {
     const double L[3] = {qpoint<DEG>(q, 0), qpoint<DEG>(q, 1), qpoint<DEG>(q, 2)};
     const double w = 0.5 * qweight<DEG>(q) * g.adet;
-    double phi[NL], dphi[NL][3], gphi[NL][2];
-    basis<DEG>(L, phi, dphi);
-    phys_grad<NL>(g, dphi, gphi);
+    double uq[2], vq[2], gu[2][2], gv[2][2];
 #pragma unroll
     for (int a = 0; a < 2; ++a) {
-      double du = 0.0;
-#pragma unroll
-      for (int j = 0; j < NL; ++j) du += (Ui[a][j] - U0[a][j]) * phi[j];
-#pragma unroll
-      for (int i = 0; i < NL; ++i) acc[a][i] += w * du * phi[i];
-    }
-    if (ci != 0.0)
-      add_rhs_weak_point<NL>(w * ci, prm.rho, prm.mu, Ui, P, L, phi, gphi, acc);
-    if (cexp != 0.0)
-      add_rhs_weak_point<NL>(w * cexp, prm.rho, prm.mu, U0, P, L, phi, gphi, acc);
-  }
-  if (mask) {
-    if (ci != 0.0) add_rhs_weak_facets<DEG>(mask, ci, prm.mu, g, Ui, P, acc);
-    if (cexp != 0.0) add_rhs_weak_facets<DEG>(mask, cexp, prm.mu, g, U0, P, acc);
-  }
-  if (ci != 0.0) add_source<NL>(f1, nc, c, 2, ci * g.adet, acc);
-  if (cexp != 0.0) add_source<NL>(f0, nc, c, 2, cexp * g.adet, acc);
-#pragma unroll
-  for (int a = 0; a < 2; ++a)
-#pragma unroll
-    for (int i = 0; i < NL; ++i)
-      scratch[static_cast<size_t>(a * NL + i) * nc + c] = acc[a][i];
+      uq[a] = eval_at<DEG>(U[a], L);
+      vq[a] = eval_at<DEG>(V[a], L);
+      double gur[3], gvr[3];
+      ref_gradient<DEG>(U[a], L, gur);
+      ref_gradient<DEG>(V[a], L, gvr);
+#pragma unroll
+      for (int d = 0; d < 2; ++d) {
+        gu[a][d] = gur[0] * g.gl[0][d] + gur[1] * g.gl[1][d] + gur[2] * g.gl[2][d];
+        gv[a][d] = gvr[0] * g.gl[0][d] + gvr[1] * g.gl[1][d] + gvr[2] * g.gl[2][d];
+      }
+    }
+#pragma unroll
+    for (int a = 0; a < 2; ++a) {
+      const double dconv = gv[a][0] * uq[0] + gv[a][1] * uq[1] +
+                           gu[a][0] * vq[0] + gu[a][1] * vq[1];
+      const double s0 = w * (vq[a] - ci * hr * dconv);
+      double S1[2];
+#pragma unroll
+      for (int d = 0; d < 2; ++d)
+        S1[d] = w * ci * (hr * (vq[d] * uq[a] + uq[d] * vq[a]) -
+                          mu * (gv[a][d] + gv[d][a]));
+      double T[3];
+#pragma unroll
+      for (int k = 0; k < 3; ++k) T[k] = g.gl[k][0] * S1[0] + g.gl[k][1] * S1[1];
+      test_accumulate<DEG>(L, s0, T, acc[a]);
+    }
+  }
+  if (mask && ci != 0.0) {
+    const double P0[3] = {0.0, 0.0, 0.0};
+    add_rhs_weak_facets<DEG>(mask, ci, mu, g, V, P0, acc);
+  }
 }
 
 template <int DEG>
@@ -383,68 +502,87 @@
     const double* __restrict__ prm_dev,
     double* __restrict__ scratch, const double* __restrict__ stop) {
   constexpr int NL = Elem<DEG>::NL;
-  constexpr int NQ = Elem<DEG>::NQ;
   if (stopped(stop)) return;
   const int c = cb + xcd_tile(blockIdx.x, gridDim.x) * blockDim.x + threadIdx.x;
   if (c >= ce) return;
-  const Geom g = load_geom(xy, nc, c);
-  double U[2][NL], V[2][NL];
-  load_local<NL>(ui, nu, cdu, nc, c, 2, U);
-  load_local<NL>(v, nv, cdu, nc, c, 2, V);
-  const int mask = bfmask[c];
-  const double ci = prm_dev ? load_scalar(prm_dev)
-                            : -prm.dt / prm.rho * prm.theta_i;
-  const double hr = prm_dev ? load_scalar(prm_dev + 1) : 0.5 * prm.rho;
-  const double mu = prm_dev ? load_scalar(prm_dev + 2) : prm.mu;
   double acc[2][NL];
-#pragma unroll
-  for (int a = 0; a < 2; ++a)
-#pragma unroll
-    for (int i = 0; i < NL; ++i) acc[a][i] = 0.0;
-
-#pragma unroll
-  for (int q = 0; q < NQ; ++q) {
-    const double L[3] = {qpoint<DEG>(q, 0), qpoint<DEG>(q, 1), qpoint<DEG>(q, 2)};
-    const double w = 0.5 * qweight<DEG>(q) * g.adet;
-    double uq[2], vq[2], gu[2][2], gv[2][2];
-#pragma unroll
-    for (int a = 0; a < 2; ++a) {
-      uq[a] = eval_at<DEG>(U[a], L);
-      vq[a] = eval_at<DEG>(V[a], L);
-      double gur[3], gvr[3];
-      ref_gradient<DEG>(U[a], L, gur);
-      ref_gradient<DEG>(V[a], L, gvr);
-#pragma unroll
-      for (int d = 0; d < 2; ++d) {
-        gu[a][d] = gur[0] * g.gl[0][d] + gur[1] * g.gl[1][d] + gur[2] * g.gl[2][d];
-        gv[a][d] = gvr[0] * g.gl[0][d] + gvr[1] * g.gl[1][d] + gvr[2] * g.gl[2][d];
-      }
-    }
-#pragma unroll
-    for (int a = 0; a < 2; ++a) {
-      const double dconv = gv[a][0] * uq[0] + gv[a][1] * uq[1] +
-                           gu[a][0] * vq[0] + gu[a][1] * vq[1];
-      const double s0 = w * (vq[a] - ci * hr * dconv);
-      double S1[2];
-#pragma unroll
-      for (int d = 0; d < 2; ++d)
-        S1[d] = w * ci * (hr * (vq[d] * uq[a] + uq[d] * vq[a]) -
-                          mu * (gv[a][d] + gv[d][a]));
-      double T[3];
-#pragma unroll
-      for (int k = 0; k < 3; ++k) T[k] = g.gl[k][0] * S1[0] + g.gl[k][1] * S1[1];
-      test_accumulate<DEG>(L, s0, T, acc[a]);
-    }
-  }
-  if (mask && ci != 0.0) {
-    const double P0[3] = {0.0, 0.0, 0.0};
-    add_rhs_weak_facets<DEG>(mask, ci, mu, g, V, P0, acc);
-  }
+  jvp_cell<DEG>(nc, xy, cdu, nu, nv, bfmask, ui, v, prm, prm_dev, c, acc);
 #pragma unroll
   for (int a = 0; a < 2; ++a)
 #pragma unroll
     for (int i = 0; i < NL; ++i)
       scratch[static_cast<size_t>(a * NL + i) * nc + c] = acc[a][i];
+}
+
+template <int DEG>
+struct JvpCell {
+  int nc;
+  const double* xy;
+  const int* cdu;
+  int nu, nv;
+  const int* bfmask;
+  const double *ui, *v;
+  flow_ns_params prm;
+  const double* prm_dev;
+  __device__ __forceinline__ void operator()(int c, double acc[2][Elem<DEG>::NL]) const {
+    jvp_cell<DEG>(nc, xy, cdu, nu, nv, bfmask, ui, v, prm, prm_dev, c, acc);
+  }
+};
+
+template <int DEG, class Cell, int WAVES, int UNROLL>
+__global__ __launch_bounds__(kBlock, WAVES) void tiled_cell_kernel(
+    Cell cell, flow_cell_tiles tp, double* __restrict__ bscr,
+    double* __restrict__ out, size_t out_stride,
+    const unsigned char* __restrict__ idrow, const double* __restrict__ v,
+    size_t v_stride, const double* __restrict__ stop) {
+  constexpr int NL = Elem<DEG>::NL;
+  constexpr int T = FLOW_TILE_CELLS;
+  __shared__ double lds[2 * NL * T];
+  if (stopped(stop)) return;
+  const int t = xcd_tile(blockIdx.x, gridDim.x);
+  const int k0 = tp.cell_ptr[t];
+  const int nk = tp.cell_ptr[t + 1] - k0;
+  const size_t nb = static_cast<size_t>(tp.nbnd);
+  static_assert(T % kBlock == 0, "tile of whole blocks");
+#pragma unroll UNROLL
+  for (int r = 0; r < T / kBlock; ++r) {
+    const int k = r * kBlock + threadIdx.x;
+    if (k >= nk) break;
+    double acc[2][NL];
+    cell(tp.cells[k0 + k], acc);
+#pragma unroll
+    for (int a = 0; a < 2; ++a)
+#pragma unroll
+      for (int i = 0; i < NL; ++i) lds[(a * NL + i) * T + k] = acc[a][i];
+    const unsigned bm = tp.cell_bnd[k0 + k];
+    const unsigned mask = bm >> 26;
+    size_t j = bm & ((1u << 26) - 1);
+#pragma unroll
+    for (int i = 0; i < NL; ++i)
+      if ((mask >> i) & 1) {
+        bscr[j] = acc[0][i];
+        bscr[nb + j] = acc[1][i];
+        ++j;
+      }
+  }
+  __syncthreads();
+  const int r1 = tp.row_ptr[t + 1];
+  for (int k = tp.row_ptr[t] + threadIdx.x; k < r1; k += kBlock) {
+    const int row = tp.rows[k];
+    const int e1 = tp.ent_ptr[k + 1];
+    double s0 = 0.0, s1 = 0.0;
+    for (int e = tp.ent_ptr[k]; e < e1; ++e) {
+      const int sl = tp.slots[e];
+      s0 += lds[sl];
+      s1 += lds[NL * T + sl];
+    }
+    if (idrow) {
+      if (idrow[row]) s0 = v[row];
+      if (idrow[tp.n + row]) s1 = v[v_stride + row];
+    }
+    out[row] = s0;
+    out[out_stride + row] = s1;
+  }
 }
 
 template <int DEG>
@@ -1254,6 +1392,117 @@
     FLOW_CHECK_LAUNCH();
   }
   return FLOW_OK;
+}
+
+static int tiles_check(const flow_cell_tiles* tp, const flow_mesh* mesh,
+                       const flow_space* W) {
+  FLOW_REQUIRE(tp != nullptr, "cell tiles are NULL");
+  FLOW_REQUIRE(tp->ntiles > 0 && tp->nbnd >= 0 && tp->nbrows >= 0 &&
+                   tp->cell_ptr && tp->cells && tp->cell_bnd && tp->row_ptr &&
+                   tp->rows && tp->ent_ptr && tp->slots,
+               "cell tiles");
+  FLOW_REQUIRE(tp->nbrows == 0 || (tp->brows && tp->bptr && tp->bsrc),
+               "cell tiles: boundary rows");
+  FLOW_REQUIRE(W->deg == 2, "cell tiles: P2 velocity spaces");
+  FLOW_REQUIRE(tp->nc == mesh->nc && tp->n == W->n,
+               "cell tiles of another mesh or space");
+  FLOW_REQUIRE(mesh->c1 <= 0 && W->r1 <= 0,
+               "cell tiles cover whole meshes: no cell or row ranges");
+  return FLOW_OK;
+}
+
+static int gather_tile_rows(const flow_cell_tiles* tp, const double* bscr,
+                            double* out, size_t os, hipStream_t st,
+                            const double* stop, const unsigned char* idrow,
+                            const double* v, size_t vs) {
+  if (tp->nbrows == 0) return FLOW_OK;
+  hipLaunchKernelGGL(gather_rows_kernel<2>,
+                     dim3(grid_for(tp->nbrows, kBlock, 1 << 20)), dim3(kBlock),
+                     0, st, tp->nbrows, tp->brows, tp->bptr, tp->bsrc, bscr,
+                     static_cast<size_t>(tp->nbnd), os, out, stop, idrow,
+                     static_cast<size_t>(tp->n), v, vs);
+  FLOW_CHECK_LAUNCH();
+  return FLOW_OK;
+}
+
+int flow::momentum_jvp_tiled_check(const flow_momentum_jvp_tiled* A) {
+  FLOW_REQUIRE(A != nullptr, "tiled matrix-free Jacobian is NULL");
+  int rc = momentum_jvp_check(A->J);
+  if (rc) return rc;
+  return tiles_check(A->tiles, A->J->mesh, A->J->W);
+}
+
+int flow::momentum_jvp_tiled_apply(const flow_momentum_jvp_tiled* A,
+                                   const double* v, double* out, hipStream_t st,
+                                   int v_stride, int out_stride,
+                                   const double* stop, const double* prm_dev) {
+  const flow_momentum_jvp* J = A->J;
+  static const bool pair = [] {
+    const char* e = getenv("FLOW_AMD_JVP_PAIR");
+    return e && e[0] == '1';
+  }();
+  if (pair)
+    return momentum_jvp_apply(J, v, out, st, v_stride, out_stride, stop, prm_dev);
+  const flow_mesh* mesh = J->mesh;
+  const flow_space* W = J->W;
+  const flow_cell_tiles* tp = A->tiles;
+  const int vs = v_stride ? v_stride : W->n;
+  const int os = out_stride ? out_stride : W->n;
+  const unsigned char* idrow = J->nbc > 0 ? J->bc_mask : nullptr;
+  const JvpCell<2> cell{mesh->nc, mesh->xy, W->cell_dofs, W->n, vs,
+                        J->bfmask, J->ui, v, J->prm, prm_dev};
+  hipLaunchKernelGGL((tiled_cell_kernel<2, JvpCell<2>, 3, FLOW_TILE_CELLS / kBlock>), dim3(tp->ntiles),
+                     dim3(kBlock), 0, st, cell, *tp, J->scratch, out,
+                     static_cast<size_t>(os), idrow, v, static_cast<size_t>(vs),
+                     stop);
+  FLOW_CHECK_LAUNCH();
+  int rc = gather_tile_rows(tp, J->scratch, out, os, st, stop, idrow, v, vs);
+  if (rc) return rc;
+  if (J->nbc > 0 && !J->bc_mask) {
+    hipLaunchKernelGGL(bc_copy_kernel, dim3(grid_for(J->nbc)), dim3(kBlock), 0,
+                       st, J->nbc, J->bc_dofs, W->n, 0, W->n, v, vs, out, os,
+                       stop);
+    FLOW_CHECK_LAUNCH();
+  }
+  return FLOW_OK;
+}
+
+extern "C" int flow_momentum_jvp_tiled_apply(const flow_momentum_jvp_tiled* A,
+                                             const double* v, double* out,
+                                             void* stream) {
+  int rc = momentum_jvp_tiled_check(A);
+  if (rc) return rc;
+  FLOW_REQUIRE(v && out && v != out, "jvp vectors");
+  return momentum_jvp_tiled_apply(A, v, out, as_stream(stream), 0, 0, nullptr);
+}
+
+extern "C" int flow_assemble_momentum_residual_tiled(
+    const flow_mesh* mesh, const flow_space* W, const flow_space* P,
+    const flow_cell_tiles* tiles, const int* bfmask, const double* ui,
+    const double* u0, const double* p0, const flow_coef* f0,
+    const flow_coef* f1, const flow_ns_params* prm, double* scratch, double* F,
+    void* stream) {
+  int rc = check_mesh_space(mesh, W);
+  if (rc) return rc;
+  if ((rc = check_mesh_space(mesh, P))) return rc;
+  if ((rc = check_coef(f0))) return rc;
+  if ((rc = check_coef(f1))) return rc;
+  if ((rc = tiles_check(tiles, mesh, W))) return rc;
+  FLOW_REQUIRE(P->deg == 1, "pressure space must be P1");
+  FLOW_REQUIRE(bfmask && ui && u0 && p0 && prm && scratch && F, "pointers");
+  FLOW_REQUIRE(prm->dt > 0.0 && prm->rho > 0.0 && prm->mu > 0.0, "parameters");
+  hipStream_t st = as_stream(stream);
+  const ResidualCell<2> cell{mesh->nc, mesh->xy, W->cell_dofs, W->n,
+                             P->cell_dofs, bfmask, ui, u0, p0, *f0, *f1, *prm};
+  hipLaunchKernelGGL((tiled_cell_kernel<2, ResidualCell<2>, 2, 1>),
+                     dim3(tiles->ntiles), dim3(kBlock), 0, st, cell, *tiles,
+                     scratch, F, static_cast<size_t>(W->n),
+                     static_cast<const unsigned char*>(nullptr),
+                     static_cast<const double*>(nullptr), size_t(0),
+                     static_cast<const double*>(nullptr));
+  FLOW_CHECK_LAUNCH();
+  return gather_tile_rows(tiles, scratch, F, W->n, st, nullptr, nullptr,
+                          nullptr, 0);
 }
 
 extern "C" int flow_momentum_jvp_apply(const flow_momentum_jvp* J,
diff --git a/flow_amd/csrc/common.h b/flow_amd/csrc/common.h
--- a/flow_amd/csrc/common.h
+++ b/flow_amd/csrc/common.h
@@ -69,6 +69,17 @@
                        const double* stop = nullptr,
                        const double* prm_dev = nullptr);
 int momentum_jvp_params(const flow_momentum_jvp* J, double* dst, hipStream_t st);
+int momentum_jvp_tiled_check(const flow_momentum_jvp_tiled* A);
+int momentum_jvp_tiled_apply(const flow_momentum_jvp_tiled* A, const double* v,
+                             double* out, hipStream_t st, int v_stride = 0,
+                             int out_stride = 0, const double* stop = nullptr,
+                             const double* prm_dev = nullptr);
+inline const flow_momentum_jvp* operator_jvp(const flow_operator* A) {
+  if (A->kind == 3) return static_cast<const flow_momentum_jvp*>(A->matfree);
+  if (A->kind == 5 && A->matfree)
+    return static_cast<const flow_momentum_jvp_tiled*>(A->matfree)->J;
+  return nullptr;
+}
 
 constexpr long long kReplayAutoRows = 1500000;
 struct KeyHash {
diff --git a/flow_amd/csrc/la_kernels.hip b/flow_amd/csrc/la_kernels.hip
--- a/flow_amd/csrc/la_kernels.hip
+++ b/flow_amd/csrc/la_kernels.hip
@@ -220,7 +220,15 @@
 
 int check_operator(const flow_operator* A) {
   FLOW_REQUIRE(A != nullptr, "operator is NULL");
-  FLOW_REQUIRE(A->kind >= 0 && A->kind <= 4, "operator kind");
+  FLOW_REQUIRE(A->kind >= 0 && A->kind <= 5, "operator kind");
+  if (A->kind == 5) {
+    const flow_momentum_jvp_tiled* T =
+        static_cast<const flow_momentum_jvp_tiled*>(A->matfree);
+    int rc = momentum_jvp_tiled_check(T);
+    if (rc) return rc;
+    FLOW_REQUIRE(A->n == T->J->W->n, "matrix-free operator size");
+    return FLOW_OK;
+  }
   if (A->kind == 3) {
     const flow_momentum_jvp* J =
         static_cast<const flow_momentum_jvp*>(A->matfree);
@@ -259,10 +267,12 @@
 
 void key_operator(KeyHash& k, const flow_operator* A, bool skip_prm) {
   k.obj(A);
-  if (A && A->kind == 3 && A->matfree) {
-    flow_momentum_jvp J = *static_cast<const flow_momentum_jvp*>(A->matfree);
+  if (A && (A->kind == 3 || A->kind == 5) && A->matfree) {
+    flow_momentum_jvp J = *operator_jvp(A);
     if (skip_prm) J.prm = flow_ns_params{0.0, 0.0, 0.0, 0.0, 0.0};
     k.obj(&J).obj(J.mesh).obj(J.W);
+    if (A->kind == 5)
+      k.obj(static_cast<const flow_momentum_jvp_tiled*>(A->matfree)->tiles);
   }
 }
 
@@ -274,6 +284,12 @@
     FLOW_REQUIRE(dpart == nullptr, "matrix-free operators carry no fused dot");
     return momentum_jvp_apply(static_cast<const flow_momentum_jvp*>(A->matfree),
                               x, y, st, vec_stride, out_stride, stop, jvp_prm);
+  }
+  if (A->kind == 5) {
+    FLOW_REQUIRE(dpart == nullptr, "matrix-free operators carry no fused dot");
+    return momentum_jvp_tiled_apply(
+        static_cast<const flow_momentum_jvp_tiled*>(A->matfree), x, y, st,
+        vec_stride, out_stride, stop, jvp_prm);
   }
   const int xs = vec_stride ? vec_stride : A->n;
   const dim3 grid(A->nblocks, A->kind == 1 ? 2 : 1);
@@ -1326,7 +1342,8 @@
   int rc = check_operator(A);
   if (rc) return rc;
   FLOW_REQUIRE(diag_idx && dinv, "diag_idx, dinv");
-  FLOW_REQUIRE(A->kind != 3, "a matrix-free operator has no stored diagonal");
+  FLOW_REQUIRE(A->kind != 3 && A->kind != 5,
+               "a matrix-free operator has no stored diagonal");
   const double* v1 = (A->kind == 0 || A->kind == 4)
                          ? A->vals[0]
                          : (A->kind == 1 ? A->vals[1] : A->vals[3]);
@@ -2136,10 +2153,9 @@
     key_operator(base, A, true);
     base.pod(dinv).obj(ilu).obj(ilu ? ilu->plan : nullptr).obj(pmg);
     base.pod(work).pod(N).pod(m);
-    if (A->kind == 3) {
+    if (operator_jvp(A)) {
       jprm = G + kGJvp;
-      if ((rc = momentum_jvp_params(
-               static_cast<const flow_momentum_jvp*>(A->matfree), G + kGJvp, st)))
+      if ((rc = momentum_jvp_params(operator_jvp(A), G + kGJvp, st)))
         return rc;
     }
   }
@@ -2275,7 +2291,8 @@
                              first_check, work, work_len, 5, iters_host,
                              resid_host);
   if (rc) return rc;
-  FLOW_REQUIRE(A->kind != 3, "CG: assembled (symmetric) operators only");
+  FLOW_REQUIRE(A->kind != 3 && A->kind != 5,
+               "CG: assembled (symmetric) operators only");
   if (coarse) {
     FLOW_REQUIRE(dinv != nullptr, "two-level preconditioner needs dinv");
     FLOW_REQUIRE(A->kind == 0, "two-level preconditioner: scalar operators");
@@ -2309,7 +2326,8 @@
                              first_check, work, work_len, 5, iters_host,
                              resid_host);
   if (rc) return rc;
-  FLOW_REQUIRE(A->kind != 3, "CG: assembled (symmetric) operators only");
+  FLOW_REQUIRE(A->kind != 3 && A->kind != 5,
+               "CG: assembled (symmetric) operators only");
   if (coarse) {
     FLOW_REQUIRE(dinv != nullptr, "two-level preconditioner needs dinv");
     FLOW_REQUIRE(A->kind == 0, "two-level preconditioner: scalar operators");
diff --git a/flow_amd/fem/ops.py b/flow_amd/fem/ops.py
--- a/flow_amd/fem/ops.py
+++ b/flow_amd/fem/ops.py
@@ -34,6 +34,50 @@
             )
         layout._dev['struct'] = s
     return layout._dev['struct']
+
+
+def cell_tiles(layout):
+    if layout.degree != 2:
+        return None
+    if 'tiles_struct' not in layout._dev:
+        nc = layout.mesh.num_cells()
+        nt = layout.tiles('ntiles')
+        nrows = len(layout.tiles('rows'))
+        nbrows = len(layout.tiles('brows'))
+
+        def dev(name, numel, dtype=torch.int32):
+            t = layout.dev('tiles.' + name)
+            return _hip._ptr(t, dtype, numel, name)
+        s = _hip.CellTiles(
+            nt, nc, layout.N, layout.tiles('nbnd'), nbrows,
+            dev('cell_ptr', nt + 1), dev('cells', nc), dev('cell_bnd', nc),
+            dev('row_ptr', nt + 1), dev('rows', nrows),
+            dev('ent_ptr', nrows + 1),
+            dev('slots', len(layout.tiles('slots')), torch.int16),
+            dev('brows', nbrows), dev('bptr', nbrows + 1),
+            dev('bsrc', len(layout.tiles('bsrc'))),
+            )
+        layout._dev['tiles_struct'] = s
+    return layout._dev['tiles_struct']
+
+
+def assemble_momentum(mesh_s, space_s, pspace_s, tiles, bfmask, ui, u0, p0,
+                      f0s, f1s, prm, buf, F, Jvals, j_stride, st):
+    lib = _hip.lib()
+    if F is not None and tiles is not None:
+        _hip.check(lib.flow_assemble_momentum_residual_tiled(
+            ctypes.byref(mesh_s), ctypes.byref(space_s), ctypes.byref(pspace_s),
+            ctypes.byref(tiles), bfmask, ui, u0, p0, ctypes.byref(f0s),
+            ctypes.byref(f1s), ctypes.byref(prm), buf, F, st
+            ))
+        F = None
+        if Jvals is None:
+            return
+    _hip.check(lib.flow_assemble_momentum(
+        ctypes.byref(mesh_s), ctypes.byref(space_s), ctypes.byref(pspace_s),
+        bfmask, ui, u0, p0, ctypes.byref(f0s), ctypes.byref(f1s),
+        ctypes.byref(prm), buf, F, Jvals, j_stride, st
+        ))
 
 
 _G_CACHE = {}
@@ -195,6 +239,8 @@
         self.size = W.size()
         n2 = self.size
         nc = mesh.num_cells()
+        self.tiles = cell_tiles(W.layout) \
+            if mesh_s is None and space_s is None else None
         if mesh_s is None:
             mesh_s = mesh_struct(mesh)
         if space_s is None:
@@ -210,9 +256,17 @@
             self._bc_mask(bc_dofs),
             )
         op = _hip.Operator()
-        op.kind = 3
         op.n = W.layout.N
-        op.matfree = ctypes.cast(ctypes.pointer(self.struct), ctypes.c_void_p)
+        if self.tiles is None:
+            op.kind = 3
+            op.matfree = ctypes.cast(ctypes.pointer(self.struct),
+                                     ctypes.c_void_p)
+        else:
+            self.tiled = _hip.MomentumJvpTiled(ctypes.pointer(self.struct),
+                                               ctypes.pointer(self.tiles))
+            op.kind = 5
+            op.matfree = ctypes.cast(ctypes.pointer(self.tiled),
+                                     ctypes.c_void_p)
         self._op = op
 
     def operator(self):
@@ -256,6 +310,12 @@
     def apply(self, x, y):
         lib = _hip.lib()
         assert x.data_ptr() != y.data_ptr()
+        if self.tiles is not None:
+            _hip.check(lib.flow_momentum_jvp_tiled_apply(
+                ctypes.byref(self.tiled), _hip.f64(x, self.size, 'x'),
+                _hip.f64(y, self.size, 'y'), _hip.stream()
+                ))
+            return y
         _hip.check(lib.flow_momentum_jvp_apply(
             ctypes.byref(self.struct), _hip.f64(x, self.size, 'x'),
             _hip.f64(y, self.size, 'y'), _hip.stream()
diff --git a/flow_amd/fem/space.py b/flow_amd/fem/space.py
--- a/flow_amd/fem/space.py
+++ b/flow_amd/fem/space.py
@@ -4,6 +4,8 @@
 
 SPMV_ROWS_PER_BLOCK = 256
 SPMV_NNZ_PER_BLOCK = 1022
+TILE_CELLS = 512
+TILE_BOX = (16, 16)
 
 
 class ScalarLayout(object):
@@ -44,6 +46,7 @@
         self.cell_dofs = numpy.ascontiguousarray(self.cell_dofs)
         self._pattern = None
         self._vmap = None
+        self._tiles = None
         self._dev = {}
         return
 
@@ -113,6 +116,83 @@
             self._build_vmap()
         return self._vmap[name]
 
+    def _build_tiles(self):
+        mesh = self.mesh
+        nc, nloc, T = len(self.cell_dofs), self.nloc, TILE_CELLS
+        vptr = self.vmap('vptr').astype(numpy.int64)
+        vsrc = self.vmap('vsrc').astype(numpy.int64)
+        p = mesh.points[mesh.cell_vertices]
+        cen = p.mean(axis=1)
+        d1, d2 = p[:, 1] - p[:, 0], p[:, 2] - p[:, 0]
+        area = 0.5 * numpy.abs(d1[:, 0] * d2[:, 1] - d1[:, 1] * d2[:, 0])
+        h = numpy.sqrt(2.0 * area.sum() / nc)
+        lo = mesh.points.min(axis=0)
+        bx = numpy.floor((cen[:, 0] - lo[0]) / (TILE_BOX[0] * h)).astype(numpy.int64)
+        by = numpy.floor((cen[:, 1] - lo[1]) / (TILE_BOX[1] * h)).astype(numpy.int64)
+        cells = numpy.lexsort((numpy.arange(nc), by, bx))
+        box = bx[cells] * (by.max() + 1) + by[cells]
+        starts = numpy.flatnonzero(numpy.r_[True, box[1:] != box[:-1]])
+        sizes = numpy.diff(numpy.r_[starts, nc])
+        parts = -(-sizes // T)
+        cut = [starts]
+        for k in range(2, int(parts.max()) + 1):
+            for j in range(1, k):
+                sel = parts == k
+                cut.append(starts[sel] + (sizes[sel] * j) // k)
+        cell_ptr = numpy.r_[numpy.unique(numpy.concatenate(cut)), nc]
+        ntiles = len(cell_ptr) - 1
+        assert numpy.diff(cell_ptr).max() <= T
+        tile = numpy.empty(nc, dtype=numpy.int64)
+        tile[cells] = numpy.repeat(numpy.arange(ntiles), numpy.diff(cell_ptr))
+        pos = numpy.empty(nc, dtype=numpy.int64)
+        pos[cells] = numpy.arange(nc) - numpy.repeat(cell_ptr[:-1],
+                                                     numpy.diff(cell_ptr))
+        counts = numpy.diff(vptr)
+        ctile = tile[vsrc % nc]
+        tmin = numpy.minimum.reduceat(ctile, vptr[:-1])
+        interior = tmin == numpy.maximum.reduceat(ctile, vptr[:-1])
+        rows = numpy.flatnonzero(interior)
+        rows = rows[numpy.argsort(tmin[rows], kind='stable')]
+        row_ptr = numpy.zeros(ntiles + 1, dtype=numpy.int64)
+        numpy.cumsum(numpy.bincount(tmin[rows], minlength=ntiles),
+                     out=row_ptr[1:])
+        ent = vsrc[_segments(vptr, rows)]
+        slots = (ent // nc) * T + pos[ent % nc]
+        bnd = ~interior[self.cell_dofs[cells]]
+        mask = (bnd * (1 << numpy.arange(nloc))).sum(axis=1)
+        base = numpy.r_[0, numpy.cumsum(bnd.sum(axis=1))]
+        nbnd = int(base[-1])
+        assert nbnd < 1 << 26 and nloc <= 6
+        cbase = numpy.empty(nc, dtype=numpy.int64)
+        cbase[cells] = base[:-1]
+        brows = numpy.flatnonzero(~interior)
+        bent = vsrc[_segments(vptr, brows)]
+        bc, bi = bent % nc, bent // nc
+        cmask = numpy.empty(nc, dtype=numpy.int64)
+        cmask[cells] = mask
+        low = cmask[bc] & ((1 << bi) - 1)
+        bsrc = cbase[bc] + _popcount(low)
+        i32 = numpy.int32
+        self._tiles = {
+            'ntiles': ntiles, 'nbnd': nbnd,
+            'cell_ptr': cell_ptr.astype(i32),
+            'cells': cells.astype(i32),
+            'cell_bnd': ((mask << 26) | base[:-1]).astype(numpy.uint32),
+            'row_ptr': row_ptr.astype(i32),
+            'rows': rows.astype(i32),
+            'ent_ptr': numpy.r_[0, numpy.cumsum(counts[rows])].astype(i32),
+            'slots': slots.astype(numpy.uint16),
+            'brows': brows.astype(i32),
+            'bptr': numpy.r_[0, numpy.cumsum(counts[brows])].astype(i32),
+            'bsrc': bsrc.astype(i32),
+            }
+        return
+
+    def tiles(self, name):
+        if self._tiles is None:
+            self._build_tiles()
+        return self._tiles[name]
+
     def dev(self, name):
         from .. import device
         if name not in self._dev:
@@ -120,12 +200,30 @@
                 arr = numpy.ascontiguousarray(self.cell_dofs.T)
             elif name in ('vptr', 'vsrc'):
                 arr = self.vmap(name)
+            elif name.startswith('tiles.'):
+                arr = self.tiles(name[6:])
+                arr = arr.view({numpy.dtype(numpy.uint32): numpy.int32,
+                                numpy.dtype(numpy.uint16): numpy.int16}.get(
+                                    arr.dtype, arr.dtype))
             else:
                 arr = self.pattern(name)
             if name == 'cols':
                 arr = numpy.concatenate([arr, numpy.zeros(4, dtype=arr.dtype)])
             self._dev[name] = device.to_device(arr)
         return self._dev[name]
+
+
+def _segments(ptr, rows):
+    counts = ptr[rows + 1] - ptr[rows]
+    first = numpy.cumsum(counts) - counts
+    return numpy.repeat(ptr[rows] - first, counts) + numpy.arange(counts.sum())
+
+
+def _popcount(x):
+    n = numpy.zeros_like(x)
+    for b in range(8):
+        n += (x >> b) & 1
+    return n
 
 
 def csr_stream_rowblocks(rowptr, rows_per_block=SPMV_ROWS_PER_BLOCK,
diff --git a/flow_amd/navier_stokes/pressure_correction.py b/flow_amd/navier_stokes/pressure_correction.py
--- a/flow_amd/navier_stokes/pressure_correction.py
+++ b/flow_amd/navier_stokes/pressure_correction.py
@@ -263,18 +263,18 @@
     ms = ops.mesh_struct(mesh)
     ws = ops.space_struct(lay)
     ps = ops.space_struct(P.layout)
+    tiles = ops.cell_tiles(lay)
     st = _hip.stream()
     npar = solver_parameters['newton']
 
     def assemble(want_f, want_j):
-        _hip.check(lib.flow_assemble_momentum(
-            ctypes.byref(ms), ctypes.byref(ws), ctypes.byref(ps),
-            _hip.i32(bfmask, nc, 'bfmask'), _hip.f64(ui.data, n2),
-            _hip.f64(u[0].data, n2), _hip.f64(p0.data, P.size()),
-            ctypes.byref(f0s), ctypes.byref(f1s), ctypes.byref(prm),
-            _hip.f64(buf), _hip.f64(F, n2) if want_f else None,
+        ops.assemble_momentum(
+            ms, ws, ps, tiles, _hip.i32(bfmask, nc, 'bfmask'),
+            _hip.f64(ui.data, n2), _hip.f64(u[0].data, n2),
+            _hip.f64(p0.data, P.size()), f0s, f1s, prm, _hip.f64(buf),
+            _hip.f64(F, n2) if want_f else None,
             _hip.f64(J.vals, 4 * J.stride) if want_j else None, J.stride, st
-            ))
+            )
 
     def residual():
         assemble(True, False)
diff --git a/include/flow_hip.h b/include/flow_hip.h
--- a/include/flow_hip.h
+++ b/include/flow_hip.h
@@ -446,6 +446,39 @@
 int flow_momentum_jvp_apply(const flow_momentum_jvp* J, const double* v,
                             double* out, void* stream);
 
+#define FLOW_TILE_CELLS 512
+typedef struct {
+  int ntiles;
+  int nc;
+  int n;
+  int nbnd;
+  int nbrows;
+  const int* cell_ptr;
+  const int* cells;
+  const unsigned* cell_bnd;
+  const int* row_ptr;
+  const int* rows;
+  const int* ent_ptr;
+  const unsigned short* slots;
+  const int* brows;
+  const int* bptr;
+  const int* bsrc;
+} flow_cell_tiles;
+
+typedef struct {
+  const flow_momentum_jvp* J;
+  const flow_cell_tiles* tiles;
+} flow_momentum_jvp_tiled;
+int flow_momentum_jvp_tiled_apply(const flow_momentum_jvp_tiled* A,
+                                  const double* v, double* out, void* stream);
+
+int flow_assemble_momentum_residual_tiled(
+    const flow_mesh* mesh, const flow_space* W, const flow_space* P,
+    const flow_cell_tiles* tiles, const int* bfmask, const double* ui,
+    const double* u0, const double* p0, const flow_coef* f0,
+    const flow_coef* f1, const flow_ns_params* prm, double* scratch, double* F,
+    void* stream);
+
 int flow_assemble_source(const flow_mesh* mesh, const flow_space* V, int dim,
                          const flow_coef* f, double* scratch, double* b,
                          void* stream);
```

New measurement: 121.8, median of 2. -4.2%, worse.
